# jackhwalters/DCS-Net

Measured on AMD Instinct MI355X. Metric: STFT frames/sec (train fwd+bwd+Adam), higher is better.
Workload: dtype f32

## Files before the change

dcs-net_amd/csrc/attention.hip:

```cpp
#include "conv_common.h"
#include "cbn_geom.h"

namespace {

constexpr int kThreads = 256;
#ifndef DCS_ATT_APP_IT
#define DCS_ATT_APP_IT 2
#endif
#ifndef DCS_ATT_GRID_CAP
#define DCS_ATT_GRID_CAP 8192
#endif
constexpr int kMaxChunks = DCS_ATT_MAX_CHUNKS;

inline bool att_geom(int C, int* G) { return att::geom(C, G); }
inline int ca_chunks(long HW, int G) { return att::ca_chunks(HW, G); }

__device__ __forceinline__ void ca_pool_kernel_body(const act_t* __restrict__ x, double* __restrict__ part,
                                                            long HW, int C, int G, int bx, int by, int gx) {
    __shared__ double red[kThreads * 4];
    const int t = threadIdx.x, g = t % G, r0 = t / G, rpi = kThreads / G;
    const int b = by;
    const ActIn4<act_t> x4 = act_in4(x) + (long)b * HW * G;
    float s0 = 0.f, s1 = 0.f, s2 = 0.f, s3 = 0.f;
    for (long r = (long)bx * rpi + r0; r < HW; r += (long)gx * rpi) {
        const float4 v = x4[r * G + g];
        s0 += v.x; s1 += v.y; s2 += v.z; s3 += v.w;
    }
    red[t * 4 + 0] = s0; red[t * 4 + 1] = s1; red[t * 4 + 2] = s2; red[t * 4 + 3] = s3;
    __syncthreads();
    for (int o = t; o < G * 4; o += kThreads) {
        const int gg = o / 4, i = o % 4;
        double a = 0;
        for (int r = 0; r < rpi; ++r) a += red[(r * G + gg) * 4 + i];
        part[(((long)b * gx + bx) * C + 2 * gg) * 2 + i] = a;
    }
}

__device__ __forceinline__ void ca_fc_kernel_body(const double* __restrict__ part, int nchunks,
                                                          const float2* __restrict__ w1, const float2* __restrict__ w2,
                                                          float2* __restrict__ ca_out, float2* __restrict__ pooled_out,
                                                          float2* __restrict__ hidden_out, long HW, int C, int Ch, int bx, int by, int gx) {
    __shared__ float2 pooled[128];
    __shared__ float2 hid[64];
    __shared__ double red[kThreads * 2];
    const int b = bx, t = threadIdx.x;
    {
        const int nsl = kThreads / C, c = t % C, sl = t / C;
        double sr = 0, si = 0;
        if (sl < nsl)
#pragma unroll 8
            for (int k = sl; k < nchunks; k += nsl) {
                const double* p = part + (((long)b * nchunks + k) * C + c) * 2;
                sr += p[0]; si += p[1];
            }
        red[t * 2] = sr; red[t * 2 + 1] = si;
        __syncthreads();
        if (t < C) {
            for (int q = 1; q < nsl; ++q) { sr += red[(q * C + t) * 2]; si += red[(q * C + t) * 2 + 1]; }
            const float2 m = make_float2((float)(sr / (double)HW), (float)(si / (double)HW));
            pooled[t] = m;
            pooled_out[(long)b * C + t] = m;
        }
    }
    __syncthreads();
    for (int h = t >> 5; h < Ch; h += kThreads / 32) {
        float ar = 0.f, ai = 0.f;
#pragma unroll 4
        for (int c = t & 31; c < C; c += 32) {
            const float2 w = w1[c * Ch + h], p = pooled[c];
            ar = fmaf(w.x, p.x, ar); ar = fmaf(-w.y, p.y, ar);
            ai = fmaf(w.x, p.y, ai); ai = fmaf(w.y, p.x, ai);
        }
#pragma unroll
        for (int o = 16; o > 0; o >>= 1) { ar += __shfl_xor(ar, o, 64); ai += __shfl_xor(ai, o, 64); }
        if ((t & 31) == 0) {
            hidden_out[(long)b * Ch + h] = make_float2(ar, ai);
            hid[h] = make_float2(ar > 0.f ? ar : 0.f, ai > 0.f ? ai : 0.f);
        }
    }
    __syncthreads();
    for (int c = t; c < C; c += kThreads) {
        float ar = 0.f, ai = 0.f;
#pragma unroll 8
        for (int h = 0; h < Ch; ++h) {
            const float2 w = w2[h * C + c], p = hid[h];
            ar = fmaf(w.x, p.x, ar); ar = fmaf(-w.y, p.y, ar);
            ai = fmaf(w.x, p.y, ai); ai = fmaf(w.y, p.x, ai);
        }
        ar += ar; ai += ai;
        ca_out[(long)b * C + c] = make_float2(1.f / (1.f + expf(-ar)), 1.f / (1.f + expf(-ai)));
    }
}

__device__ __forceinline__ float group_sum(float v, int G) { return dcs_group_sum(v, G); }
__device__ __forceinline__ float group_max(float v, int G) { return dcs_group_max(v, G); }

__device__ __forceinline__ void spatial_pool_kernel_body(const act_t* __restrict__ x,
                                                                 const float* __restrict__ ca,
                                                                 float4* __restrict__ pooled, long HW, int C, int G, int bx, int by, int gx) {
    const int t = threadIdx.x, g = t % G, r0 = t / G, rpi = kThreads / G;
    const int b = by;
    const ActIn4<act_t> x4 = act_in4(x) + (long)b * HW * G;
    float4 a = make_float4(1.f, 0.f, 1.f, 0.f);
    if (ca) a = reinterpret_cast<const float4*>(ca)[(long)b * G + g];
    const float invC = 1.f / (float)C;
    const long iters = (HW + (long)gx * rpi - 1) / ((long)gx * rpi);
    for (long k = 0; k < iters; ++k) {
        const long r = (k * gx + bx) * rpi + r0;
        const bool ok = r < HW;
        float4 v = make_float4(0.f, 0.f, 0.f, 0.f);
        if (ok) v = x4[r * G + g];
        const float z0r = a.x * v.x - a.y * v.y, z0i = a.x * v.y + a.y * v.x;
        const float z1r = a.z * v.z - a.w * v.w, z1i = a.z * v.w + a.w * v.z;
        const float sr = group_sum(z0r + z1r, G), si = group_sum(z0i + z1i, G);
        const float mr = group_max(fmaxf(z0r, z1r), G), mi = group_max(fmaxf(z0i, z1i), G);
        if (ok && g == 0) pooled[(long)b * HW + r] = make_float4(sr * invC, si * invC, mr, mi);
    }
}

template <bool DROP>
__device__ __forceinline__ void attention_apply_kernel_body(const act_t* __restrict__ x,
                                                                    const float* __restrict__ ca,
                                                                    const float2* __restrict__ sa, act_t* __restrict__ y,
                                                                    long HW, int C, int G, float drop_p, uint64_t seed, const uint64_t* __restrict__ seed_dev, int bx, int by, int gx) {
    if (seed_dev) seed += seed_dev[0];
    const int t = threadIdx.x, g = t % G, r0 = t / G, rpi = kThreads / G;
    const int b = by;
    const long base = (long)b * HW * G;
    const ActIn4<act_t> x4 = act_in4(x) + base;
    const ActOut4<act_t> y4 = act_out4(y) + base;
    float4 a = make_float4(1.f, 0.f, 1.f, 0.f);
    if (ca) a = reinterpret_cast<const float4*>(ca)[(long)b * G + g];
    const float inv_keep = DROP ? 1.f / (1.f - drop_p) : 1.f;
    for (long r = (long)bx * rpi + r0; r < HW; r += (long)gx * rpi) {
        const float4 v = x4[r * G + g];
        float2 s = make_float2(1.f, 0.f);
        if (sa) s = sa[(long)b * HW + r];
        const float z0r = fmaf(a.x, v.x, -(a.y * v.y)), z0i = fmaf(a.x, v.y, a.y * v.x);
        const float z1r = fmaf(a.z, v.z, -(a.w * v.w)), z1i = fmaf(a.z, v.w, a.w * v.z);
        float4 o;
        o.x = fmaf(s.x, z0r, -(s.y * z0i)); o.y = fmaf(s.x, z0i, s.y * z0r);
        o.z = fmaf(s.x, z1r, -(s.y * z1i)); o.w = fmaf(s.x, z1i, s.y * z1r);
        if (DROP) {
            const uint64_t e = (uint64_t)(base + r * G + g) * 4;
            o.x *= dcs_keep_scale(seed, e, drop_p, inv_keep);
            o.y *= dcs_keep_scale(seed, e + 1, drop_p, inv_keep);
            o.z *= dcs_keep_scale(seed, e + 2, drop_p, inv_keep);
            o.w *= dcs_keep_scale(seed, e + 3, drop_p, inv_keep);
        }
        y4[r * G + g] = o;
    }
}

constexpr int kMaxBatch = 8;
template <class P> struct Tbl { P p[kMaxBatch]; int x0[kMaxBatch + 1]; };
template <class P> __device__ __forceinline__ int tbl_find(const Tbl<P>& t, int bx) {
    int z = 0;
#pragma unroll
    for (int k = 1; k < kMaxBatch; ++k) z += bx >= t.x0[k] ? 1 : 0;
    return z;
}

struct CaPoolP { const act_t* x; double* part; long HW; int C, G, nx; };
struct CaFcP { const double* part; int nchunks; const float2* w1; const float2* w2; float2* ca; float2* pooled; float2* hidden;
               long HW; int C, Ch; };
struct SpPoolP { const act_t* x; const float* ca; float4* pooled; long HW; int C, G, nx; };
struct ApplyP { const act_t* x; const float* ca; const float2* sa; act_t* y; long HW; int C, G, nx; };

__global__ __launch_bounds__(kThreads) void ca_pool_kernel(CaPoolP p) {
    ca_pool_kernel_body(p.x, p.part, p.HW, p.C, p.G, blockIdx.x, blockIdx.y, gridDim.x);
}
__global__ __launch_bounds__(kThreads) void ca_pool_multi_kernel(Tbl<CaPoolP> t) {
    const int z = tbl_find(t, blockIdx.x);
    const CaPoolP& p = t.p[z];
    ca_pool_kernel_body(p.x, p.part, p.HW, p.C, p.G, blockIdx.x - t.x0[z], blockIdx.y, p.nx);
}
__global__ __launch_bounds__(kThreads) void ca_fc_kernel(CaFcP p) {
    ca_fc_kernel_body(p.part, p.nchunks, p.w1, p.w2, p.ca, p.pooled, p.hidden, p.HW, p.C, p.Ch, blockIdx.x, 0, 0);
}
__global__ __launch_bounds__(kThreads) void ca_fc_multi_kernel(Tbl<CaFcP> t) {
    const CaFcP& p = t.p[blockIdx.z];
    ca_fc_kernel_body(p.part, p.nchunks, p.w1, p.w2, p.ca, p.pooled, p.hidden, p.HW, p.C, p.Ch, blockIdx.x, 0, 0);
}
__global__ __launch_bounds__(kThreads) void spatial_pool_kernel(SpPoolP p) {
    spatial_pool_kernel_body(p.x, p.ca, p.pooled, p.HW, p.C, p.G, blockIdx.x, blockIdx.y, gridDim.x);
}
__global__ __launch_bounds__(kThreads) void spatial_pool_multi_kernel(Tbl<SpPoolP> t) {
    const int z = tbl_find(t, blockIdx.x);
    const SpPoolP& p = t.p[z];
    spatial_pool_kernel_body(p.x, p.ca, p.pooled, p.HW, p.C, p.G, blockIdx.x - t.x0[z], blockIdx.y, p.nx);
}
template <bool DROP>
__global__ __launch_bounds__(kThreads) void attention_apply_kernel(ApplyP p, float drop_p, uint64_t seed, const uint64_t* seed_dev) {
    attention_apply_kernel_body<DROP>(p.x, p.ca, p.sa, p.y, p.HW, p.C, p.G, drop_p, seed, seed_dev, blockIdx.x, blockIdx.y, gridDim.x);
}
__global__ __launch_bounds__(kThreads) void attention_apply_multi_kernel(Tbl<ApplyP> t) {
    const int z = tbl_find(t, blockIdx.x);
    const ApplyP& p = t.p[z];
    attention_apply_kernel_body<false>(p.x, p.ca, p.sa, p.y, p.HW, p.C, p.G, 0.f, 0, nullptr, blockIdx.x - t.x0[z], blockIdx.y, p.nx);
}

#ifndef DCS_ACT_BF16
__global__ __launch_bounds__(kThreads) void dropout_kernel(const float* __restrict__ x, float* __restrict__ y, long n,
                                                            float drop_p, uint64_t seed, const uint64_t* __restrict__ seed_dev) {
    if (seed_dev) seed += seed_dev[0];
    const float inv_keep = 1.f / (1.f - drop_p);
    for (long i = (long)blockIdx.x * kThreads + threadIdx.x; i < n; i += (long)gridDim.x * kThreads)
        y[i] = x[i] * (drop_p > 0.f ? dcs_keep_scale(seed, (uint64_t)i, drop_p, inv_keep) : 1.f);
}
#endif

inline int stream_grid(long HW, int G, int B) {
    const int rpi = kThreads / G;
    long it = (HW + rpi - 1) / rpi;
    long nb = it <= DCS_ATT_SMALL_IT ? (it + DCS_ATT_APP_IT - 1) / DCS_ATT_APP_IT : (it + 3) / 4;
    long cap = (it <= DCS_ATT_SMALL_IT ? DCS_ATT_GRID_CAP : 2048) / (B > 0 ? B : 1);
    if (cap < 1) cap = 1;
    return (int)(nb < 1 ? 1 : (nb > cap ? cap : nb));
}

}

#ifndef DCS_ACT_BF16
extern "C" long dcs_ca_workspace_bytes(int B, long HW, int C) {
    int G;
    if (B <= 0 || HW <= 0 || !att_geom(C, &G)) return -1;
    return (long)B * ca_chunks(HW, G) * C * 2 * (long)sizeof(double);
}
#endif

extern "C" int DCS_SYM(dcs_channel_attention_fwd)(const act_t* x, const float* w1, const float* w2, float* ca_out,
                                         float* pooled_out, float* hidden_out, void* workspace, long workspace_bytes,
                                         int B, long HW, int C, int Ch, dcs_stream_t stream) {
    int G;
    if (!x || !w1 || !w2 || !ca_out || !pooled_out || !hidden_out || !workspace) return DCS_ERR_BADARG;
    if (B <= 0 || B > 65535 || HW <= 0 || !att_geom(C, &G) || Ch <= 0 || Ch > 64) return DCS_ERR_BADARG;
    const int nch = ca_chunks(HW, G);
    if (workspace_bytes < (long)B * nch * C * 2 * (long)sizeof(double)) return DCS_ERR_WORKSPACE;
    hipStream_t s = dcs_stream(stream);
    const CaPoolP pp{x, (double*)workspace, HW, C, G, nch};
    DCS_LAUNCH(ca_pool_kernel, dim3(nch, B), dim3(kThreads), 0, s, pp);
    DCS_CHECK_LAUNCH();
    const CaFcP fp{(const double*)workspace, nch, (const float2*)w1, (const float2*)w2, (float2*)ca_out, (float2*)pooled_out,
                   (float2*)hidden_out, HW, C, Ch};
    DCS_LAUNCH(ca_fc_kernel, dim3(B), dim3(kThreads), 0, s, fp);
    DCS_CHECK_LAUNCH();
    return DCS_OK;
}

#ifndef DCS_ACT_BF16
extern "C" int dcs_ca_pool_chunks(long HW, int C) {
    int G;
    if (HW <= 0 || !att_geom(C, &G)) return -1;
    return ca_chunks(HW, G);
}

extern "C" int dcs_channel_attention_fc_fwd(const void* part, const float* w1, const float* w2, float* ca_out,
                                            float* pooled_out, float* hidden_out, int B, long HW, int C, int Ch,
                                            dcs_stream_t stream) {
    int G;
    if (!part || !w1 || !w2 || !ca_out || !pooled_out || !hidden_out) return DCS_ERR_BADARG;
    if (B <= 0 || B > 65535 || HW <= 0 || !att_geom(C, &G) || Ch <= 0 || Ch > 64) return DCS_ERR_BADARG;
    const CaFcP fp{(const double*)part, ca_chunks(HW, G), (const float2*)w1, (const float2*)w2, (float2*)ca_out,
                   (float2*)pooled_out, (float2*)hidden_out, HW, C, Ch};
    DCS_LAUNCH(ca_fc_kernel, dim3(B), dim3(kThreads), 0, dcs_stream(stream), fp);
    DCS_CHECK_LAUNCH();
    return DCS_OK;
}
#endif

extern "C" int DCS_SYM(dcs_spatial_pool_fwd)(const act_t* x, const float* ca, float* pooled, int B, long HW, int C,
                                    dcs_stream_t stream) {
    int G;
    if (!x || !pooled || B <= 0 || B > 65535 || HW <= 0 || !att_geom(C, &G)) return DCS_ERR_BADARG;
    const int nx = stream_grid(HW, G, B);
    const SpPoolP sp{x, ca, (float4*)pooled, HW, C, G, nx};
    DCS_LAUNCH(spatial_pool_kernel, dim3(nx, B), dim3(kThreads), 0, dcs_stream(stream), sp);
    DCS_CHECK_LAUNCH();
    return DCS_OK;
}

extern "C" int DCS_SYM(dcs_attention_apply_fwd)(const act_t* x, const float* ca, const float* sa, act_t* y, int B, long HW,
                                       int C, float drop_p, unsigned long long seed, const unsigned long long* seed_dev, dcs_stream_t stream) {
    int G;
    if (!x || !y || B <= 0 || B > 65535 || HW <= 0 || !att_geom(C, &G)) return DCS_ERR_BADARG;
    if (!(drop_p >= 0.f && drop_p < 1.f)) return DCS_ERR_BADARG;
    const int nx = stream_grid(HW, G, B);
    dim3 grid(nx, B);
    const ApplyP ap{x, ca, (const float2*)sa, y, HW, C, G, nx};
    if (drop_p > 0.f)
        DCS_LAUNCH(attention_apply_kernel<true>, grid, dim3(kThreads), 0, dcs_stream(stream), ap, drop_p,
                           (uint64_t)seed, (const uint64_t*)seed_dev);
    else
        DCS_LAUNCH(attention_apply_kernel<false>, grid, dim3(kThreads), 0, dcs_stream(stream), ap, drop_p,
                           (uint64_t)seed, (const uint64_t*)seed_dev);
    DCS_CHECK_LAUNCH();
    return DCS_OK;
}

static long fwd_batched_workspace_bytes(int n, const dcs_attention_item* items, int B) {
    if (n < 1 || n > kMaxBatch || !items || B <= 0) return -1;
    long total = 0;
    for (int i = 0; i < n; ++i) {
        int G;
        if (!att_geom(items[i].C, &G)) return -1;
        const long b = (long)B * ca_chunks((long)items[i].H * items[i].W, G) * items[i].C * 2 * (long)sizeof(double);
        total += (b + 255) / 256 * 256;
    }
    return total;
}

#ifndef DCS_ACT_BF16
extern "C" long dcs_attention_fwd_batched_workspace_bytes(int n, const dcs_attention_item* items, int B) {
    return fwd_batched_workspace_bytes(n, items, B);
}
#endif

extern "C" int DCS_SYM(dcs_attention_fwd_batched)(int n, const dcs_attention_item* items, void* workspace, long workspace_bytes, int B,
                                         dcs_stream_t stream) {
    if (n < 1 || n > kMaxBatch || !items || !workspace || B <= 0 || B > 65535) return DCS_ERR_BADARG;
    if (workspace_bytes < fwd_batched_workspace_bytes(n, items, B)) return DCS_ERR_WORKSPACE;
    Tbl<CaPoolP> tp; Tbl<CaFcP> tf; Tbl<SpPoolP> ts; Tbl<ApplyP> ta;
    conv::Args ca_[kMaxBatch];
    int nx_pool = 1, nx_stream = 1;
    char* ws = (char*)workspace;
    for (int i = 0; i < n; ++i) {
        const dcs_attention_item& it = items[i];
        int G;
        if (!it.x || !it.w1 || !it.w2 || !it.wsa || !it.sa_bias || !it.ca || !it.pooled || !it.hidden || !it.sp || !it.sa ||
            !it.y || it.H <= 0 || it.W <= 0 || it.Ch <= 0 || it.Ch > 64 || !att_geom(it.C, &G))
            return DCS_ERR_BADARG;
        const long HW = (long)it.H * it.W;
        const int nch = ca_chunks(HW, G), nxs = stream_grid(HW, G, B);
        tp.p[i] = CaPoolP{(const act_t*)it.x, (double*)ws, HW, it.C, G, nch};
        tf.p[i] = CaFcP{(const double*)ws, nch, (const float2*)it.w1, (const float2*)it.w2, (float2*)it.ca, (float2*)it.pooled,
                        (float2*)it.hidden, HW, it.C, it.Ch};
        ts.p[i] = SpPoolP{(const act_t*)it.x, it.ca, (float4*)it.sp, HW, it.C, G, nxs};
        ta.p[i] = ApplyP{(const act_t*)it.x, it.ca, (const float2*)it.sa, (act_t*)it.y, HW, it.C, G, nxs};
        ws += ((long)B * nch * it.C * 2 * (long)sizeof(double) + 255) / 256 * 256;
        nx_pool = nch > nx_pool ? nch : nx_pool;
        nx_stream = nxs > nx_stream ? nxs : nx_stream;
        conv::Args& a = ca_[i];
        a = conv::Args{};
        a.x1 = (const act2_t*)it.sp;     a.x2 = nullptr; a.wp = (const float2*)it.wsa; a.bias = (const float2*)it.sa_bias;
        a.y = (act2_t*)it.sa;
        a.B = B; a.Hin = it.H; a.Win = it.W; a.C1 = 2; a.C2 = 0; a.up_f = 1; a.up_t = 1; a.zero_ins = 0; a.Cout = 1;
        a.kh = 7; a.kw = 7; a.sf = 1; a.st = 1; a.pad_f = 3; a.pad_t = 3; a.act = DCS_ACT_SIGMOID;
        a.Hv = it.H; a.Wv = it.W; a.Hout = it.H; a.Wout = it.W;
    }
    hipStream_t s = dcs_stream(stream);
    {
        int ap = 0, as_ = 0;
        for (int k = 0; k <= kMaxBatch; ++k) {
            tp.x0[k] = k < n ? ap : 0x7fffffff; ts.x0[k] = ta.x0[k] = k < n ? as_ : 0x7fffffff;
            if (k < n) { ap += tp.p[k].nx; as_ += ts.p[k].nx; }
        }
        tp.x0[n] = ap; ts.x0[n] = ta.x0[n] = as_;
        nx_pool = ap; nx_stream = as_;
    }
    DCS_LAUNCH(ca_pool_multi_kernel, dim3(nx_pool, B, 1), dim3(kThreads), 0, s, tp);
    DCS_CHECK_LAUNCH();
    DCS_LAUNCH(ca_fc_multi_kernel, dim3(B, 1, n), dim3(kThreads), 0, s, tf);
    DCS_CHECK_LAUNCH();
    DCS_LAUNCH(spatial_pool_multi_kernel, dim3(nx_stream, B, 1), dim3(kThreads), 0, s, ts);
    DCS_CHECK_LAUNCH();
    const int rc = dcs_conv_direct_multi(ca_, n, s);
    if (rc != DCS_OK) return rc;
    DCS_LAUNCH(attention_apply_multi_kernel, dim3(nx_stream, B, 1), dim3(kThreads), 0, s, ta);
    DCS_CHECK_LAUNCH();
    return DCS_OK;
}

#ifndef DCS_ACT_BF16
extern "C" int dcs_dropout_fwd(const float* x, float* y, long n, float drop_p, unsigned long long seed,
                               const unsigned long long* seed_dev, dcs_stream_t stream) {
    if (!x || !y || n <= 0 || !(drop_p >= 0.f && drop_p < 1.f)) return DCS_ERR_BADARG;
    long nb = (n + kThreads * 4 - 1) / (kThreads * 4);
    const int grid = (int)(nb < 1 ? 1 : (nb > 2048 ? 2048 : nb));
    DCS_LAUNCH(dropout_kernel, dim3(grid), dim3(kThreads), 0, dcs_stream(stream), x, y, n, drop_p,
                       (uint64_t)seed, (const uint64_t*)seed_dev);
    DCS_CHECK_LAUNCH();
    return DCS_OK;
}
#endif
```

dcs-net_amd/dcsnet/_lib.py:

```python
import ctypes
import os

_HERE = os.path.dirname(os.path.abspath(__file__))
LIB_PATH = os.environ.get('DCS_LIB_PATH') or os.path.join(os.path.dirname(_HERE), 'lib', 'libdcsnet_hip.so')

ACT_NONE, ACT_RELU, ACT_LRELU, ACT_SIGMOID = 0, 1, 2, 3

_P = ctypes.c_void_p
_I = ctypes.c_int
_L = ctypes.c_long
_F = ctypes.c_float
_U64 = ctypes.c_ulonglong



class AttentionItem(ctypes.Structure):
    _fields_ = [(n, _P) for n in ('x', 'w1', 'w2', 'wsa', 'sa_bias', 'ca', 'pooled', 'hidden', 'sp', 'sa', 'y', 'g_out',
                                  'wsa_bwd', 'g_pre', 'g_sp', 'g_x', 'g_fc0_r', 'g_fc0_i', 'g_fc2_r', 'g_fc2_i')] + \
               [(n, _I) for n in ('H', 'W', 'C', 'Ch')] + [('g_pooled', _P)]


SIGNATURES = {
    'dcs_abi_version': (_I, []),
    'dcs_error_string': (ctypes.c_char_p, [_I]),
    'dcs_pack_conv_weight': (_I, [_P, _P, _P, _P, _P, _P, _I, _I, _I, _I, _I, _I, _I, _P]),
    'dcs_cconv2d_fwd_workspace_bytes': (_L, [_I] * 14),
    'dcs_cconv2d_fwd': (_I, [_P, _P, _P, _P, _P, _P, _L] + [_I] * 15 + [_P]),
    'dcs_cconv2d_fwd_affine': (_I, [_P, _P, _P, _P, _P, _P, _P, _L] + [_I] * 15 + [_P]),
    'dcs_cconv2d_fwd_stats_rows': (_I, [_I] * 14),
    'dcs_cconv2d_fwd_stats': (_I, [_P] * 6 + [_I, _P, _P, _L] + [_I] * 14 + [_P]),
    'dcs_rconv2d_fwd_workspace_bytes': (_L, [_I] * 14),
    'dcs_rconv2d_fwd': (_I, [_P, _P, _P, _P, _P, _P, _L] + [_I] * 15 + [_P]),
    'dcs_rconv2d_bwd_data_workspace_bytes': (_L, [_I] * 11),
    'dcs_rconv2d_bwd_data': (_I, [_P, _P, _P, _P, _L] + [_I] * 11 + [_P]),
    'dcs_rbn_fwd': (_I, [_P] * 9 + [_L, _L, _I, _F, _F, _I, _I, _P]),
    'dcs_rbn_bwd': (_I, [_P] * 8 + [_L, _L, _I, _I, _I, _P]),
    'dcs_packed_weight_floats': (_L, [_I] * 6),
    'dcs_packed_weight_bwd_floats': (_L, [_I] * 10),
    'dcs_pack_conv_weight_bwd': (_I, [_P, _P] + [_I] * 10 + [_P]),
    'dcs_cconv2d_bwd_data_workspace_bytes': (_L, [_I] * 14),
    'dcs_cconv2d_bwd_data': (_I, [_P] * 5 + [_L] + [_I] * 14 + [_P]),
    'dcs_upsample_cat_bwd': (_I, [_P, _P, _P] + [_I] * 7 + [_P]),
    'dcs_cconv2d_bwd_weight_workspace_bytes': (_L, [_I] * 14),
    'dcs_cconv2d_bwd_weight': (_I, [_P] * 8 + [_L] + [_I] * 15 + [_P]),
    'dcs_cbn_workspace_bytes': (_L, [_L, _I]),
    'dcs_cbn_fwd': (_I, [_P] * 9 + [_L, _L, _I, _F, _F, _I, _I, _F, _U64, _P, _P]),
    'dcs_cbn_fwd_slabs': (_I, [_P] * 9 + [_I, _I, _P, _L, _I, _F, _F, _I, _F, _U64, _P, _P]),
    'dcs_ca_pool_chunks': (_I, [_L, _I]),
    'dcs_cbn_fwd_slabs_pool': (_I, [_P] * 9 + [_I, _I, _P, _P, _L, _I, _L, _I, _F, _F, _I, _P]),
    'dcs_channel_attention_fc_fwd': (_I, [_P] * 6 + [_I, _L, _I, _I, _P]),
    'dcs_cbn_bwd_workspace_bytes': (_L, [_L, _I]),
    'dcs_cbn_bwd': (_I, [_P] * 9 + [_L, _L, _I, _I, _I, _F, _U64, _P, _P]),
    'dcs_cbn_bwd_add': (_I, [_P] * 9 + [_L, _L, _I, _I, _I, _F, _U64, _P, _P, _F, _L, _P, _P]),
    'dcs_ca_workspace_bytes': (_L, [_I, _L, _I]),
    'dcs_channel_attention_fwd': (_I, [_P] * 7 + [_L, _I, _L, _I, _I, _P]),
    'dcs_spatial_pool_fwd': (_I, [_P, _P, _P, _I, _L, _I, _P]),
    'dcs_attention_apply_fwd': (_I, [_P, _P, _P, _P, _I, _L, _I, _F, _U64, _P, _P]),
    'dcs_rattention_workspace_bytes': (_L, [_I, _L, _I]),
    'dcs_rattention_fwd': (_I, [_P] * 8 + [_L] + [_I] * 6 + [_P]),
    'dcs_rattention_train_workspace_bytes': (_L, [_I, _L, _I, _I]),
    'dcs_rattention_pool_fwd': (_I, [_P] * 8 + [_L] + [_I] * 5 + [_P]),
    'dcs_rattention_apply_fwd': (_I, [_P] * 4 + [_I] * 4 + [_P]),
    'dcs_rattention_apply_bwd': (_I, [_P] * 8 + [_L] + [_I] * 4 + [_P]),
    'dcs_rattention_pool_bwd': (_I, [_P] * 11 + [_I] + [_P, _L] + [_I] * 5 + [_P]),
    'dcs_attention_bwd_sa': (_I, [_P] * 5 + [_I, _L, _I, _F, _U64, _P, _P]),
    'dcs_attention_bwd_workspace_bytes': (_L, [_I, _L, _I, _I]),
    'dcs_attention_bwd_x': (_I, [_P] * 16 + [_L, _I, _L, _I, _I, _F, _U64, _P, _P]),
    'dcs_attention_bwd_fc_weights': (_I, [_P, _L, _P, _P, _P, _P, _P, _P, _I, _L, _I, _I, _P]),
    'dcs_attention_fwd_batched_workspace_bytes': (_L, [_I, _P, _I]),
    'dcs_attention_fwd_batched': (_I, [_I, _P, _P, _L, _I, _P]),
    'dcs_attention_bwd_batched_workspace_bytes': (_L, [_I, _P, _I]),
    'dcs_attention_bwd_batched': (_I, [_I, _P, _P, _L, _I, _P]),
    'dcs_lstm_layer_fwd': (_I, [_P] * 6 + [_I, _I, _I, _I, _L, _L, _L, _P]),
    'dcs_lstm_layer_fwd_bias': (_I, [_P, _P, _P, _P, _P, _P, _P, _P, _I, _I, _I, _I, _L, _L, _L, _P]),
    'dcs_lstm_layer_bwd': (_I, [_P] * 6 + [_I] * 4 + [_P]),
    'dcs_dropout_fwd': (_I, [_P, _P, _L, _F, _U64, _P, _P]),
    'dcs_complex_act_fwd': (_I, [_P, _P, _L, _I, _P]),
    'dcs_complex_upsample_fwd': (_I, [_P, _P, _I, _I, _I, _I, _I, _I, _P]),
    'dcs_tapsum_fwd': (_I, [_P, _P, _P, _P] + [_I] * 10 + [_P]),
    'dcs_cconv_up2_single_fwd': (_I, [_P] * 6 + [_I] * 6 + [_P]),
    'dcs_cconv_up2_single_bwd_data': (_I, [_P] * 4 + [_I] * 6 + [_P]),
    'dcs_cconv_up2_single_bwd_weight_workspace_bytes': (_L, []),
    'dcs_cconv_up2_single_bwd_weight': (_I, [_P] * 7 + [_I, _P, _L] + [_I] * 5 + [_P]),
    'dcs_tapsum_bwd_workspace_bytes': (_L, []),
    'dcs_tapsum_bwd': (_I, [_P, _P, _P, _P, _P, _L] + [_I] * 10 + [_P]),
    'dcs_bound_crm_fwd': (_I, [_P, _P, _L, _F, _P]),
    'dcs_bound_mask_apply_fwd': (_I, [_P, _P, _P, _P, _P, _L, _F, _P]),
    'dcs_bound_mask_apply_bwd': (_I, [_P] * 6 + [_L, _F, _P]),
    'dcs_bound2_mask_apply_fwd': (_I, [_P] * 6 + [_L, _F, _F, _U64, _P, _P]),
    'dcs_bound2_mask_apply_bwd': (_I, [_P] * 7 + [_L, _F, _F, _U64, _P, _P]),
    'dcs_bound2_apply_polar_frames_fwd': (_I, [_P] * 4 + [_I] * 4 + [_F, _F, _U64, _P, _P]),
    'dcs_bound2_apply_polar_frames_bwd': (_I, [_P] * 5 + [_I] * 4 + [_F, _I, _F, _U64, _P, _P]),
    'dcs_complex_abs_f32': (_I, [_P, _P, _L, _P]),
    'dcs_rmask_apply_polar_frames_fwd': (_I, [_P] * 4 + [_I] * 4 + [_F, _I, _P]),
    'dcs_rmask_apply_polar_frames_bwd': (_I, [_P] * 5 + [_I] * 4 + [_F, _I, _I, _P]),
    'dcs_irfft512_frames': (_I, [_P, _P, _L, _P]),
    'dcs_rfft512_frames': (_I, [_P, _P, _L, _P]),
    'dcs_rfft512_ola_frames': (_I, [_P, _P, _P, _P, _I, _I, _I, _F, _P]),
    'dcs_irfft512_ola_frames': (_I, [_P, _P, _P, _P, _I, _I, _I, _F, _P]),
    'dcs_polar_frames_fwd': (_I, [_P, _P, _I, _I, _I, _I, _F, _P]),
    'dcs_polar_frames_bwd': (_I, [_P, _P, _P, _I, _I, _I, _I, _F, _I, _P]),
    'dcs_istft_envelope': (_I, [_P, _P, _I, _I, _I, _P]),
    'dcs_istft_ola_fwd': (_I, [_P, _P, _P, _P, _I, _I, _I, _I, _F, _P]),
    'dcs_istft_ola_bwd': (_I, [_P, _P, _P, _P, _I, _I, _I, _I, _F, _P]),
    'dcs_stft_frames_fwd': (_I, [_P, _P, _P, _P, _I, _I, _I, _I, _I, _P]),
    'dcs_stft_bins_fwd': (_I, [_P, _P, _I, _I, _I, _F, _P]),
    'dcs_sisnr_fwd': (_I, [_P, _P, _P, _P, _I, _I, _F, _P]),
    'dcs_sisnr_bwd': (_I, [_P, _P, _P, _P, _F, _P, _I, _I, _P]),
    'dcs_sisnr_losses_fwd': (_I, [_P, _P, _P, _I, _F, _P]),
    'dcs_lstm_whh_grad': (_I, [_P, _P, _P, _I, _I, _I, _P]),
    'dcs_atb_chunks': (_I, [_P, _P, _P, _L, _L, _L, _L, _I, _I, _I, _I, _I, _I, _I, _I, _P]),
    'dcs_chunk_sum_acc': (_I, [_P, _P, _L, _L, _I, _I, _I, _L, _P]),
    'dcs_atb_chunks_strided': (_I, [_P, _P, _P, _L, _L, _L, _L, _I, _I, _I, _I, _I, _I, _I, _I, _I, _P]),
    'dcs_gemm_f32': (_I, [_P, _P, _P] + [_I] * 8 + [_L, _L, _I, _L, _L, _L, _I, _I, _P]),
    'dcs_lstm_combine_fwd': (_I, [_P, _P, _L, _P]),
    'dcs_lstm_combine_bwd': (_I, [_P, _P, _L, _P]),
    'dcs_lstm_param_grads': (_I, [_P, _P, _P, _P, _P, _I, _I, _I, _P]),
    'dcs_lstm_param_grads_ih': (_I, [_P, _P, _P, _P, _P, _I, _I, _I, _P, _P, _I, _L, _I, _P]),
    'dcs_sisnr_losses_guard_fwd': (_I, [_P, _P, _P, _I, _F, _P, _P]),
    'dcs_sisnr_pair_bwd': (_I, [_P, _P, _P, _P, _P, _P, _F, _P, _I, _I, _P]),
    'dcs_crm_fwd': (_I, [_P, _P, _P, _L, _F, _P]),
    'dcs_adam_amsgrad_step': (_I, [_P] * 6 + [_F, _F, _L, _P, _F, _F, _F, _F, _I, _P, _P, _P]),
    'dcs_adam_amsgrad_step_sumsq': (_I, [_P] * 6 + [_I, _F, _F, _L, _P, _F, _F, _F, _F, _I, _P, _P, _P]),
    'dcs_swa_average_f32': (_I, [_P, _P, _L, _L, _P]),
    'dcs_grad_sumsq_parts': (_I, [_P, _L, _P, _I, _P, _P, _P, _P, _I, _P]),
    'dcs_step_guard': (_I, [_P, _P, _P]),
    'dcs_stream_hold': (_I, [_P, _I, _P]),
    'dcs_kernel_timer_begin': (_I, [_I]),
    'dcs_kernel_timer_end': (_I, []),
    'dcs_kernel_timer_read': (_I, [_I, _P]),
    'dcs_step_advance': (_I, [_P, _P, _P, _P]),
    'dcs_step_advance_counters': (_I, [_P, _P, _P, _P, _I, _P]),
    'dcs_pack_tap_rows': (_I, [_P, _P, _P, _P, _I, _I, _I, _I, _P]),
    'dcs_tap_rows_wgrad_scatter': (_I, [_P, _P, _P, _P, _I, _I, _I, _I, _P]),
    'dcs_set_conv_precision': (_I, [_I]),
    'dcs_get_conv_precision': (_I, []),
    'dcs_wgrad_defer_begin': (_I, []),
    'dcs_wgrad_defer_suspend': (_I, [_I]),
    'dcs_wgrad_defer_flush': (_I, [_P]),
    'dcs_pack_plan_begin': (_I, []),
    'dcs_pack_plan_end': (_I, [_P]),
    'dcs_pack_plan_jobs': (_I, [_P, _P, _P]),
    'dcs_pack_plan_run': (_I, [_P, _P]),
    'dcs_pack_plan_destroy': (_I, [_P]),
    'dcs_resample_poly_f32': (_I, [_P, _P, _I, _L, _P, _I, _I, _I, _P]),
    'dcs_stoi_workspace_bytes': (_L, [_I, _L]),
    'dcs_stoi_f32': (_I, [_P, _P, _I, _L, _P, _P, _P, _P, _P, _L, _P]),
    'dcs_resample_sinc_f32': (_I, [_P, _P, _P, _P, _I, _L, _P, _I, _I, _I, _P]),
    'dcs_audio_stft_batch_f32': (_I, [_P, _P, _P, _I, _P, _P, _I, _P, _I, _I, _I, _F, _P, _P, _P, _P]),
    'dcs_audio_stft_segments_f32': (_I, [_P, _P, _I, _P, _P, _I, _P, _I, _I, _I, _I, _F, _P, _P]),
    'dcs_segments_stitch_f32': (_I, [_P, _L, _P, _P, _I, _L, _I, _I, _I, _P, _P, _P]),
}

_lib = None


class DcsHipError(RuntimeError):
    pass


for _n in ('dcs_cconv2d_fwd', 'dcs_cconv2d_fwd_affine', 'dcs_cconv2d_fwd_stats', 'dcs_cconv2d_bwd_data', 'dcs_cconv2d_bwd_weight',
           'dcs_cconv_up2_single_fwd', 'dcs_cconv_up2_single_bwd_data', 'dcs_cconv_up2_single_bwd_weight', 'dcs_tapsum_bwd', 'dcs_cbn_fwd', 'dcs_cbn_fwd_slabs', 'dcs_cbn_fwd_slabs_pool', 'dcs_cbn_bwd', 'dcs_cbn_bwd_add',
           'dcs_channel_attention_fwd', 'dcs_spatial_pool_fwd', 'dcs_attention_apply_fwd', 'dcs_attention_fwd_batched',
           'dcs_attention_bwd_sa', 'dcs_attention_bwd_x', 'dcs_attention_bwd_batched'):
    SIGNATURES[_n + '_h'] = SIGNATURES[_n]


def load():
    global _lib
    if _lib is not None:
        return _lib
    import torch
    if not os.path.exists(LIB_PATH):
        raise DcsHipError(f'{LIB_PATH} not found: build it with `python dcs-net_amd/build.py` '
                          '(there is no CPU or eager fallback)')
    lib = ctypes.CDLL(LIB_PATH)
    for name, (res, args) in SIGNATURES.items():
        try:
            fn = getattr(lib, name)
        except AttributeError as e:
            raise DcsHipError(f'{LIB_PATH} does not export {name}; rebuild it') from e
        fn.restype = res
        fn.argtypes = args
    _lib = lib
    return lib


def check(code, what):
    if code != 0:
        msg = load().dcs_error_string(code).decode()
        raise DcsHipError(f'{what}: {msg} (code {code})')


def ptr(t):
    return None if t is None else t.data_ptr()


def cur_stream():
    import torch
    return torch.cuda.current_stream().cuda_stream
```

dcs-net_amd/dcsnet/functional.py:

```python
import os
import weakref

import torch

from . import _derived
from . import ops
from .ops import ACT_NONE, ACT_RELU, ACT_LRELU, ACT_SIGMOID, to_nhwc, from_nhwc
from ._lib import DcsHipError

_PACKED = _derived.Derived(capacity=512)


def bump_param_generation():
    _derived.bump_generation()
    ops.pack_plan_invalidate()


def note_state_update():
    _derived.bump_generation()


state_generation = _derived.generation


def begin_pack_plan():
    _derived.bump_generation()
    return ops.pack_plan_begin()


def end_pack_plan():
    return ops.pack_plan_end()


def run_pack_plan(plan):
    ops.pack_plan_run(plan)


def packed_weight(w_r, w_i, b_r, b_i, transposed, up=(1, 1), tap_rows=0):
    plan = ops.PLAN
    if plan is not None:
        pkey = (id(w_r), id(w_i), id(b_r), id(b_i), bool(transposed), tuple(up), int(tap_rows))
        if plan.valid and not plan.recording:
            e = plan.fwd.get(pkey)
            if e is not None and e[0][0]() is w_r and e[0][1]() is w_i and e[2] == (
                    w_r._version, w_i._version, None if b_r is None else b_r._version,
                    None if b_i is None else b_i._version):
                return e[1]

    def make():
        d = lambda t: None if t is None else t.detach()
        wr, wi = d(w_r), d(w_i)
        if wr.dim() == 2:
            wr, wi = wr.view(*wr.shape, 1, 1), wi.view(*wi.shape, 1, 1)
        if tap_rows:
            packed = ops.pack_tap_rows(wr, wi, int(tap_rows))
        else:
            packed = ops.pack_conv_weight(wr, wi, d(b_r), d(b_i), transposed, tuple(up))
        if plan is not None and plan.recording:
            wref = lambda t: None if t is None else weakref.ref(t)
            plan.fwd[pkey] = [(wref(w_r), wref(w_i), wref(b_r), wref(b_i)), packed, None]
        return packed
    return _PACKED.get(w_r, (bool(transposed), tuple(up), int(tap_rows)), (w_r, w_i, b_r, b_i), make, ops.conv_precision())


ATTENTION_BATCH_MAX = ops.ATTENTION_BATCH_MAX

FLUSH_AT_NEXT_FORK = False
WGRAD_SIDE = None
sink_hits = 0


def _sink(p):
    if p is None or not p.requires_grad:
        return None
    s = getattr(p, '_dcs_grad_sink', None)
    if s is None or p.grad is None or p.grad.data_ptr() != s.data_ptr():
        return None
    global sink_hits
    sink_hits += 1
    return s


DEFER_FC = os.environ.get('DCS_DEFER_FC', '1') != '0'
PENDING_SIDE = []


def _run_pending_side():
    while PENDING_SIDE:
        job = PENDING_SIDE.pop(0)
        ops.attention_bwd_fc_weights(job)
        if ops.WGRAD_DEFER is not None:
            ops.WGRAD_DEFER.append(job)


class _CConv2dFn(torch.autograd.Function):

    @staticmethod
    def forward(ctx, x1, x2, w_r, w_i, b_r, b_i, transposed, ksize, stride, pad, up, act, holder=None):
        wp, bias = packed_weight(w_r, w_i, b_r, b_i, transposed, up)
        if holder is not None:
            y, holder['stat'] = ops.cconv2d_stats(x1, x2, wp, bias, ksize, stride, pad, up)
        else:
            y = ops.cconv2d(x1, x2, wp, bias, ksize, stride, pad, up, act)
        ctx.geom = (transposed, tuple(ksize), tuple(stride), tuple(pad), tuple(up), act, tuple(w_r.shape),
                    b_r is not None)
        ctx.sinks = (_sink(w_r), _sink(w_i), _sink(b_r), _sink(b_i))
        ctx.save_for_backward(x1, x2, wp, y if act == ACT_SIGMOID else None)
        return y

    @staticmethod
    def backward(ctx, gy):
        x1, x2, wp, y = ctx.saved_tensors
        transposed, ksize, stride, pad, up, act, w_shape, has_bias = ctx.geom
        gy = gy.contiguous()
        if act == ACT_SIGMOID:
            gy = gy * y * (1.0 - y)
        elif act != ACT_NONE:
            raise DcsHipError('cconv2d backward: only ACT_NONE / ACT_SIGMOID epilogues are differentiable here')
        gx1 = gx2 = gw_r = gw_i = gb_r = gb_i = None
        need = ctx.needs_input_grad
        want_w = need[2] or need[3] or need[4] or need[5]
        side = None
        if (want_w and WGRAD_SIDE is not None and ops.WGRAD_DEFER is not None and gy.is_cuda and
                ctx.sinks[0] is not None and ctx.sinks[1] is not None and (not has_bias or (ctx.sinks[2] is not None and ctx.sinks[3] is not None))):
            side = WGRAD_SIDE
            side.wait_stream(torch.cuda.current_stream())
        if need[0] or need[1]:
            C1 = x1.shape[3]
            Cin = C1 + (x2.shape[3] if x2 is not None else 0)
            gx1, gx2 = ops.cconv2d_bwd_data(gy, ops.pack_conv_weight_bwd(wp, ksize, stride, pad, up),
                                            (x1.shape[1], x1.shape[2], Cin), ksize, stride, pad, up, C1)
        if want_w:
            if side is not None:
                with torch.cuda.stream(side):
                    _run_pending_side()
                    g = ops.cconv2d_bwd_weight(x1, x2, gy, w_shape, has_bias, ksize, stride, pad, up, transposed, ctx.sinks,
                                               immediate=True)
                    global FLUSH_AT_NEXT_FORK
                    if FLUSH_AT_NEXT_FORK:
                        FLUSH_AT_NEXT_FORK = False
                        ops.wgrad_defer_flush(partial=True)
            else:
                g = ops.cconv2d_bwd_weight(x1, x2, gy, w_shape, has_bias, ksize, stride, pad, up, transposed, ctx.sinks)
            gw_r, gw_i, gb_r, gb_i = (None if sk is not None else t for t, sk in zip(g, ctx.sinks))
        return gx1, gx2, gw_r, gw_i, gb_r, gb_i, None, None, None, None, None, None, None


def cconv2d(x1, x2, w_r, w_i, b_r, b_i, transposed, ksize, stride, pad, up=(1, 1), act=ACT_NONE):
    return _CConv2dFn.apply(x1, x2, w_r, w_i, b_r, b_i, transposed, tuple(ksize), tuple(stride), tuple(pad),
                            tuple(up), act)


def cconv2d_with_stats(x1, x2, w_r, w_i, b_r, b_i, transposed, ksize, stride, pad, up=(1, 1)):
    holder = {}
    y = _CConv2dFn.apply(x1, x2, w_r, w_i, b_r, b_i, transposed, tuple(ksize), tuple(stride), tuple(pad), tuple(up),
                         ACT_NONE, holder)
    return y, holder.get('stat')


def cconv2d_cbn_eval(x1, x2, w_r, w_i, b_r, b_i, transposed, ksize, stride, pad, up, coef, act):
    wp, bias = packed_weight(w_r, w_i, b_r, b_i, transposed, tuple(up))
    return ops.cconv2d(x1, x2, wp, bias, tuple(ksize), tuple(stride), tuple(pad), tuple(up), act, coef=coef)


class _CbnFn(torch.autograd.Function):

    @staticmethod
    def forward(ctx, x, weight, bias, running_mean, running_covar, eps, momentum, use_batch_stats, act, drop_p, seed, stat=None):
        y, stats, coef = ops.cbn(x, weight, bias, running_mean, running_covar, eps, momentum, use_batch_stats,
                                 act, drop_p, seed, stat=stat)
        ctx.cfg = (bool(use_batch_stats), act, float(drop_p), int(seed), weight is not None)
        ctx.sinks = (_sink(weight), _sink(bias))
        ctx.save_for_backward(x, weight, stats, coef)
        return y

    @staticmethod
    def backward(ctx, g_out):
        x, weight, stats, coef = ctx.saved_tensors
        use_batch, act, drop_p, seed, affine = ctx.cfg
        g_x, g_w, g_b = ops.cbn_bwd(x, g_out.contiguous(), weight, stats, coef, use_batch, act, drop_p, seed, affine,
                                    ctx.sinks, need_gx=ctx.needs_input_grad[0])
        g_w = None if ctx.sinks[0] is not None else g_w
        g_b = None if ctx.sinks[1] is not None else g_b
        return g_x, g_w, g_b, None, None, None, None, None, None, None, None, None


def cbn(x, weight, bias, running_mean, running_covar, eps, momentum, use_batch_stats, act=ACT_NONE,
        drop_p=0.0, seed=0, stat=None):
    return _CbnFn.apply(x, weight, bias, running_mean, running_covar, eps, momentum, use_batch_stats, act,
                        drop_p, seed, stat)


class _CbnTwoFn(torch.autograd.Function):

    @staticmethod
    def forward(ctx, x, weight, bias, running_mean, running_covar, eps, momentum, use_batch_stats, act, drop_p, seed, stat=None):
        y, stats, coef = ops.cbn(x, weight, bias, running_mean, running_covar, eps, momentum, use_batch_stats,
                                 act, drop_p, seed, stat=stat)
        ctx.cfg = (bool(use_batch_stats), act, float(drop_p), int(seed), weight is not None)
        ctx.sinks = (_sink(weight), _sink(bias))
        ctx.save_for_backward(x, weight, stats, coef)
        ctx.set_materialize_grads(False)
        y2 = torch.empty(0, dtype=y.dtype, device=y.device).set_(y.untyped_storage(), y.storage_offset(), y.shape, y.stride())
        return y, y2

    @staticmethod
    def backward(ctx, g_a, g_b):
        x, weight, stats, coef = ctx.saved_tensors
        use_batch, act, drop_p, seed, affine = ctx.cfg
        if g_a is None and g_b is None:
            return (None,) * 12
        if g_a is None:
            g_a, g_b = g_b, None
        g_add = None
        for g_ in (g_a, g_b):
            if g_ is not None and _POOL_ADD:
                hit = _POOL_ADD.pop(g_.data_ptr(), None)
                if hit is not None:
                    if g_add is not None:
                        raise DcsHipError('cbn_two backward: two split pool terms for one stage output')
                    g_add = hit
        g_x, g_w, g_b_ = ops.cbn_bwd(x, g_a.contiguous(), weight, stats, coef, use_batch, act, drop_p, seed, affine,
                                     ctx.sinks, g_add=g_add, g_out2=None if g_b is None else g_b.contiguous())
        g_w = None if ctx.sinks[0] is not None else g_w
        g_b_ = None if ctx.sinks[1] is not None else g_b_
        return g_x, g_w, g_b_, None, None, None, None, None, None, None, None, None


def cbn_two(x, weight, bias, running_mean, running_covar, eps, momentum, use_batch_stats, act=ACT_NONE,
            drop_p=0.0, seed=0, stat=None):
    y, y2 = _CbnTwoFn.apply(x, weight, bias, running_mean, running_covar, eps, momentum, use_batch_stats, act,
                            drop_p, seed, stat)
    y2._dcs_adds_pool_term = True
    return y, y2


def channel_attention(x, fc0_r, fc0_i, fc2_r, fc2_i):
    w1, _ = packed_weight(fc0_r, fc0_i, None, None, False)
    w2, _ = packed_weight(fc2_r, fc2_i, None, None, False)
    ca, _, _ = ops.channel_attention(x, w1, w2)
    return ca


def spatial_attention(x, ca, conv_r, conv_i, ksize):
    pooled = ops.spatial_pool(x, ca)
    wp, bias = packed_weight(conv_r, conv_i, None, None, False)
    k = (ksize, ksize)
    return ops.cconv2d(pooled, None, wp, bias, k, (1, 1), (ksize // 2, ksize // 2), (1, 1), ACT_SIGMOID)


def attention_apply(x, ca, sa, drop_p=0.0, seed=0):
    return ops.attention_apply(x, ca, sa, drop_p, seed)


class _AttentionFn(torch.autograd.Function):

    @staticmethod
    def forward(ctx, x, fc0_r, fc0_i, fc2_r, fc2_i, c1_r, c1_i, ksize, drop_p, seed):
        w1, _ = packed_weight(fc0_r, fc0_i, None, None, False)
        w2, _ = packed_weight(fc2_r, fc2_i, None, None, False)
        wsa, zero_bias = packed_weight(c1_r, c1_i, None, None, False)
        ca, pooled, hidden = ops.channel_attention(x, w1, w2)
        sp = ops.spatial_pool(x, ca)
        sa = ops.cconv2d(sp, None, wsa, zero_bias, (ksize, ksize), (1, 1), (ksize // 2, ksize // 2), (1, 1),
                         ACT_SIGMOID)
        out = ops.attention_apply(x, ca, sa, drop_p, seed)
        ctx.cfg = (ksize, float(drop_p), int(seed))
        ctx.sinks = tuple(_sink(t) for t in (fc0_r, fc0_i, fc2_r, fc2_i, c1_r, c1_i))
        ctx.save_for_backward(x, ca, sa, sp, pooled, hidden, w1, w2, wsa)
        return out

    @staticmethod
    def backward(ctx, g_out):
        x, ca, sa, sp, pooled, hidden, w1, w2, wsa = ctx.saved_tensors
        ksize, drop_p, seed = ctx.cfg
        g = ops.attention_bwd(x, g_out.contiguous(), ca, sa, sp, pooled, hidden, w1, w2, wsa, ksize, drop_p, seed,
                              ctx.sinks)
        gw = tuple(None if sk is not None else t for t, sk in zip(g[1:], ctx.sinks))
        return (g[0], *gw, None, None, None)


def attention_block(x, fc0_r, fc0_i, fc2_r, fc2_i, c1_r, c1_i, ksize, drop_p=0.0, seed=0):
    return _AttentionFn.apply(x, fc0_r, fc0_i, fc2_r, fc2_i, c1_r, c1_i, ksize, drop_p, seed)


class _CbnAttentionFn(torch.autograd.Function):

    @staticmethod
    def forward(ctx, x, weight, bias, running_mean, running_covar, eps, momentum, use_batch_stats, act,
                fc0_r, fc0_i, fc2_r, fc2_i, c1_r, c1_i, ksize, drop_p, seed, stat=None):
        w1, _ = packed_weight(fc0_r, fc0_i, None, None, False)
        w2, _ = packed_weight(fc2_r, fc2_i, None, None, False)
        wsa, zero_bias = packed_weight(c1_r, c1_i, None, None, False)
        if stat is not None and use_batch_stats and weight is not None and ops.FUSE_APPLY_POOL:
            a, stats, coef, ca, pooled, hidden = ops.cbn_channel_attention(x, weight, bias, running_mean, running_covar, eps,
                                                                           momentum, act, stat, w1, w2)
        else:
            a, stats, coef = ops.cbn(x, weight, bias, running_mean, running_covar, eps, momentum, use_batch_stats, act, 0.0, 0,
                                     stat=stat)
            ca, pooled, hidden = ops.channel_attention(a, w1, w2)
        sp = ops.spatial_pool(a, ca)
        sa = ops.cconv2d(sp, None, wsa, zero_bias, (ksize, ksize), (1, 1), (ksize // 2, ksize // 2), (1, 1), ACT_SIGMOID)
        out = ops.attention_apply(a, ca, sa, drop_p, seed)
        ctx.cfg = (bool(use_batch_stats), act, weight is not None, ksize, float(drop_p), int(seed))
        ctx.sinks = tuple(_sink(t) for t in (weight, bias, fc0_r, fc0_i, fc2_r, fc2_i, c1_r, c1_i))
        ctx.save_for_backward(x, weight, stats, coef, a, ca, sa, sp, pooled, hidden, w1, w2, wsa)
        return out

    @staticmethod
    def backward(ctx, g_out):
        x, weight, stats, coef, a, ca, sa, sp, pooled, hidden, w1, w2, wsa = ctx.saved_tensors
        use_batch, act, affine, ksize, drop_p, seed = ctx.cfg
        sk = ctx.sinks
        defer = DEFER_FC and WGRAD_SIDE is not None and ops.WGRAD_DEFER is not None and all(s_ is not None for s_ in sk[2:6])
        g = ops.attention_bwd(a, g_out.contiguous(), ca, sa, sp, pooled, hidden, w1, w2, wsa, ksize, drop_p, seed, sk[2:],
                              split_pool=True, defer_fc=defer)
        if defer:
            PENDING_SIDE.append(g[8])
        g_x, g_w, g_b = ops.cbn_bwd(x, g[0], weight, stats, coef, use_batch, act, 0.0, 0, affine, sk[:2], g_add=g[7])
        full = (g_w, g_b, *g[1:7])
        gp = tuple(None if s_ is not None else t for t, s_ in zip(full, sk))
        return (g_x, gp[0], gp[1], None, None, None, None, None, None, *gp[2:], None, None, None, None)


def cbn_attention(x, weight, bias, running_mean, running_covar, eps, momentum, use_batch_stats, act,
                  fc0_r, fc0_i, fc2_r, fc2_i, c1_r, c1_i, ksize, drop_p=0.0, seed=0, stat=None):
    return _CbnAttentionFn.apply(x, weight, bias, running_mean, running_covar, eps, momentum, use_batch_stats, act,
                                 fc0_r, fc0_i, fc2_r, fc2_i, c1_r, c1_i, ksize, drop_p, seed, stat)


class _AttentionBlocksFn(torch.autograd.Function):

    @staticmethod
    def forward(ctx, n, ksize, split, *args):
        xs, params = args[:n], [args[n + 6 * i:n + 6 * i + 6] for i in range(n)]
        ctx.split = tuple(split)
        w1s, w2s, wsas, biases = [], [], [], []
        for fc0_r, fc0_i, fc2_r, fc2_i, c1_r, c1_i in params:
            w1s.append(packed_weight(fc0_r, fc0_i, None, None, False)[0])
            w2s.append(packed_weight(fc2_r, fc2_i, None, None, False)[0])
            wsa, zero_bias = packed_weight(c1_r, c1_i, None, None, False)
            wsas.append(wsa)
            biases.append(zero_bias)
        outs = ops.attention_blocks_fwd(xs, w1s, w2s, wsas, biases)
        ctx.n, ctx.ksize = n, ksize
        ctx.sinks = [tuple(_sink(t) for t in pr) for pr in params]
        ctx.shapes = [(tuple(pr[0].shape), tuple(pr[2].shape)) for pr in params]
        saved = []
        for x, o, w1, w2, wsa in zip(xs, outs, w1s, w2s, wsas):
            saved += [x, o['ca'], o['sa'], o['sp'], o['pooled'], o['hidden'], w1, w2, wsa]
        ctx.save_for_backward(*saved)
        return tuple(o['y'] for o in outs)

    @staticmethod
    def backward(ctx, *g_outs):
        n, ksize = ctx.n, ctx.ksize
        t = ctx.saved_tensors
        k, pad = (ksize, ksize), (ksize // 2, ksize // 2)
        saved, gs, wbs, fcs, sps = [], [], [], [], []
        for i in range(n):
            x, ca, sa, sp, pooled, hidden, w1, w2, wsa = t[9 * i:9 * i + 9]
            saved.append(dict(x=x, ca=ca, sa=sa, pooled=pooled, hidden=hidden, w1=w1, w2=w2))
            sps.append(sp)
            g = g_outs[i]
            gs.append(torch.zeros_like(x) if g is None else g.contiguous())
            wbs.append(ops.pack_conv_weight_bwd(wsa, k, (1, 1), pad))
            sk, (s0, s2) = ctx.sinks[i], ctx.shapes[i]
            new = lambda shape: torch.empty(shape, dtype=torch.float32, device=x.device)
            fcs.append(tuple(sk[j] if sk[j] is not None else new(s0 if j < 2 else s2) for j in range(4)))
        split = tuple(sp_ and ctx.needs_input_grad[3 + i] for i, sp_ in enumerate(ctx.split))
        res = ops.attention_blocks_bwd(saved, gs, wbs, fcs, split)
        if any(split):
            _POOL_ADD.clear()
            for (g_x, _, g_pooled), sp_ in zip(res, split):
                if sp_:
                    _POOL_ADD[g_x.data_ptr()] = g_pooled
            torch.autograd.Variable._execution_engine.queue_callback(_pool_add_consumed)
        grads_x, grads_p = [], []
        for i in range(n):
            g_x, g_pre, _ = res[i]
            sk = ctx.sinks[i]
            g_c1r, g_c1i, _, _ = ops.cconv2d_bwd_weight(sps[i], None, g_pre, (1, 2, ksize, ksize), False, k, (1, 1), pad,
                                                        outs=(sk[4], sk[5], None, None))
            full = (*fcs[i], g_c1r, g_c1i)
            grads_x.append(g_x)
            grads_p += [None if s_ is not None else g_ for g_, s_ in zip(full, sk)]
        global FLUSH_AT_NEXT_FORK
        if WGRAD_SIDE is not None and ops.WGRAD_DEFER is not None:
            ops.WGRAD_DEFER.append((sps, [r[1] for r in res]))
            FLUSH_AT_NEXT_FORK = True
        return (None, None, None, *grads_x, *grads_p)


SPLIT_SKIP_POOL = os.environ.get('DCS_SPLIT_SKIP_POOL', '1') != '0'
_POOL_ADD = {}


def _pool_add_consumed():
    if _POOL_ADD:
        _POOL_ADD.clear()
        raise DcsHipError('attention_blocks backward: a split average-pool term was not consumed by a cbn_two backward')


def attention_blocks(xs, params, ksize):
    flat = [p for pr in params for p in pr]
    split = tuple(bool(SPLIT_SKIP_POOL and getattr(x, '_dcs_adds_pool_term', False) and torch.is_grad_enabled() and x.requires_grad)
                  for x in xs)
    return _AttentionBlocksFn.apply(len(xs), ksize, split, *xs, *flat)



def _as_real(z):
    if z.dtype != torch.complex64:
        raise DcsHipError(f'expected complex64, got {z.dtype}')
    return torch.view_as_real(z.contiguous() if not _dense(z) else z)


def _dense(z):
    return z.is_contiguous() or (z.dim() == 4 and z.is_contiguous(memory_format=torch.channels_last))


def _elementwise(z, act):
    if z.dim() == 4 and z.is_contiguous(memory_format=torch.channels_last) and not z.is_contiguous():
        x = to_nhwc(z)
        return from_nhwc(ops.complex_act(x, act))
    x = torch.view_as_real(z.contiguous())
    return torch.view_as_complex(ops.complex_act(x, act))


def complex_relu(z):
    return _elementwise(z, ACT_RELU)


def complex_lrelu(z):
    return _elementwise(z, ACT_LRELU)


def complex_sigmoid(z):
    return _elementwise(z, ACT_SIGMOID)


def complex_upsample(z, scale_factor):
    sf = (scale_factor, scale_factor) if isinstance(scale_factor, (int, float)) else tuple(scale_factor)
    up = (int(sf[0]), int(sf[1]))
    if up != tuple(sf) or min(up) < 1:
        raise DcsHipError(f'complex_upsample: integer scale factors only, got {scale_factor}')
    return from_nhwc(ops.complex_upsample(to_nhwc(z), up))


def complex_linear(z, w_r, w_i, b_r, b_i):
    in_f = z.shape[-1]
    lead = z.shape[:-1]
    x = torch.view_as_real(z.reshape(-1, in_f).contiguous())
    N = x.shape[0]
    W = 16 if N % 16 == 0 else 1
    x = x.view(1, N // W, W, in_f, 2)
    y = cconv2d(x, None, w_r, w_i, b_r, b_i, False, (1, 1), (1, 1), (0, 0))
    return torch.view_as_complex(y.view(N, -1, 2)).view(*lead, -1)


class _LstmRecFn(torch.autograd.Function):

    @staticmethod
    def forward(ctx, gx, w_hh):
        n_sets, seqs, S, _, G4 = gx.shape
        need = gx.requires_grad or w_hh.requires_grad
        out, gates, c = ops.lstm_layer(gx, w_hh, n_sets, seqs, S, (seqs * S * 2 * G4, S * 2 * G4, 2 * G4), need)
        ctx.dims = (n_sets, seqs, S)
        if need:
            ctx.save_for_backward(out, gates, c, w_hh)
        return out

    @staticmethod
    def backward(ctx, g_out):
        out, gates, c, w_hh = ctx.saved_tensors
        n_sets, seqs, S = ctx.dims
        H = w_hh.shape[-1]
        g_pre = ops.lstm_layer_bwd(g_out.contiguous(), gates, c, w_hh, n_sets, seqs, S)
        g_pre5 = g_pre.view(n_sets, seqs, S, 2, 4 * H)
        g_whh = None
        if ctx.needs_input_grad[1]:
            o = out.view(n_sets, seqs, S, 2, H)
            h_prev = torch.zeros_like(o)
            h_prev[:, :, 1:, 0] = o[:, :, :-1, 0]
            h_prev[:, :, :-1, 1] = o[:, :, 1:, 1]
            g_whh = torch.einsum('sntdj,sntdk->sdjk', g_pre5, h_prev)
        return g_pre5, g_whh


def _project(inp, w_ih, shared, per_set=False, train=True):
    G8, K = w_ih.shape[1], w_ih.shape[2]
    M = inp.shape[-2]
    if not (ops.gemm_ok(M, G8, K, 2, train) and inp.is_contiguous() and w_ih.is_contiguous()):
        if shared and not per_set:
            return torch.mm(inp, w_ih.reshape(2 * G8, -1).t())
        return torch.matmul(inp, w_ih.transpose(1, 2))
    if shared and not per_set:
        gx = torch.empty((M, 2 * G8), dtype=torch.float32, device=inp.device)
        return ops.gemm_f32(inp, w_ih, gx, M, 2 * G8, K, K, K, 2 * G8, True)
    gx = torch.empty((2, M, G8), dtype=torch.float32, device=inp.device)
    return ops.gemm_f32(inp, w_ih, gx, M, G8, K, K, K, G8, True, nbatch=2, a_batch=0 if shared else M * K, b_batch=G8 * K,
                        c_batch=M * G8)


def _project_bwd(g_gx, w_ih, shared):
    G8, K = w_ih.shape[1], w_ih.shape[2]
    M = g_gx.shape[1]
    if not (ops.gemm_ok(M, K, G8, 2, True) and g_gx.is_contiguous() and w_ih.is_contiguous()):
        if shared:
            g_inp = torch.mm(g_gx[0], w_ih[0])
            return g_inp.addmm_(g_gx[1], w_ih[1])
        return torch.bmm(g_gx, w_ih)
    if shared:
        g_inp = torch.empty((M, K), dtype=torch.float32, device=g_gx.device)
        return ops.gemm_f32(g_gx, w_ih, g_inp, M, K, G8, G8, K, K, False, nseg=2, a_seg=M * G8, b_seg=G8 * K)
    g_inp = torch.empty((2, M, K), dtype=torch.float32, device=g_gx.device)
    return ops.gemm_f32(g_gx, w_ih, g_inp, M, K, G8, G8, K, K, False, nbatch=2, a_batch=M * G8, b_batch=G8 * K, c_batch=M * K)


class _ProjectFn(torch.autograd.Function):

    @staticmethod
    def forward(ctx, inp, w_ih):
        ctx.save_for_backward(inp, w_ih)
        return _project(inp, w_ih, shared=inp.dim() == 2, per_set=True)

    @staticmethod
    def backward(ctx, g):
        inp, w_ih = ctx.saved_tensors
        g = g.contiguous()
        g_inp = _project_bwd(g, w_ih, shared=inp.dim() == 2) if ctx.needs_input_grad[0] else None
        g_w = torch.matmul(g.transpose(1, 2), inp) if ctx.needs_input_grad[1] else None
        return g_inp, g_w


class _LstmLayerFn(torch.autograd.Function):

    @staticmethod
    def forward(ctx, inp, anchor, st, B2, S):
        w_ih, w_hh = st['weight_ih'][0], st['weight_hh'][0]
        need = inp.requires_grad or anchor.requires_grad
        ctx.planes = 0
        if inp.is_complex():
            zr = torch.view_as_real(inp)
            G8, K = w_ih.shape[1], w_ih.shape[2]
            ctx.planes = R0 = zr.shape[0] * zr.shape[1]
            gx = torch.empty((2 * R0, 2 * G8), dtype=torch.float32, device=inp.device)
            ops.gemm_f32(zr, w_ih, gx, 2 * R0, 2 * G8, K, K, K, 2 * G8, True, a_planes=R0)
            inp = zr
            G4 = G8 // 2
            strides = (G8, S * 2 * G8, 2 * G8)
        elif inp.dim() == 2:
            G8 = w_ih.shape[1]
            gx = _project(inp, w_ih, shared=True)
            G4 = G8 // 2
            strides = (G8, S * 2 * G8, 2 * G8)
        else:
            gx = _project(inp, w_ih, shared=False)
            G4 = gx.shape[-1] // 2
            strides = (B2 * S * 2 * G4, S * 2 * G4, 2 * G4)
        out, gates, c, hprev = ops.lstm_layer(gx, w_hh, 2, B2, S, strides, need, True,
                                              bias=(st['bias_ih'][0], st['bias_hh'][0]))
        ctx.st, ctx.dims = st, (B2, S)
        if need:
            ctx.save_for_backward(inp, hprev, gates, c)
        return out

    @staticmethod
    def backward(ctx, g_out):
        global sink_hits
        inp, hprev, gates, c = ctx.saved_tensors
        st, (B2, S) = ctx.st, ctx.dims
        w_ih, w_hh = st['weight_ih'][0], st['weight_hh'][0]
        H = w_hh.shape[-1]
        NT = B2 * S
        g_pre, b_part = ops.lstm_layer_bwd(g_out.contiguous(), gates, c, w_hh, 2, B2, S, True)
        g_gx = g_pre.view(2, NT, 8 * H)
        _LstmLayerFn._param_grads(st, inp, hprev, g_pre, b_part, g_gx, B2, S, H, NT, planes=ctx.planes)
        if ctx.planes:
            g_z = None
            if ctx.needs_input_grad[0]:
                G8, K = w_ih.shape[1], w_ih.shape[2]
                gz = torch.empty(inp.shape, dtype=torch.float32, device=inp.device)
                ops.gemm_f32(g_gx, w_ih, gz, NT, K, G8, G8, K, K, False, nseg=2, a_seg=NT * G8, b_seg=G8 * K, c_planes=ctx.planes)
                g_z = torch.view_as_complex(gz)
            return g_z, None, None, None, None
        g_inp = _project_bwd(g_gx, w_ih, shared=inp.dim() == 2) if ctx.needs_input_grad[0] else None
        return g_inp, None, None, None, None

    @staticmethod
    def _param_grads(st, inp, hprev, g_pre, b_part, g_gx, B2, S, H, NT, planes=0):
        global sink_hits
        CK = 16 if NT % 32 == 0 else 1
        if H % 64 == 0 and NT % (8 * CK) == 0:
            part = ops.lstm_whh_grad(g_pre, hprev, NT, CK, H)
        else:
            R = NT // CK
            part = torch.empty((2, 2 * CK, 4 * H, H), dtype=g_pre.dtype, device=g_pre.device)
            for d in range(2):
                a = g_pre.as_strided((2 * CK, R, 4 * H), (R * 8 * H, 8 * H, 1), g_pre.storage_offset() + d * 4 * H)
                h = hprev.as_strided((2 * CK, R, H), (R * 2 * H, 2 * H, 1), hprev.storage_offset() + d * H)
                torch.bmm(a.transpose(1, 2), h, out=part[d])
        b_part = b_part.contiguous()
        g_wih = st['weight_ih'][1]
        sink_hits += 16
        ih = None
# ... 563 lines not shown
```

dcs-net_amd/dcsnet/ops.py:

```python
import os as _os
import torch

from . import _lib
from ._lib import ACT_NONE, ACT_RELU, ACT_LRELU, ACT_SIGMOID, check, ptr, cur_stream


def _chk(t, name, dims=None, act=False):
    if t is None:
        return
    if not t.is_cuda:
        raise _lib.DcsHipError(f'{name}: expected a CUDA (HIP) tensor; the HIP path has no CPU fallback')
    if t.dtype != torch.float32 and not (act and t.dtype == torch.bfloat16):
        raise _lib.DcsHipError(f'{name}: expected float32{" or bfloat16" if act else ""}, got {t.dtype}')
    if not t.is_contiguous():
        raise _lib.DcsHipError(f'{name}: expected a contiguous tensor')
    if dims is not None and t.dim() != dims:
        raise _lib.DcsHipError(f'{name}: expected {dims} dims, got shape {tuple(t.shape)}')


def _sym(name, *acts):
    dts = {t.dtype for t in acts if t is not None}
    if len(dts) > 1:
        raise _lib.DcsHipError(f'{name}: activation tensors of different dtypes {sorted(str(d) for d in dts)}')
    bf = dts == {torch.bfloat16}
    if bf and conv_precision() != 'bf16' and 'conv' in name:
        raise _lib.DcsHipError(f'{name}: bf16 activations need set_conv_precision("bf16") (bf16 weight panels)')
    return getattr(_lib.load(), name + ('_h' if bf else ''))


CONV_TIMER = None

SEED_STATE = None

_workspaces = {}
_retired = []


def set_conv_precision(mode):
    code = {'f32': 0, 'fp32': 0, 'bf16': 1, 'bf16x6': 2}[mode]
    check(_lib.load().dcs_set_conv_precision(code), 'dcs_set_conv_precision')
    global BF16_OPERANDS_ON_PURPOSE, _conv_precision
    _conv_precision = _CONV_PRECISIONS[code]
    if code != 1:
        BF16_OPERANDS_ON_PURPOSE = False
    elif not _IN_SET_ACTIVATION_DTYPE:
        BF16_OPERANDS_ON_PURPOSE = True
    pack_plan_drop()


BF16_OPERANDS_ON_PURPOSE = _os.environ.get('DCS_CONV_PRECISION', '').strip() == '1'
_IN_SET_ACTIVATION_DTYPE = False


_CONV_PRECISIONS = ('f32', 'bf16', 'bf16x6')
_conv_precision = None


def conv_precision():
    global _conv_precision
    if _conv_precision is None:
        _conv_precision = _CONV_PRECISIONS[_lib.load().dcs_get_conv_precision()]
    return _conv_precision


class PackPlan:

    def __init__(self):
        self.handle, self.recording, self.valid = None, True, False
        self.fwd, self.bwd, self.keep = {}, {}, []

    def stats(self):
        import ctypes
        nj, nl = ctypes.c_int(0), ctypes.c_int(0)
        check(_lib.load().dcs_pack_plan_jobs(self.handle, ctypes.byref(nj), ctypes.byref(nl)), 'dcs_pack_plan_jobs')
        return nj.value, nl.value

    def __del__(self):
        try:
            if self.handle:
                _lib.load().dcs_pack_plan_destroy(self.handle)
        except Exception:
            pass


PLAN = None


def pack_plan_begin():
    global PLAN
    check(_lib.load().dcs_pack_plan_begin(), 'dcs_pack_plan_begin')
    PLAN = PackPlan()
    return PLAN


def pack_plan_end():
    import ctypes
    h = ctypes.c_void_p()
    plan = PLAN
    check(_lib.load().dcs_pack_plan_end(ctypes.byref(h)), 'dcs_pack_plan_end')
    plan.handle, plan.recording = h.value, False
    _plan_snapshot(plan)
    plan.valid = True
    return plan


def _plan_snapshot(plan):
    for e in plan.fwd.values():
        e[2] = tuple(None if r is None or r() is None else r()._version for r in e[0])


def pack_plan_run(plan):
    global PLAN
    PLAN = plan
    check(_lib.load().dcs_pack_plan_run(plan.handle, cur_stream()), 'dcs_pack_plan_run')
    _plan_snapshot(plan)
    plan.valid = True


def pack_plan_invalidate():
    if PLAN is not None:
        PLAN.valid = False


def pack_plan_drop():
    global PLAN
    PLAN = None



def _workspace(nbytes, device):
    key = (device.index, cur_stream())
    buf = _workspaces.get(key)
    if buf is None or buf.numel() < nbytes:
        if buf is not None:
            _retired.append(buf)
        buf = torch.empty(max(int(nbytes), 1 << 20), dtype=torch.uint8, device=device)
        _workspaces[key] = buf
    return buf


def pack_conv_weight(w_r, w_i, b_r=None, b_i=None, transposed=False, up=(1, 1)):
    for n, t in (('w_r', w_r), ('w_i', w_i), ('b_r', b_r), ('b_i', b_i)):
        _chk(t, n)
    if transposed:
        Cin, Cout, kh, kw = w_r.shape
    else:
        Cout, Cin, kh, kw = w_r.shape
    lib = _lib.load()
    buf = torch.empty(lib.dcs_packed_weight_floats(Cout, Cin, kh, kw, up[0], up[1]), dtype=torch.float32,
                      device=w_r.device)
    wp = buf[:kh * kw * Cin * Cout * 2].view(kh * kw, Cin, Cout, 2)
    bias = torch.empty((Cout, 2), dtype=torch.float32, device=w_r.device)
    check(lib.dcs_pack_conv_weight(ptr(w_r), ptr(w_i), ptr(b_r), ptr(b_i), ptr(wp), ptr(bias),
                                   Cout, Cin, kh, kw, int(bool(transposed)), up[0], up[1], cur_stream()),
          'dcs_pack_conv_weight')
    return wp, bias


def pack_tap_rows(w_r, w_i, ct):
    _chk(w_r, 'w_r', 4)
    _chk(w_i, 'w_i', 4)
    Cin, one, kh, kw = w_r.shape
    if one != 1 or ct < kh * kw:
        raise _lib.DcsHipError(f'pack_tap_rows: expected [Cin,1,kh,kw] and ct >= kh*kw, got {tuple(w_r.shape)}, ct={ct}')
    lib = _lib.load()
    buf = torch.empty(lib.dcs_packed_weight_floats(ct, Cin, 1, 1, 1, 1), dtype=torch.float32, device=w_r.device)
    wp = buf[:Cin * ct * 2].view(1, Cin, ct, 2)
    bias = torch.empty((ct, 2), dtype=torch.float32, device=w_r.device)
    check(lib.dcs_pack_tap_rows(ptr(w_r), ptr(w_i), ptr(wp), ptr(bias), Cin, kh, kw, ct, cur_stream()), 'dcs_pack_tap_rows')
    return wp, bias


def tap_rows_scatter(gt_r, gt_i, w_shape, outs=None):
    Cin, _, kh, kw = w_shape
    acc = outs is not None and outs[0] is not None and outs[1] is not None
    g_r = outs[0] if acc else torch.empty(w_shape, dtype=torch.float32, device=gt_r.device)
    g_i = outs[1] if acc else torch.empty(w_shape, dtype=torch.float32, device=gt_r.device)
    check(_lib.load().dcs_tap_rows_wgrad_scatter(ptr(gt_r), ptr(gt_i), ptr(g_r), ptr(g_i), Cin, kh, kw, int(acc),
                                                 cur_stream()), 'dcs_tap_rows_wgrad_scatter')
    return g_r, g_i


def cconv2d(x1, x2, wp, bias, ksize, stride=(1, 1), pad=(0, 0), up=(1, 1), act=ACT_NONE, coef=None):
    _chk(x1, 'x1', 5, act=True)
    _chk(x2, 'x2', 5, act=True)
    _chk(wp, 'wp', 4)
    _chk(bias, 'bias', 2)
    B, Hin, Win, C1, _ = x1.shape
    C2 = 0
    if x2 is not None:
        if x2.shape[:3] != x1.shape[:3]:
            raise _lib.DcsHipError(f'cconv2d: x1 {tuple(x1.shape)} and x2 {tuple(x2.shape)} differ in B/H/W')
        C2 = x2.shape[3]
    kh, kw = ksize
    if wp.shape[0] != kh * kw or wp.shape[1] != C1 + C2:
        raise _lib.DcsHipError(f'cconv2d: packed weight {tuple(wp.shape)} does not match k={ksize}, Cin={C1 + C2}')
    Cout = wp.shape[2]
    Hout = (Hin * up[0] + 2 * pad[0] - kh) // stride[0] + 1
    Wout = (Win * up[1] + 2 * pad[1] - kw) // stride[1] + 1
    y = torch.empty((B, Hout, Wout, Cout, 2), dtype=x1.dtype, device=x1.device)
    lib = _lib.load()
    nbytes = lib.dcs_cconv2d_fwd_workspace_bytes(B, Hin, Win, C1, C2, up[0], up[1], Cout, kh, kw, stride[0], stride[1],
                                                 pad[0], pad[1])
    ws = _workspace(nbytes, x1.device) if nbytes > 0 else None
    nbytes = max(nbytes, 0)
    ev = (CONV_TIMER.begin(8.0 * B * Hout * Wout * Cout * (C1 + C2) * kh * kw, 'enc_fwd' if max(stride) > 1 else None,
                           executed=_fold_fraction(C1, C1 + C2, Cout, ksize, stride, pad, up),
                           emulated=_emulated(C1 + C2, Cout, kh * kw if tuple(up) == (1, 1) else 0) and (C1 % 2 == 0 or C1 + C2 == 1),
                           nbytes=_conv_bytes(x1, B * Hin * Win * (C1 + C2), B * Hout * Wout * Cout, kh * kw * (C1 + C2) * Cout))
          if CONV_TIMER is not None else None)
    if coef is not None:
        _chk(coef, 'coef', 2)
        if tuple(coef.shape) != (Cout, 6):
            raise _lib.DcsHipError(f'cconv2d: coef {tuple(coef.shape)} does not match Cout={Cout}')
    check(_sym('dcs_cconv2d_fwd_affine', x1, x2)(ptr(x1), ptr(x2), ptr(wp), ptr(bias), ptr(coef), ptr(y), ptr(ws), nbytes, B, Hin, Win,
                                     C1, C2, up[0], up[1], Cout, kh, kw, stride[0], stride[1], pad[0], pad[1], act,
                                     cur_stream()), 'dcs_cconv2d_fwd_affine')
    if ev is not None:
        CONV_TIMER.end(ev)
    return y


def cconv2d_stats(x1, x2, wp, bias, ksize, stride=(1, 1), pad=(0, 0), up=(1, 1)):
    import ctypes
    _chk(x1, 'x1', 5, act=True)
    _chk(x2, 'x2', 5, act=True)
    _chk(wp, 'wp', 4)
    _chk(bias, 'bias', 2)
    B, Hin, Win, C1, _ = x1.shape
    C2 = 0 if x2 is None else x2.shape[3]
    kh, kw = ksize
    Cout = wp.shape[2]
    lib = _lib.load()
    geo = (B, Hin, Win, C1, C2, up[0], up[1], Cout, kh, kw, stride[0], stride[1], pad[0], pad[1])
    rows = lib.dcs_cconv2d_fwd_stats_rows(*geo) if STATS_EPILOGUE else 0
    if rows < 1:
        return cconv2d(x1, x2, wp, bias, ksize, stride, pad, up, ACT_NONE), None
    if x2 is not None and x2.shape[:3] != x1.shape[:3]:
        raise _lib.DcsHipError(f'cconv2d: x1 {tuple(x1.shape)} and x2 {tuple(x2.shape)} differ in B/H/W')
    if wp.shape[0] != kh * kw or wp.shape[1] != C1 + C2:
        raise _lib.DcsHipError(f'cconv2d: packed weight {tuple(wp.shape)} does not match k={ksize}, Cin={C1 + C2}')
    Hout = (Hin * up[0] + 2 * pad[0] - kh) // stride[0] + 1
    Wout = (Win * up[1] + 2 * pad[1] - kw) // stride[1] + 1
    y = torch.empty((B, Hout, Wout, Cout, 2), dtype=x1.dtype, device=x1.device)
    part = torch.empty((Cout, 5, rows), dtype=torch.float32, device=x1.device)
    nbytes = max(lib.dcs_cconv2d_fwd_workspace_bytes(*geo), 0)
    ws = _workspace(nbytes, x1.device) if nbytes > 0 else None
    ev = (CONV_TIMER.begin(8.0 * B * Hout * Wout * Cout * (C1 + C2) * kh * kw, 'enc_fwd' if max(stride) > 1 else None,
                           executed=_fold_fraction(C1, C1 + C2, Cout, ksize, stride, pad, up),
                           emulated=_emulated(C1 + C2, Cout, kh * kw if tuple(up) == (1, 1) else 0) and (C1 % 2 == 0 or C1 + C2 == 1),
                           nbytes=_conv_bytes(x1, B * Hin * Win * (C1 + C2), B * Hout * Wout * Cout, kh * kw * (C1 + C2) * Cout))
          if CONV_TIMER is not None else None)
    used = ctypes.c_int(0)
    check(_sym('dcs_cconv2d_fwd_stats', x1, x2)(ptr(x1), ptr(x2), ptr(wp), ptr(bias), ptr(y), ptr(part), rows, ctypes.byref(used), ptr(ws),
                                    nbytes, *geo, cur_stream()), 'dcs_cconv2d_fwd_stats')
    if ev is not None:
        CONV_TIMER.end(ev)
    return y, (part, used.value, bias)


import os as _os
FUSE_APPLY_POOL = _os.environ.get('DCS_FUSE_APPLY_POOL', '1') != '0'
STATS_EPILOGUE = _os.environ.get('DCS_STATS_EPILOGUE', '1') != '0'


def _conv_bytes(act, n_in, n_out, n_w):
    e = 4.0 if act.dtype == torch.bfloat16 else 8.0
    w = 4.0 if conv_precision() == 'bf16' else 8.0
    return e * (n_in + n_out) + w * n_w


def _emulated(k_channels, n_channels, taps=0):
    if conv_precision() == 'bf16x6' and k_channels == 1 and n_channels == 8 and taps == 49:
        return True
    return (conv_precision() == 'bf16x6' and n_channels % 8 == 0 and
            (k_channels % 16 == 0 or (k_channels == 8 and taps in (49, 16) and n_channels != 8)))


def _wgrad_emulated(C1, Cin, Cout, ksize):
    import os
    if conv_precision() != 'bf16x6' or os.environ.get('DCS_WGRAD_X6', '1') == '0':
        return False
    if Cin % 8 or Cout % 8 or C1 % 2 or ksize[0] != ksize[1]:
        return False
    return ksize[0] in (1, 3, 5) or (ksize[0] == 7 and 16 <= Cout < 32)


def _fold_fraction(C1, Cin, Cout, ksize, stride, pad, up):
    if (tuple(ksize) == (3, 3) and tuple(stride) == (1, 1) and tuple(pad) == (1, 1) and tuple(up) in ((2, 1), (1, 2), (2, 2))
            and Cin % 8 == 0 and Cout % 8 == 0 and C1 % 2 == 0):
        return (2 if up[0] == 2 else 3) * (2 if up[1] == 2 else 3) / 9.0
    return 1.0


def pack_conv_weight_bwd(wp, ksize, stride=(1, 1), pad=(0, 0), up=(1, 1)):
    _chk(wp, 'wp', 4)
    taps, Cin, Cout, _ = wp.shape
    kh, kw = ksize
    plan = PLAN
    key = (wp.data_ptr(), tuple(ksize), tuple(stride), tuple(pad), tuple(up))
    if plan is not None and plan.valid and not plan.recording:
        hit = plan.bwd.get(key)
        if hit is not None:
            return hit
    lib = _lib.load()
    geo = (Cout, Cin, kh, kw, stride[0], stride[1], pad[0], pad[1], up[0], up[1])
    buf = torch.empty(lib.dcs_packed_weight_bwd_floats(*geo), dtype=torch.float32, device=wp.device)
    wpb = buf[:taps * Cin * Cout * 2].view(taps, Cout, Cin, 2)
    check(lib.dcs_pack_conv_weight_bwd(ptr(wp), ptr(wpb), *geo, cur_stream()), 'dcs_pack_conv_weight_bwd')
    if plan is not None and plan.recording:
        plan.bwd[key] = wpb
        plan.keep.append((wp, buf))
    return wpb


def cconv2d_bwd_data(gy, wp_bwd, in_shape, ksize, stride, pad, up=(1, 1), C1=None):
    _chk(gy, 'gy', 5, act=True)
    _chk(wp_bwd, 'wp_bwd', 4)
    B, Hout, Wout, Cout, _ = gy.shape
    Hin, Win, Cin = in_shape
    C1 = Cin if C1 is None else C1
    C2 = Cin - C1
    gx1 = torch.empty((B, Hin, Win, C1, 2), dtype=gy.dtype, device=gy.device)
    gx2 = torch.empty((B, Hin, Win, C2, 2), dtype=gy.dtype, device=gy.device) if C2 else None
    lib = _lib.load()
    geo = (B, Hin, Win, C1, C2, up[0], up[1], Cout, ksize[0], ksize[1], stride[0], stride[1], pad[0], pad[1])
    nbytes = lib.dcs_cconv2d_bwd_data_workspace_bytes(*geo)
    if nbytes < 0:
        raise _lib.DcsHipError(f'cconv2d_bwd_data: unsupported geometry {geo}')
    ws = _workspace(nbytes, gy.device) if nbytes else None
    ev = (CONV_TIMER.begin(8.0 * B * Hout * Wout * Cout * Cin * ksize[0] * ksize[1],
                           executed=_fold_fraction(C1, Cin, Cout, ksize, stride, pad, up), emulated=_emulated(Cout, Cin),
                           nbytes=_conv_bytes(gy, B * Hout * Wout * Cout, B * Hin * Win * Cin, ksize[0] * ksize[1] * Cin * Cout))
          if CONV_TIMER is not None else None)
    check(_sym('dcs_cconv2d_bwd_data', gy)(ptr(gy), ptr(wp_bwd), ptr(gx1), ptr(gx2), ptr(ws), ws.numel() if ws is not None else 0,
                                   *geo, cur_stream()), 'dcs_cconv2d_bwd_data')
    if ev is not None:
        CONV_TIMER.end(ev)
    return gx1, gx2


def cconv2d_bwd_weight(x1, x2, gy, w_shape, has_bias, ksize, stride, pad, up=(1, 1), transposed=False, outs=None, immediate=False):
    _chk(x1, 'x1', 5, act=True)
    _chk(x2, 'x2', 5, act=True)
    _chk(gy, 'gy', 5, act=True)
    B, Hin, Win, C1, _ = x1.shape
    C2 = 0 if x2 is None else x2.shape[3]
    Cout = gy.shape[3]
    dev = gy.device
    o = outs or (None, None, None, None)
    gw_r = o[0] if o[0] is not None else torch.empty(w_shape, dtype=torch.float32, device=dev)
    gw_i = o[1] if o[1] is not None else torch.empty(w_shape, dtype=torch.float32, device=dev)
    gb_r = (o[2] if o[2] is not None else torch.empty(Cout, dtype=torch.float32, device=dev)) if has_bias else None
    gb_i = (o[3] if o[3] is not None else torch.empty(Cout, dtype=torch.float32, device=dev)) if has_bias else None
    for n, t in (('gw_r', gw_r), ('gw_i', gw_i), ('gb_r', gb_r), ('gb_i', gb_i)):
        _chk(t, n)
    lib = _lib.load()
    geo = (B, Hin, Win, C1, C2, up[0], up[1], Cout, ksize[0], ksize[1], stride[0], stride[1], pad[0], pad[1])
    nbytes = lib.dcs_cconv2d_bwd_weight_workspace_bytes(*geo)
    if nbytes < 0:
        raise _lib.DcsHipError(f'cconv2d_bwd_weight: unsupported geometry {geo}')
    scope = WGRAD_DEFER
    all_out = outs is not None and o[0] is not None and o[1] is not None and (not has_bias or (o[2] is not None and o[3] is not None))
    if scope is not None and all_out:
        ws = torch.empty(max(nbytes, 16), dtype=torch.uint8, device=dev)
        scope.append((ws, x1, x2, gy))
    else:
        ws = _workspace(nbytes, dev)
    suspend = scope is not None and (not all_out or immediate)
    if suspend:
        lib.dcs_wgrad_defer_suspend(1)
    ev = None
    if CONV_TIMER is not None:
        ev = CONV_TIMER.begin(8.0 * B * gy.shape[1] * gy.shape[2] * Cout * (C1 + C2) * ksize[0] * ksize[1],
                              executed=_fold_fraction(C1, C1 + C2, Cout, ksize, stride, pad, up),
                              emulated=_wgrad_emulated(C1, C1 + C2, Cout, ksize),
                              nbytes=(_conv_bytes(x1, B * Hin * Win * (C1 + C2) + B * gy.shape[1] * gy.shape[2] * Cout, 0, 0) +
                                      8.0 * ksize[0] * ksize[1] * (C1 + C2) * Cout))
    try:
        check(_sym('dcs_cconv2d_bwd_weight', x1, x2, gy)(ptr(x1), ptr(x2), ptr(gy), ptr(gw_r), ptr(gw_i), ptr(gb_r), ptr(gb_i), ptr(ws),
                                         ws.numel(), *geo, int(bool(transposed)), cur_stream()), 'dcs_cconv2d_bwd_weight')
    finally:
        if suspend:
            lib.dcs_wgrad_defer_suspend(0)
    if ev is not None:
        CONV_TIMER.end(ev)
    return gw_r, gw_i, gb_r, gb_i


WGRAD_DEFER = None


def wgrad_defer_begin():
    global WGRAD_DEFER
    check(_lib.load().dcs_wgrad_defer_begin(), 'dcs_wgrad_defer_begin')
    WGRAD_DEFER = []


def wgrad_defer_flush(partial=False):
    global WGRAD_DEFER
    ev = CONV_TIMER.begin(0.0) if CONV_TIMER is not None else None
    try:
        check(_lib.load().dcs_wgrad_defer_flush(cur_stream()), 'dcs_wgrad_defer_flush')
    finally:
        if not partial:
            WGRAD_DEFER = None
    if partial:
        check(_lib.load().dcs_wgrad_defer_begin(), 'dcs_wgrad_defer_begin')
    if ev is not None:
        CONV_TIMER.end(ev)



def cbn(x, weight, bias, running_mean, running_covar, eps=1e-5, momentum=0.1, use_batch_stats=True,
        act=ACT_NONE, drop_p=0.0, seed=0, out=None, coef_cached=None, stat=None):
    _chk(x, 'x', 5, act=True)
    for n, t in (('weight', weight), ('bias', bias), ('running_mean', running_mean), ('running_covar', running_covar)):
        _chk(t, n)
    B, H, W, C, _ = x.shape
    P = B * H * W
    y = torch.empty_like(x) if out is None else out
    lib = _lib.load()
    if stat is not None and use_batch_stats:
        part, rows, pivot = stat
        _chk(part, 'stat part', 3)
        _chk(pivot, 'stat pivot', 2)
        if part.shape[2] < rows or tuple(part.shape[:2]) != (C, 5) or tuple(pivot.shape) != (C, 2):
            raise _lib.DcsHipError(f'cbn: statistics slabs {tuple(part.shape)} / pivot {tuple(pivot.shape)} do not match C={C}')
        stats = torch.empty((C, 8), dtype=torch.float32, device=x.device)
        coef = torch.empty((C, 6), dtype=torch.float32, device=x.device)
        check(_sym('dcs_cbn_fwd_slabs', x, y)(ptr(x), ptr(y), ptr(weight), ptr(bias), ptr(running_mean), ptr(running_covar), ptr(stats),
                                    ptr(coef), ptr(part), int(rows), int(part.shape[2]), ptr(pivot), P, C, eps,
                                    -1.0 if momentum is None else momentum, act, float(drop_p), int(seed), ptr(SEED_STATE),
                                    cur_stream()), 'dcs_cbn_fwd_slabs')
        return y, stats, coef
    nbytes = lib.dcs_cbn_workspace_bytes(P, C)
    if nbytes < 0:
        raise _lib.DcsHipError(f'cbn: unsupported channel count C={C}')
    ws = _workspace(nbytes, x.device)
    mode = int(bool(use_batch_stats))
    if coef_cached is not None:
        if mode != 0:
            raise _lib.DcsHipError('cbn: cached coefficients are an eval-mode feature')
        stats, coef = coef_cached
        mode = 2
    else:
        stats = torch.empty((C, 8), dtype=torch.float32, device=x.device)
        coef = torch.empty((C, 6), dtype=torch.float32, device=x.device)
    check(_sym('dcs_cbn_fwd', x, y)(ptr(x), ptr(y), ptr(weight), ptr(bias), ptr(running_mean), ptr(running_covar),
                          ptr(stats), ptr(coef), ptr(ws), ws.numel(), P, C, eps,
                          -1.0 if momentum is None else momentum, mode, act,
                          float(drop_p), int(seed), ptr(SEED_STATE), cur_stream()), 'dcs_cbn_fwd')
    return y, stats, coef


def cbn_channel_attention(x, weight, bias, running_mean, running_covar, eps, momentum, act, stat, w1, w2):
    _chk(x, 'x', 5, act=True)
    for n, t in (('weight', weight), ('bias', bias), ('running_mean', running_mean), ('running_covar', running_covar),
                 ('w1', w1), ('w2', w2)):
        _chk(t, n)
    part, rows, pivot = stat
    B, H, W, C, _ = x.shape
    HW = H * W
    Ch = w1.shape[-2]
    lib = _lib.load()
    nch = lib.dcs_ca_pool_chunks(HW, C)
    if nch < 1 or part.shape[2] < rows or tuple(part.shape[:2]) != (C, 5) or tuple(pivot.shape) != (C, 2):
        raise _lib.DcsHipError(f'cbn_channel_attention: unsupported C={C} or mismatching statistics slabs {tuple(part.shape)}')
    dev = x.device
    a = torch.empty_like(x)
    new = lambda *sh: torch.empty(sh, dtype=torch.float32, device=dev)
    stats, coef, ca, pooled, hidden = new(C, 8), new(C, 6), new(B, C, 2), new(B, C, 2), new(B, Ch, 2)
    nbytes = B * nch * C * 2 * 8
    ws = _workspace(nbytes, dev)
    check(_sym('dcs_cbn_fwd_slabs_pool', x, a)(ptr(x), ptr(a), ptr(weight), ptr(bias), ptr(running_mean), ptr(running_covar),
                                              ptr(stats), ptr(coef), ptr(part), int(rows), int(part.shape[2]), ptr(pivot),
                                              ptr(ws), ws.numel(), B, HW, C, eps, -1.0 if momentum is None else momentum, act,
                                              cur_stream()), 'dcs_cbn_fwd_slabs_pool')
    check(lib.dcs_channel_attention_fc_fwd(ptr(ws), ptr(w1), ptr(w2), ptr(ca), ptr(pooled), ptr(hidden), B, HW, C, Ch,
                                           cur_stream()), 'dcs_channel_attention_fc_fwd')
    return a, stats, coef, ca, pooled, hidden


def cbn_bwd(x, g_out, weight, stats, coef, use_batch_stats, act, drop_p=0.0, seed=0, affine=True, outs=None,
            g_add=None, g_out2=None, need_gx=True):
    _chk(x, 'x', 5, act=True)
    _chk(g_out, 'g_out', 5, act=True)
    _chk(g_out2, 'g_out2', 5, act=True)
    if g_out2 is not None and g_out2.shape != g_out.shape:
        raise _lib.DcsHipError(f'cbn_bwd: g_out {tuple(g_out.shape)} vs g_out2 {tuple(g_out2.shape)}')
    B, H, W, C, _ = x.shape
    P = B * H * W
    g_x = torch.empty_like(x) if need_gx else None
    o = outs or (None, None)
    g_w = (o[0] if o[0] is not None else torch.empty((C, 3), dtype=torch.float32, device=x.device)) if affine else None
    g_b = (o[1] if o[1] is not None else torch.empty((C, 2), dtype=torch.float32, device=x.device)) if affine else None
    lib = _lib.load()
    nbytes = lib.dcs_cbn_bwd_workspace_bytes(P, C)
    if nbytes < 0:
        raise _lib.DcsHipError(f'cbn_bwd: unsupported channel count C={C}')
    ws = _workspace(nbytes, x.device)
    if g_add is not None:
        _chk(g_add, 'g_add', 3)
    check(_sym('dcs_cbn_bwd_add', x, g_out, g_out2)(ptr(x), ptr(g_out), ptr(g_x), ptr(weight), ptr(stats), ptr(coef), ptr(g_w), ptr(g_b),
                              ptr(ws), ws.numel(), P, C, int(bool(use_batch_stats)), act, float(drop_p), int(seed),
                              ptr(SEED_STATE), ptr(g_add), 1.0 / (H * W), H * W, ptr(g_out2), cur_stream()), 'dcs_cbn_bwd_add')
    return g_x, g_w, g_b


def channel_attention(x, w1, w2):
    _chk(x, 'x', 5, act=True)
    _chk(w1, 'w1')
    _chk(w2, 'w2')
    B, H, W, C, _ = x.shape
    Ch = w1.shape[-2]
    ca = torch.empty((B, C, 2), dtype=torch.float32, device=x.device)
    pooled = torch.empty((B, C, 2), dtype=torch.float32, device=x.device)
    hidden = torch.empty((B, Ch, 2), dtype=torch.float32, device=x.device)
    lib = _lib.load()
    nbytes = lib.dcs_ca_workspace_bytes(B, H * W, C)
    if nbytes < 0:
        raise _lib.DcsHipError(f'channel_attention: unsupported channel count C={C}')
    ws = _workspace(nbytes, x.device)
    check(_sym('dcs_channel_attention_fwd', x)(ptr(x), ptr(w1), ptr(w2), ptr(ca), ptr(pooled), ptr(hidden), ptr(ws),
                                        ws.numel(), B, H * W, C, Ch, cur_stream()), 'dcs_channel_attention_fwd')
    return ca, pooled, hidden


def spatial_pool(x, ca=None):
    _chk(x, 'x', 5, act=True)
    _chk(ca, 'ca', 3)
    B, H, W, C, _ = x.shape
    pooled = torch.empty((B, H, W, 2, 2), dtype=torch.float32, device=x.device)
    check(_sym('dcs_spatial_pool_fwd', x)(ptr(x), ptr(ca), ptr(pooled), B, H * W, C, cur_stream()),
          'dcs_spatial_pool_fwd')
    return pooled


def attention_apply(x, ca=None, sa=None, drop_p=0.0, seed=0, out=None):
    _chk(x, 'x', 5, act=True)
    _chk(ca, 'ca', 3)
    _chk(sa, 'sa')
    B, H, W, C, _ = x.shape
    y = torch.empty_like(x) if out is None else out
    check(_sym('dcs_attention_apply_fwd', x, y)(ptr(x), ptr(ca), ptr(sa), ptr(y), B, H * W, C, float(drop_p),
                                              int(seed), ptr(SEED_STATE), cur_stream()), 'dcs_attention_apply_fwd')
    return y


def attention_bwd(x, g_out, ca, sa, sp, pooled, hidden, w1, w2, wsa, ksize, drop_p=0.0, seed=0, outs=None,
                  split_pool=False, defer_fc=False):
    _chk(x, 'x', 5, act=True)
    _chk(g_out, 'g_out', 5, act=True)
    B, H, W, C, _ = x.shape
    HW = H * W
    Ch = hidden.shape[1]
    dev = x.device
    lib = _lib.load()
    g_pre = torch.empty((B, H, W, 1, 2), dtype=torch.float32, device=dev)
    check(_sym('dcs_attention_bwd_sa', x, g_out)(ptr(x), ptr(g_out), ptr(ca), ptr(sa), ptr(g_pre), B, HW, C, float(drop_p),
                                   int(seed), ptr(SEED_STATE), cur_stream()), 'dcs_attention_bwd_sa')
    k, pad = (ksize, ksize), (ksize // 2, ksize // 2)
    g_sp, _ = cconv2d_bwd_data(g_pre, pack_conv_weight_bwd(wsa, k, (1, 1), pad), (H, W, 2), k, (1, 1), pad)
    o = outs or (None,) * 6
    g_c1r, g_c1i, _, _ = cconv2d_bwd_weight(sp, None, g_pre, (1, 2, ksize, ksize), False, k, (1, 1), pad,
                                            outs=(o[4], o[5], None, None))
    g_x = torch.empty_like(x)
    new = lambda shape: torch.empty(shape, dtype=torch.float32, device=dev)
    g0r = o[0] if o[0] is not None else new((Ch, C, 1, 1))
    g0i = o[1] if o[1] is not None else new((Ch, C, 1, 1))
    g2r = o[2] if o[2] is not None else new((C, Ch, 1, 1))
    g2i = o[3] if o[3] is not None else new((C, Ch, 1, 1))
    nbytes = lib.dcs_attention_bwd_workspace_bytes(B, HW, C, Ch)
    if nbytes < 0:
        raise _lib.DcsHipError(f'attention_bwd: unsupported channel count C={C}')
    defer_fc = bool(defer_fc and split_pool)
    ws = torch.empty(nbytes, dtype=torch.uint8, device=dev) if defer_fc else _workspace(nbytes, dev)
    g_pooled = new((B, C, 2)) if split_pool else None
    fcp = (None,) * 4 if defer_fc else (g0r, g0i, g2r, g2i)
    check(_sym('dcs_attention_bwd_x', x, g_out)(ptr(x), ptr(g_out), ptr(ca), ptr(sa), ptr(g_sp), ptr(pooled), ptr(hidden), ptr(w1),
                                  ptr(w2), ptr(g_x), ptr(fcp[0]), ptr(fcp[1]), ptr(fcp[2]), ptr(fcp[3]), ptr(g_pooled), ptr(ws),
                                  ws.numel(), B, HW, C, Ch, float(drop_p), int(seed), ptr(SEED_STATE), cur_stream()),
          'dcs_attention_bwd_x')
    if defer_fc:
        return g_x, g0r, g0i, g2r, g2i, g_c1r, g_c1i, g_pooled, (ws, pooled, hidden, g0r, g0i, g2r, g2i, B, HW, C, Ch)
    if split_pool:
        return g_x, g0r, g0i, g2r, g2i, g_c1r, g_c1i, g_pooled
    return g_x, g0r, g0i, g2r, g2i, g_c1r, g_c1i


def attention_bwd_fc_weights(job):
    ws, pooled, hidden, g0r, g0i, g2r, g2i, B, HW, C, Ch = job
    check(_lib.load().dcs_attention_bwd_fc_weights(ptr(ws), ws.numel(), ptr(pooled), ptr(hidden), ptr(g0r), ptr(g0i), ptr(g2r),
                                                   ptr(g2i), B, HW, C, Ch, cur_stream()), 'dcs_attention_bwd_fc_weights')


ATTENTION_BATCH_MAX = 8


def _attention_items(blocks):
    items = (_lib.AttentionItem * len(blocks))()
    for it, blk in zip(items, blocks):
        for k, v in blk.items():
            setattr(it, k, v if isinstance(v, int) else ptr(v))
    return items


def attention_blocks_fwd(xs, w1s, w2s, wsas, biases):
    lib = _lib.load()
    B, dev = xs[0].shape[0], xs[0].device
    new = lambda *shape: torch.empty(shape, dtype=torch.float32, device=dev)
    blocks, outs = [], []
    for x, w1, w2, wsa, bias in zip(xs, w1s, w2s, wsas, biases):
        _chk(x, 'x', 5, act=True)
        _, H, W, C, _ = x.shape
        Ch = w1.shape[-2]
        o = dict(y=torch.empty_like(x), ca=new(B, C, 2), pooled=new(B, C, 2), hidden=new(B, Ch, 2), sp=new(B, H, W, 2, 2),
                 sa=new(B, H, W, 1, 2))
        blocks.append(dict(x=x, w1=w1, w2=w2, wsa=wsa, sa_bias=bias, H=H, W=W, C=C, Ch=Ch, **o))
        outs.append(o)
    items = _attention_items(blocks)
    n = len(blocks)
    nbytes = lib.dcs_attention_fwd_batched_workspace_bytes(n, items, B)
    if nbytes < 0:
        raise _lib.DcsHipError('attention_blocks_fwd: unsupported block geometry')
    ws = _workspace(nbytes, dev)
    check(_sym('dcs_attention_fwd_batched', *xs)(n, items, ptr(ws), ws.numel(), B, cur_stream()), 'dcs_attention_fwd_batched')
    return outs


def attention_blocks_bwd(saved, g_outs, wsa_bwds, fc_outs, split_pool=None):
    lib = _lib.load()
    B, dev = g_outs[0].shape[0], g_outs[0].device
    blocks, res = [], []
    split_pool = split_pool or (False,) * len(saved)
    for (sv, g, wb, fo), split in zip(zip(saved, g_outs, wsa_bwds, fc_outs), split_pool):
        _chk(g, 'g_out', 5, act=True)
        x = sv['x']
        _, H, W, C, _ = x.shape
        g_pre = torch.empty((B, H, W, 1, 2), dtype=torch.float32, device=dev)
        g_sp = torch.empty((B, H, W, 2, 2), dtype=torch.float32, device=dev)
        g_x = torch.empty_like(x)
        g_pooled = torch.empty((B, C, 2), dtype=torch.float32, device=dev) if split else None
        blocks.append(dict(x=x, w1=sv['w1'], w2=sv['w2'], ca=sv['ca'], pooled=sv['pooled'], hidden=sv['hidden'], sa=sv['sa'],
                           g_out=g, wsa_bwd=wb, g_pre=g_pre, g_sp=g_sp, g_x=g_x, g_fc0_r=fo[0], g_fc0_i=fo[1], g_fc2_r=fo[2],
                           g_fc2_i=fo[3], H=H, W=W, C=C, Ch=sv['hidden'].shape[1], **({'g_pooled': g_pooled} if split else {})))
        res.append((g_x, g_pre, g_pooled))
    items = _attention_items(blocks)
    n = len(blocks)
    nbytes = lib.dcs_attention_bwd_batched_workspace_bytes(n, items, B)
    if nbytes < 0:
        raise _lib.DcsHipError('attention_blocks_bwd: unsupported block geometry')
    ws = _workspace(nbytes, dev)
    check(_sym('dcs_attention_bwd_batched', *g_outs, *[sv['x'] for sv in saved])(n, items, ptr(ws), ws.numel(), B, cur_stream()), 'dcs_attention_bwd_batched')
    return res


def lstm_layer(gx, w_hh, n_sets, seqs_per_set, S, strides, save=False, save_hprev=False, bias=None):
    _chk(gx, 'gx')
    _chk(w_hh, 'w_hh', 4)
    H = w_hh.shape[-1]
    NS = n_sets * seqs_per_set
    out = torch.empty((NS, S, 2 * H), dtype=torch.float32, device=gx.device)
    gates = torch.empty((NS, S, 2, 4 * H), dtype=torch.float32, device=gx.device) if save else None
    c = torch.empty((NS, S, 2, H), dtype=torch.float32, device=gx.device) if save else None
    hprev = torch.empty((NS, S, 2, H), dtype=torch.float32, device=gx.device) if save and save_hprev else None
    ba, bb = (None, None) if bias is None else bias
    _chk(ba, 'bias_a')
    _chk(bb, 'bias_b')
    check(_lib.load().dcs_lstm_layer_fwd_bias(ptr(gx), ptr(w_hh), ptr(ba), ptr(bb), ptr(out), ptr(gates), ptr(c), ptr(hprev),
                                              n_sets, seqs_per_set, S, H, strides[0], strides[1], strides[2], cur_stream()),
          'dcs_lstm_layer_fwd_bias')
    return (out, gates, c, hprev) if save_hprev else (out, gates, c)


def lstm_layer_bwd(g_out, gates, c, w_hh, n_sets, seqs_per_set, S, bias_part=False):
    _chk(g_out, 'g_out', 3)
    _chk(gates, 'gates', 4)
    _chk(c, 'c', 4)
    _chk(w_hh, 'w_hh', 4)
    g_pre = torch.empty_like(gates)
    part = torch.empty((gates.shape[0], 2, gates.shape[-1]), dtype=torch.float32, device=gates.device) if bias_part else None
    check(_lib.load().dcs_lstm_layer_bwd(ptr(g_out), ptr(gates), ptr(c), ptr(w_hh), ptr(g_pre), ptr(part), n_sets,
                                         seqs_per_set, S, w_hh.shape[-1], cur_stream()), 'dcs_lstm_layer_bwd')
    return (g_pre, part) if bias_part else g_pre


def dropout(x, drop_p, seed, out=None):
    _chk(x, 'x')
    y = torch.empty_like(x) if out is None else out
    check(_lib.load().dcs_dropout_fwd(ptr(x), ptr(y), x.numel(), float(drop_p), int(seed), ptr(SEED_STATE), cur_stream()),
          'dcs_dropout_fwd')
    return y


def complex_act(x, act, out=None):
    _chk(x, 'x')
    y = torch.empty_like(x) if out is None else out
    check(_lib.load().dcs_complex_act_fwd(ptr(x), ptr(y), x.numel(), act, cur_stream()), 'dcs_complex_act_fwd')
    return y


def complex_upsample(x, up):
    _chk(x, 'x', 5)
    B, H, W, C, _ = x.shape
    y = torch.empty((B, H * up[0], W * up[1], C, 2), dtype=torch.float32, device=x.device)
    check(_lib.load().dcs_complex_upsample_fwd(ptr(x), ptr(y), B, H, W, C, up[0], up[1], cur_stream()),
          'dcs_complex_upsample_fwd')
    return y


def tapsum(z, ksize, up, pad, backward=False, grad=None, bias=None, bias_grad=None, out_dtype=torch.float32):
    lib = _lib.load()
    if not backward:
        _chk(z, 'z', 5)
        B, Hs, Ws, CT, _ = z.shape
        y = torch.empty((B, Hs * up[0], Ws * up[1], 1, 2), dtype=torch.float32, device=z.device)
        b_r, b_i = bias if bias is not None else (None, None)
        check(lib.dcs_tapsum_fwd(ptr(z), ptr(y), ptr(b_r), ptr(b_i), B, Hs, Ws, CT, ksize[0], ksize[1], up[0], up[1],
                                 pad[0], pad[1], cur_stream()), 'dcs_tapsum_fwd')
        return y
    _chk(grad, 'grad', 5)
    B, Hs, Ws, CT, _ = z
    gz = torch.empty((B, Hs, Ws, CT, 2), dtype=out_dtype, device=grad.device)
    gb_r, gb_i = bias_grad if bias_grad is not None else (None, None)
    ws = _workspace(lib.dcs_tapsum_bwd_workspace_bytes(), grad.device) if gb_r is not None else None
    check(_sym('dcs_tapsum_bwd', gz)(ptr(grad), ptr(gz), ptr(gb_r), ptr(gb_i), ptr(ws), 0 if ws is None else ws.numel(), B, Hs, Ws, CT,
                             ksize[0], ksize[1], up[0], up[1], pad[0], pad[1], cur_stream()), 'dcs_tapsum_bwd')
    return gz


def cconv_up2_single(x1, x2, wt, b_r, b_i):
    _chk(x1, 'x1', 5, act=True)
    _chk(x2, 'x2', 5, act=True)
    _chk(wt, 'wt', 4)
    B, Hs, Ws, C1, _ = x1.shape
    C2 = 0 if x2 is None else x2.shape[3]
    y = torch.empty((B, 2 * Hs, 2 * Ws, 1, 2), dtype=torch.float32, device=x1.device)
    check(_sym('dcs_cconv_up2_single_fwd', x1, x2)(ptr(x1), ptr(x2), ptr(wt), ptr(b_r), ptr(b_i), ptr(y), B, Hs, Ws, C1, C2,
                                               wt.shape[2], cur_stream()), 'dcs_cconv_up2_single_fwd')
    return y


def cconv_up2_single_bwd_data(gy, wt, C1, C2, out_dtype=torch.float32):
    _chk(gy, 'gy', 5)
    _chk(wt, 'wt', 4)
    B, Ho, Wo = gy.shape[:3]
    Hs, Ws = Ho // 2, Wo // 2
    gx1 = torch.empty((B, Hs, Ws, C1, 2), dtype=out_dtype, device=gy.device)
    gx2 = torch.empty((B, Hs, Ws, C2, 2), dtype=out_dtype, device=gy.device) if C2 else None
    ev = (CONV_TIMER.begin(8.0 * B * Hs * Ws * 16 * (C1 + C2), emulated=True,
                           nbytes=gy.numel() * 4.0 + B * Hs * Ws * (C1 + C2) * 2.0 * gx1.element_size())
          if CONV_TIMER is not None else None)
    check(_sym('dcs_cconv_up2_single_bwd_data', gx1, gx2)(ptr(gy), ptr(wt), ptr(gx1), ptr(gx2), B, Hs, Ws, C1, C2, wt.shape[2],
                                                          cur_stream()), 'dcs_cconv_up2_single_bwd_data')
    if ev is not None:
        CONV_TIMER.end(ev)
    return gx1, gx2


def cconv_up2_single_bwd_weight(gy, x1, x2, w_shape, outs=None, bias_outs=None):
    _chk(gy, 'gy', 5)
    _chk(x1, 'x1', 5, act=True)
    _chk(x2, 'x2', 5, act=True)
    B, Hs, Ws, C1, _ = x1.shape
    C2 = 0 if x2 is None else x2.shape[3]
    acc = outs is not None and outs[0] is not None and outs[1] is not None
    g_r = outs[0] if acc else torch.empty(w_shape, dtype=torch.float32, device=gy.device)
    g_i = outs[1] if acc else torch.empty(w_shape, dtype=torch.float32, device=gy.device)
    gb_r, gb_i = bias_outs if bias_outs is not None else (None, None)
    lib = _lib.load()
    ws = _workspace(lib.dcs_cconv_up2_single_bwd_weight_workspace_bytes(), gy.device)
    ev = (CONV_TIMER.begin(8.0 * B * Hs * Ws * 16 * (C1 + C2), emulated=True,
                           nbytes=gy.numel() * 4.0 + B * Hs * Ws * (C1 + C2) * 2.0 * x1.element_size())
          if CONV_TIMER is not None else None)
    check(_sym('dcs_cconv_up2_single_bwd_weight', x1, x2)(ptr(gy), ptr(x1), ptr(x2), ptr(g_r), ptr(g_i), ptr(gb_r), ptr(gb_i), int(acc),
                                                            ptr(ws), ws.numel(), B, Hs, Ws, C1, C2, cur_stream()),
          'dcs_cconv_up2_single_bwd_weight')
    if ev is not None:
        CONV_TIMER.end(ev)
    return g_r, g_i


def bound_crm(M, eps=10e-7, out=None):
    _chk(M, 'M')
    y = torch.empty_like(M) if out is None else out
    check(_lib.load().dcs_bound_crm_fwd(ptr(M), ptr(y), M.numel() // 2, eps, cur_stream()), 'dcs_bound_crm_fwd')
    return y


def bound_mask_apply(Y, M_in, eps=10e-7):
    _chk(Y, 'Y')
    _chk(M_in, 'M_in')
    if Y.shape != M_in.shape:
        raise _lib.DcsHipError(f'bound_mask_apply: Y {tuple(Y.shape)} vs M {tuple(M_in.shape)}')
    M, N, S = torch.empty_like(Y), torch.empty_like(Y), torch.empty_like(Y)
    check(_lib.load().dcs_bound_mask_apply_fwd(ptr(Y), ptr(M_in), ptr(M), ptr(N), ptr(S), Y.numel() // 2, eps,
                                               cur_stream()), 'dcs_bound_mask_apply_fwd')
    return M, N, S


def bound_mask_apply_pair(Y, M_in, eps=10e-7):
    _chk(Y, 'Y')
    _chk(M_in, 'M_in')
    if Y.shape != M_in.shape:
        raise _lib.DcsHipError(f'bound_mask_apply: Y {tuple(Y.shape)} vs M {tuple(M_in.shape)}')
    M = torch.empty_like(Y)
    NS = torch.empty((2,) + tuple(Y.shape), dtype=Y.dtype, device=Y.device)
    check(_lib.load().dcs_bound_mask_apply_fwd(ptr(Y), ptr(M_in), ptr(M), ptr(NS[0]), ptr(NS[1]), Y.numel() // 2, eps,
                                               cur_stream()), 'dcs_bound_mask_apply_fwd')
    return M, NS


def bound2_mask_apply(Y, D_raw, eps=10e-7, pair=False, keep_m1=False, drop_p=0.0, seed=0):
    _chk(Y, 'Y')
    _chk(D_raw, 'D_raw')
    if Y.shape != D_raw.shape:
        raise _lib.DcsHipError(f'bound2_mask_apply: Y {tuple(Y.shape)} vs D {tuple(D_raw.shape)}')
    M = torch.empty_like(Y)
    M1 = torch.empty_like(Y) if keep_m1 else None
    if pair:
        NS = torch.empty((2,) + tuple(Y.shape), dtype=Y.dtype, device=Y.device)
        N, S = NS[0], NS[1]
    else:
        N, S = torch.empty_like(Y), torch.empty_like(Y)
    check(_lib.load().dcs_bound2_mask_apply_fwd(ptr(Y), ptr(D_raw), ptr(M1), ptr(M), ptr(N), ptr(S), Y.numel() // 2, eps,
                                                float(drop_p), int(seed), ptr(SEED_STATE), cur_stream()),
          'dcs_bound2_mask_apply_fwd')
    return (M1, M, NS) if pair else (M1, M, N, S)


def bound2_mask_apply_bwd(Y, D_raw, g_M1, g_M, g_N, g_S, eps=10e-7, drop_p=0.0, seed=0):
    _chk(D_raw, 'D_raw')
    for n, t in (('Y', Y), ('g_M1', g_M1), ('g_M', g_M), ('g_N', g_N), ('g_S', g_S)):
        _chk(t, n)
    g = torch.empty_like(D_raw)
    check(_lib.load().dcs_bound2_mask_apply_bwd(ptr(Y), ptr(D_raw), ptr(g_M1), ptr(g_M), ptr(g_N), ptr(g_S), ptr(g),
                                                D_raw.numel() // 2, eps, float(drop_p), int(seed), ptr(SEED_STATE),
                                                cur_stream()), 'dcs_bound2_mask_apply_bwd')
    return g


def bound_mask_apply_bwd(Y, M_in, g_M, g_N, g_S, eps=10e-7):
    _chk(M_in, 'M_in')
    for n, t in (('Y', Y), ('g_M', g_M), ('g_N', g_N), ('g_S', g_S)):
        _chk(t, n)
    g = torch.empty_like(M_in)
    check(_lib.load().dcs_bound_mask_apply_bwd(ptr(Y), ptr(M_in), ptr(g_M), ptr(g_N), ptr(g_S), ptr(g),
                                               M_in.numel() // 2, eps, cur_stream()), 'dcs_bound_mask_apply_bwd')
    return g


def bound2_apply_polar_frames(Y, D_raw, Fp, eps=10e-7, drop_p=0.0, seed=0, want_mask=False, grad=None, g_M=None, hermitian=False):
    _chk(Y, 'Y', 4)
    _chk(D_raw, 'D_raw', 4)
    if Y.shape != D_raw.shape:
        raise _lib.DcsHipError(f'bound2_apply_polar_frames: Y {tuple(Y.shape)} vs D {tuple(D_raw.shape)}')
    B, F, T, _ = Y.shape
    lib = _lib.load()
    if grad is None:
        out = torch.empty((2 * B, T, Fp, 2), dtype=torch.float32, device=Y.device)
        M = torch.empty_like(Y) if want_mask else None
        check(lib.dcs_bound2_apply_polar_frames_fwd(ptr(Y), ptr(D_raw), ptr(M), ptr(out), B, F, Fp, T, eps, float(drop_p), int(seed),
                                                    ptr(SEED_STATE), cur_stream()), 'dcs_bound2_apply_polar_frames_fwd')
        return M, out
    _chk(grad, 'grad', 4)
    _chk(g_M, 'g_M', 4)
    if tuple(grad.shape) != (2 * B, T, Fp, 2):
        raise _lib.DcsHipError(f'bound2_apply_polar_frames: grad {tuple(grad.shape)} for B={B}, T={T}, Fp={Fp}')
    g = torch.empty_like(D_raw)
    check(lib.dcs_bound2_apply_polar_frames_bwd(ptr(Y), ptr(D_raw), ptr(grad), ptr(g_M), ptr(g), B, F, Fp, T, eps, int(bool(hermitian)),
                                                float(drop_p), int(seed), ptr(SEED_STATE), cur_stream()),
          'dcs_bound2_apply_polar_frames_bwd')
    return g


def complex_abs(Y):
    if Y.is_complex():
        if not Y.is_cuda:
            raise _lib.DcsHipError('complex_abs: expected a CUDA (HIP) tensor; the HIP path has no CPU fallback')
        if Y.dtype != torch.complex64:
            raise _lib.DcsHipError(f'complex_abs: expected complex64, got {Y.dtype}')
        Y = torch.view_as_real(Y.contiguous())
    _chk(Y, 'Y')
    if Y.dim() < 1 or Y.shape[-1] != 2 or Y.numel() == 0:
        raise _lib.DcsHipError(f'complex_abs: expected (re, im) pairs, got shape {tuple(Y.shape)}')
    out = torch.empty(Y.shape[:-1], dtype=torch.float32, device=Y.device)
    check(_lib.load().dcs_complex_abs_f32(ptr(Y), ptr(out), out.numel(), cur_stream()), 'dcs_complex_abs_f32')
    return out


def rmask_apply_polar_frames(Y, D, Fp, eps=10e-7, pair=True, want_mask=False, grad=None, g_M=None, hermitian=False):
    _chk(Y, 'Y', 4)
    _chk(D, 'D', 3)
    if tuple(Y.shape) != tuple(D.shape) + (2,):
        raise _lib.DcsHipError(f'rmask_apply_polar_frames: Y {tuple(Y.shape)} vs D {tuple(D.shape)}')
    B, F, T, _ = Y.shape
    rows = 2 * B if pair else B
    lib = _lib.load()
    if grad is None:
        out = torch.empty((rows, T, Fp, 2), dtype=torch.float32, device=Y.device)
        M = torch.empty_like(D) if want_mask else None
        check(lib.dcs_rmask_apply_polar_frames_fwd(ptr(Y), ptr(D), ptr(M), ptr(out), B, F, Fp, T, eps, int(bool(pair)), cur_stream()),
              'dcs_rmask_apply_polar_frames_fwd')
        return M, out
    _chk(grad, 'grad', 4)
    _chk(g_M, 'g_M', 3)
    if tuple(grad.shape) != (rows, T, Fp, 2) or (g_M is not None and g_M.shape != D.shape):
        raise _lib.DcsHipError(f'rmask_apply_polar_frames: grad {tuple(grad.shape)} for B={B}, T={T}, Fp={Fp}, pair={bool(pair)}')
    g = torch.empty_like(D)
    check(lib.dcs_rmask_apply_polar_frames_bwd(ptr(Y), ptr(D), ptr(grad), ptr(g_M), ptr(g), B, F, Fp, T, eps, int(bool(hermitian)),
                                               int(bool(pair)), cur_stream()), 'dcs_rmask_apply_polar_frames_bwd')
    return g


def polar_frames(z, Fp, eps=10e-7, grad=None, hermitian=False):
    _chk(z, 'z', 4)
    B, F, T, _ = z.shape
    lib = _lib.load()
    if grad is None:
        out = torch.empty((B, T, Fp, 2), dtype=torch.float32, device=z.device)
        check(lib.dcs_polar_frames_fwd(ptr(z), ptr(out), B, F, Fp, T, eps, cur_stream()), 'dcs_polar_frames_fwd')
        return out
    _chk(grad, 'grad', 4)
    gz = torch.empty_like(z)
    check(lib.dcs_polar_frames_bwd(ptr(z), ptr(grad), ptr(gz), B, F, Fp, T, eps, int(bool(hermitian)), cur_stream()),
          'dcs_polar_frames_bwd')
    return gz


# ... 499 lines not shown
```

include/dcsnet_hip.h:

```cpp
#ifndef DCSNET_HIP_H
#define DCSNET_HIP_H

#ifdef __cplusplus
extern "C" {
#endif

typedef void* dcs_stream_t;

#define DCS_OK              0
#define DCS_ERR_BADARG     (-1)
#define DCS_ERR_LAUNCH     (-2)
#define DCS_ERR_WORKSPACE  (-3)

#define DCS_ACT_NONE   0
#define DCS_ACT_RELU   1
#define DCS_ACT_LRELU  2
#define DCS_ACT_SIGMOID 3

int         dcs_abi_version(void);
const char* dcs_error_string(int code);

long dcs_packed_weight_floats(int Cout, int Cin, int kh, int kw, int up_f, int up_t);
int dcs_pack_conv_weight(const float* w_r, const float* w_i, const float* b_r, const float* b_i,
                         float* wp, float* bias_out,
                         int Cout, int Cin, int kh, int kw, int transposed, int up_f, int up_t,
                         dcs_stream_t stream);

long dcs_cconv2d_fwd_workspace_bytes(int B, int Hin, int Win, int C1, int C2, int up_f, int up_t,
                                     int Cout, int kh, int kw, int sf, int st, int pad_f, int pad_t);
int dcs_cconv2d_fwd(const float* x1, const float* x2, const float* wp, const float* bias, float* y,
                    void* workspace, long workspace_bytes,
                    int B, int Hin, int Win, int C1, int C2, int up_f, int up_t,
                    int Cout, int kh, int kw, int sf, int st, int pad_f, int pad_t, int act,
                    dcs_stream_t stream);

int dcs_cconv2d_fwd_stats_rows(int B, int Hin, int Win, int C1, int C2, int up_f, int up_t,
                               int Cout, int kh, int kw, int sf, int st, int pad_f, int pad_t);
int dcs_cconv2d_fwd_stats(const float* x1, const float* x2, const float* wp, const float* bias, float* y,
                          float* stat, int stat_rows, int* rows_used, void* workspace, long workspace_bytes,
                          int B, int Hin, int Win, int C1, int C2, int up_f, int up_t,
                          int Cout, int kh, int kw, int sf, int st, int pad_f, int pad_t, dcs_stream_t stream);

int dcs_cconv2d_fwd_affine(const float* x1, const float* x2, const float* wp, const float* bias, const float* coef, float* y,
                           void* workspace, long workspace_bytes,
                           int B, int Hin, int Win, int C1, int C2, int up_f, int up_t,
                           int Cout, int kh, int kw, int sf, int st, int pad_f, int pad_t, int act,
                           dcs_stream_t stream);

long dcs_rconv2d_fwd_workspace_bytes(int B, int Hin, int Win, int C1r, int C2r, int up_f, int up_t, int Coutr,
                                     int kh, int kw, int sf, int st, int pad_f, int pad_t);
int dcs_rconv2d_fwd(const float* x1, const float* x2, const float* bm, const float* bias, float* y,
                    void* workspace, long workspace_bytes,
                    int B, int Hin, int Win, int C1r, int C2r, int up_f, int up_t,
                    int Coutr, int kh, int kw, int sf, int st, int pad_f, int pad_t, int act,
                    dcs_stream_t stream);
long dcs_rconv2d_bwd_data_workspace_bytes(int B, int Hv, int Wv, int Cinr, int Coutr, int kh, int kw, int sf, int st,
                                          int pad_f, int pad_t);
int dcs_rconv2d_bwd_data(const float* gy, const float* bm_bwd, float* gxv, void* workspace, long workspace_bytes,
                         int B, int Hv, int Wv, int Cinr, int Coutr, int kh, int kw, int sf, int st, int pad_f, int pad_t,
                         dcs_stream_t stream);

int dcs_rbn_fwd(const float* x, float* y, const float* weight, const float* bias, float* running_mean, float* running_var,
                float* stats_out, float* coef_out, void* workspace, long workspace_bytes, long P, int Cr, float eps,
                float momentum, int use_batch_stats, int act, dcs_stream_t stream);
int dcs_rbn_bwd(const float* x, const float* g_out, float* g_x, const float* stats, const float* coef, float* g_weight,
                float* g_bias, void* workspace, long workspace_bytes, long P, int Cr, int use_batch_stats, int act,
                dcs_stream_t stream);

long dcs_packed_weight_bwd_floats(int Cout, int Cin, int kh, int kw, int sf, int st, int pad_f, int pad_t,
                                  int up_f, int up_t);
int  dcs_pack_conv_weight_bwd(const float* wp, float* wp_bwd, int Cout, int Cin, int kh, int kw,
                              int sf, int st, int pad_f, int pad_t, int up_f, int up_t, dcs_stream_t stream);
long dcs_cconv2d_bwd_data_workspace_bytes(int B, int Hin, int Win, int C1, int C2, int up_f, int up_t,
                                          int Cout, int kh, int kw, int sf, int st, int pad_f, int pad_t);
int  dcs_cconv2d_bwd_data(const float* gy, const float* wp_bwd, float* gx1, float* gx2,
                          void* workspace, long workspace_bytes,
                          int B, int Hin, int Win, int C1, int C2, int up_f, int up_t,
                          int Cout, int kh, int kw, int sf, int st, int pad_f, int pad_t, dcs_stream_t stream);
int  dcs_upsample_cat_bwd(const float* gxv, float* gx1, float* gx2, int B, int Hin, int Win, int C1, int C2,
                          int up_f, int up_t, dcs_stream_t stream);
long dcs_cconv2d_bwd_weight_workspace_bytes(int B, int Hin, int Win, int C1, int C2, int up_f, int up_t,
                                            int Cout, int kh, int kw, int sf, int st, int pad_f, int pad_t);
int  dcs_cconv2d_bwd_weight(const float* x1, const float* x2, const float* gy,
                            float* gw_r, float* gw_i, float* gb_r, float* gb_i,
                            void* workspace, long workspace_bytes,
                            int B, int Hin, int Win, int C1, int C2, int up_f, int up_t,
                            int Cout, int kh, int kw, int sf, int st, int pad_f, int pad_t, int transposed,
                            dcs_stream_t stream);

long dcs_cbn_workspace_bytes(long P, int C);
int  dcs_cbn_fwd(const float* x, float* y, const float* weight, const float* bias,
                 float* running_mean, float* running_covar,
                 float* stats_out, float* coef_out, void* workspace, long workspace_bytes,
                 long P, int C, float eps, float momentum, int use_batch_stats, int act,
                 float drop_p, unsigned long long seed, const unsigned long long* seed_dev, dcs_stream_t stream);

int  dcs_cbn_fwd_slabs(const float* x, float* y, const float* weight, const float* bias,
                       float* running_mean, float* running_covar, float* stats_out, float* coef_out,
                       const float* part, int rows, int stride, const float* pivot,
                       long P, int C, float eps, float momentum, int act,
                       float drop_p, unsigned long long seed, const unsigned long long* seed_dev, dcs_stream_t stream);

int dcs_ca_pool_chunks(long HW, int C);
int dcs_cbn_fwd_slabs_pool(const float* x, float* y, const float* weight, const float* bias,
                           float* running_mean, float* running_covar, float* stats_out, float* coef_out,
                           const float* part, int rows, int stride, const float* pivot, void* pool_part, long pool_bytes,
                           int B, long HW, int C, float eps, float momentum, int act, dcs_stream_t stream);
int dcs_channel_attention_fc_fwd(const void* pool_part, const float* w1, const float* w2, float* ca_out, float* pooled_out,
                                 float* hidden_out, int B, long HW, int C, int Ch, dcs_stream_t stream);

long dcs_cbn_bwd_workspace_bytes(long P, int C);
int  dcs_cbn_bwd(const float* x, const float* g_out, float* g_x, const float* weight,
                 const float* stats, const float* coef, float* g_weight, float* g_bias,
                 void* workspace, long workspace_bytes, long P, int C, int use_batch_stats, int act,
                 float drop_p, unsigned long long seed, const unsigned long long* seed_dev, dcs_stream_t stream);
int  dcs_cbn_bwd_add(const float* x, const float* g_out, float* g_x, const float* weight, const float* stats,
                     const float* coef, float* g_weight, float* g_bias, void* workspace, long workspace_bytes,
                     long P, int C, int use_batch_stats, int act, float drop_p, unsigned long long seed,
                     const unsigned long long* seed_dev, const float* g_add, float add_scale, long HW,
                     const float* g_out2, dcs_stream_t stream);

long dcs_ca_workspace_bytes(int B, long HW, int C);
int  dcs_channel_attention_fwd(const float* x, const float* w1, const float* w2,
                               float* ca_out, float* pooled_out, float* hidden_out,
                               void* workspace, long workspace_bytes,
                               int B, long HW, int C, int Ch, dcs_stream_t stream);

int dcs_spatial_pool_fwd(const float* x, const float* ca, float* pooled,
                         int B, long HW, int C, dcs_stream_t stream);

int dcs_attention_apply_fwd(const float* x, const float* ca, const float* sa, float* y,
                            int B, long HW, int C, float drop_p, unsigned long long seed,
                            const unsigned long long* seed_dev, dcs_stream_t stream);

typedef struct {
    const float* x; const float* w1; const float* w2; const float* wsa; const float* sa_bias;
    float* ca; float* pooled; float* hidden; float* sp; float* sa; float* y;
    const float* g_out; const float* wsa_bwd; float* g_pre; float* g_sp; float* g_x;
    float* g_fc0_r; float* g_fc0_i; float* g_fc2_r; float* g_fc2_i;
    int H, W, C, Ch;
    float* g_pooled;
} dcs_attention_item;
long dcs_attention_fwd_batched_workspace_bytes(int n, const dcs_attention_item* items, int B);
int dcs_attention_fwd_batched(int n, const dcs_attention_item* items, void* workspace, long workspace_bytes, int B,
                              dcs_stream_t stream);
long dcs_attention_bwd_batched_workspace_bytes(int n, const dcs_attention_item* items, int B);
int dcs_attention_bwd_batched(int n, const dcs_attention_item* items, void* workspace, long workspace_bytes, int B,
                              dcs_stream_t stream);

long dcs_rattention_workspace_bytes(int B, long HW, int C);
int  dcs_rattention_fwd(const float* x, const float* w1, const float* w2, const float* wsa, const float* sa_bias,
                        float* ca_out, float* y, void* workspace, long workspace_bytes,
                        int B, int H, int W, int C, int Ch, int ksize, dcs_stream_t stream);

long dcs_rattention_train_workspace_bytes(int B, long HW, int C, int Ch);
int  dcs_rattention_pool_fwd(const float* x, const float* w1, const float* w2, float* ca_out, float* mx_out, float* hid_out,
                             float* pooled, void* workspace, long workspace_bytes, int B, int H, int W, int C, int Ch,
                             dcs_stream_t stream);
int  dcs_rattention_apply_fwd(const float* x, const float* ca, const float* sa, float* y, int B, int H, int W, int C,
                              dcs_stream_t stream);
int  dcs_rattention_apply_bwd(const float* gy, const float* x, const float* ca, const float* sa, float* gx, float* g_sa,
                              float* g_ca, void* workspace, long workspace_bytes, int B, int H, int W, int C,
                              dcs_stream_t stream);
int  dcs_rattention_pool_bwd(const float* g_pooled, const float* g_ca, const float* x, const float* ca, const float* mx,
                             const float* hid, const float* w1, const float* w2, float* gx, float* gw1, float* gw2,
                             int accumulate, void* workspace, long workspace_bytes, int B, int H, int W, int C, int Ch,
                             dcs_stream_t stream);

int  dcs_attention_bwd_sa(const float* x, const float* g_out, const float* ca, const float* sa, float* g_pre,
                          int B, long HW, int C, float drop_p, unsigned long long seed, const unsigned long long* seed_dev, dcs_stream_t stream);
long dcs_attention_bwd_workspace_bytes(int B, long HW, int C, int Ch);
int  dcs_attention_bwd_x(const float* x, const float* g_out, const float* ca, const float* sa, const float* g_sp,
                         const float* pooled, const float* hidden, const float* w1, const float* w2,
                         float* g_x, float* g_fc0_r, float* g_fc0_i, float* g_fc2_r, float* g_fc2_i, float* g_pooled,
                         void* workspace, long workspace_bytes, int B, long HW, int C, int Ch,
                         float drop_p, unsigned long long seed, const unsigned long long* seed_dev, dcs_stream_t stream);
int dcs_attention_bwd_fc_weights(const void* workspace, long workspace_bytes, const float* pooled, const float* hidden,
                                 float* g_fc0_r, float* g_fc0_i, float* g_fc2_r, float* g_fc2_i, int B, long HW, int C, int Ch,
                                 dcs_stream_t stream);

int dcs_lstm_layer_fwd(const float* gx, const float* w_hh, float* out, float* gates_save, float* c_save,
                       float* hprev_save, int n_sets, int seqs_per_set, int S, int H, long stride_set, long stride_n, long stride_t,
                       dcs_stream_t stream);

int dcs_lstm_layer_fwd_bias(const float* gx, const float* w_hh, const float* bias_a, const float* bias_b, float* out,
                            float* gates_save, float* c_save, float* hprev_save, int n_sets, int seqs_per_set, int S,
                            int Hdim, long stride_set, long stride_n, long stride_t, dcs_stream_t stream);
int dcs_lstm_layer_bwd(const float* g_out, const float* gates, const float* c_save, const float* w_hh,
                       float* g_pre, float* g_bias_part, int n_sets, int seqs_per_set, int S, int H, dcs_stream_t stream);

int dcs_lstm_whh_grad(const float* g_pre, const float* h_prev, float* part, int NT, int CK, int H, dcs_stream_t stream);
int dcs_atb_chunks(const float* A, const float* B, float* part, long a_lo, long a_hi, long b_lo, long b_hi, int nlo, int nhi,
                   int lda, int ldb, int M, int N, int R, int CK, dcs_stream_t stream);
int dcs_chunk_sum_acc(const float* part, float* out, long o_lo, long o_hi, int nlo, int nhi, int CK, long MN,
                      dcs_stream_t stream);
int dcs_atb_chunks_strided(const float* A, const float* B, float* part, long a_lo, long a_hi, long b_lo, long b_hi, int nlo,
                           int nhi, int lda, int ldb, int b_es, int M, int N, int R, int CK, dcs_stream_t stream);
int dcs_gemm_f32(const float* A, const float* B, float* C, int M, int N, int K, int lda, int ldb, int ldc, int b_transposed,
                 int nseg, long a_seg, long b_seg, int nbatch, long a_batch, long b_batch, long c_batch, int a_planes,
                 int c_planes, dcs_stream_t stream);
int dcs_lstm_combine_fwd(const float* o, float* out, long n, dcs_stream_t stream);
int dcs_lstm_combine_bwd(const float* g, float* g_o, long n, dcs_stream_t stream);
int dcs_lstm_param_grads(const float* part, const float* b_part, float* g_whh, float* g_bih, float* g_bhh, int CK,
                         int seqs_per_set, int H, dcs_stream_t stream);
int dcs_lstm_param_grads_ih(const float* part, const float* b_part, float* g_whh, float* g_bih, float* g_bhh, int CK,
                            int seqs_per_set, int H, const float* part_ih, float* g_wih, int CK_ih, long MN_ih, int nsets,
                            dcs_stream_t stream);

int dcs_dropout_fwd(const float* x, float* y, long n, float drop_p, unsigned long long seed,
                    const unsigned long long* seed_dev, dcs_stream_t stream);

int dcs_complex_act_fwd(const float* x, float* y, long n_floats, int act, dcs_stream_t stream);
int dcs_complex_upsample_fwd(const float* x, float* y, int B, int H, int W, int C, int up_f, int up_t,
                             dcs_stream_t stream);

int dcs_tapsum_fwd(const float* z, float* y, const float* b_r, const float* b_i, int B, int Hs, int Ws, int CT,
                   int kh, int kw, int up_f, int up_t, int pad_f, int pad_t, dcs_stream_t stream);
long dcs_tapsum_bwd_workspace_bytes(void);
int dcs_tapsum_bwd(const float* gy, float* gz, float* gb_r, float* gb_i, void* workspace, long workspace_bytes,
                   int B, int Hs, int Ws, int CT, int kh, int kw, int up_f, int up_t, int pad_f, int pad_t,
                   dcs_stream_t stream);

int dcs_cconv_up2_single_fwd(const float* x1, const float* x2, const float* wt, const float* b_r, const float* b_i,
                             float* y, int B, int Hs, int Ws, int C1, int C2, int ct, dcs_stream_t stream);

int dcs_cconv_up2_single_bwd_data(const float* gy, const float* wt, float* gx1, float* gx2, int B, int Hs, int Ws, int C1, int C2,
                                  int ct, dcs_stream_t stream);
long dcs_cconv_up2_single_bwd_weight_workspace_bytes(void);
int dcs_cconv_up2_single_bwd_weight(const float* gy, const float* x1, const float* x2, float* gw_r, float* gw_i, float* gb_r,
                                    float* gb_i, int accumulate, void* workspace, long workspace_bytes, int B, int Hs, int Ws,
                                    int C1, int C2, dcs_stream_t stream);

int dcs_bound_crm_fwd(const float* M_raw, float* M_out, long n, float eps, dcs_stream_t stream);

int dcs_bound_mask_apply_fwd(const float* Y, const float* M_in, float* M_out, float* N_hat, float* S_hat,
                             long n, float eps, dcs_stream_t stream);

int dcs_bound_mask_apply_bwd(const float* Y, const float* M_in, const float* g_M, const float* g_N,
                             const float* g_S, float* g_Min, long n, float eps, dcs_stream_t stream);

int dcs_bound2_mask_apply_fwd(const float* Y, const float* D_raw, float* M1_out, float* M_out, float* N_hat, float* S_hat,
                              long n, float eps, float drop_p, unsigned long long seed, const unsigned long long* seed_dev,
                              dcs_stream_t stream);
int dcs_bound2_mask_apply_bwd(const float* Y, const float* D_raw, const float* g_M1, const float* g_M, const float* g_N,
                              const float* g_S, float* g_D, long n, float eps, float drop_p, unsigned long long seed,
                              const unsigned long long* seed_dev, dcs_stream_t stream);

int dcs_bound2_apply_polar_frames_fwd(const float* Y, const float* D_raw, float* M_out, float* out, int B, int F, int Fp, int T,
                                      float eps, float drop_p, unsigned long long seed, const unsigned long long* seed_dev,
                                      dcs_stream_t stream);
int dcs_bound2_apply_polar_frames_bwd(const float* Y, const float* D_raw, const float* g_out, const float* g_M, float* g_D,
                                      int B, int F, int Fp, int T, float eps, int hermitian, float drop_p,
                                      unsigned long long seed, const unsigned long long* seed_dev, dcs_stream_t stream);

int dcs_complex_abs_f32(const float* Y, float* out, long n, dcs_stream_t stream);
int dcs_rmask_apply_polar_frames_fwd(const float* Y, const float* D, float* M_out, float* out, int B, int F, int Fp, int T,
                                     float eps, int pair, dcs_stream_t stream);
int dcs_rmask_apply_polar_frames_bwd(const float* Y, const float* D, const float* g_out, const float* g_M, float* g_D,
                                     int B, int F, int Fp, int T, float eps, int hermitian, int pair, dcs_stream_t stream);

int dcs_irfft512_frames(const float* X, float* y, long frames, dcs_stream_t stream);
int dcs_rfft512_frames(const float* g, float* G, long frames, dcs_stream_t stream);
int dcs_rfft512_ola_frames(const float* g_y, const float* window, const float* inv_env, float* G, int B, int T, int hop,
                           float scale, dcs_stream_t stream);
int dcs_irfft512_ola_frames(const float* X, const float* window, const float* inv_env, float* y, int B, int T, int hop,
                            float scale, dcs_stream_t stream);
int dcs_polar_frames_fwd(const float* z, float* out, int B, int F, int Fp, int T, float eps, dcs_stream_t stream);
int dcs_polar_frames_bwd(const float* z, const float* g_out, float* g_z, int B, int F, int Fp, int T, float eps,
                         int hermitian, dcs_stream_t stream);
int dcs_istft_envelope(const float* window, float* inv_env, int T, int n_fft, int hop, dcs_stream_t stream);
int dcs_istft_ola_fwd(const float* frames, const float* window, const float* inv_env, float* y, int B, int T,
                      int n_fft, int hop, float scale, dcs_stream_t stream);
int dcs_istft_ola_bwd(const float* g_y, const float* window, const float* inv_env, float* g_frames, int B, int T,
                      int n_fft, int hop, float scale, dcs_stream_t stream);

int dcs_sisnr_fwd(const float* clean, const float* est, float* snr, float* coef, int B, int L, float eps,
                  dcs_stream_t stream);
int dcs_sisnr_bwd(const float* clean, const float* est, const float* coef, const float* g, float scale, float* g_est,
                  int B, int L, dcs_stream_t stream);

int dcs_sisnr_losses_fwd(const float* snr_speech, const float* snr_noise, float* out3, int B, float alpha,
                         dcs_stream_t stream);
int dcs_sisnr_losses_guard_fwd(const float* snr_speech, const float* snr_noise, float* out3, int B, float alpha,
                               float* skip, dcs_stream_t stream);
int dcs_sisnr_pair_bwd(const float* target, const float* est, const float* coef, const float* g_noise,
                       const float* g_speech, const float* g_total, float alpha, float* g_est, int B, int L,
                       dcs_stream_t stream);

int dcs_stft_frames_fwd(const float* clean, const float* noisy, const float* window, float* frames, int B, int L, int T,
                        int n_fft, int hop, dcs_stream_t stream);
int dcs_stft_bins_fwd(const float* spec, float* out, int SB, int T, int F, float scale, dcs_stream_t stream);

int dcs_crm_fwd(const float* S, const float* Y, float* M, long n, float eps, dcs_stream_t stream);

int dcs_adam_amsgrad_step(float* p, const float* g, float* m, float* v, float* vmax,
                          const float* grad_norm, float max_norm, float grad_scale, long n,
                          const float* lr, float beta1, float beta2, float eps, float weight_decay, int step,
                          const int* step_dev, const float* skip, dcs_stream_t stream);
int dcs_grad_sumsq_parts(const float* g, long n, double* parts, int n_parts, const float* skip, int* step_dev, long long* seed_dev,
                         long long* counters, int n_counters, dcs_stream_t stream);
int dcs_adam_amsgrad_step_sumsq(float* p, const float* g, float* m, float* v, float* vmax, const double* sumsq_parts, int n_parts,
                                float max_norm, float grad_scale, long n, const float* lr, float beta1, float beta2, float eps,
                                float weight_decay, int step, const int* step_dev, const float* skip, dcs_stream_t stream);

int dcs_swa_average_f32(float* avg, const float* p, long n, long n_averaged, dcs_stream_t stream);

int dcs_step_guard(const float* loss, float* skip, dcs_stream_t stream);
int dcs_stream_hold(const int* host_flag, int timeout_ms, dcs_stream_t stream);
int dcs_kernel_timer_begin(int slot);
int dcs_kernel_timer_end(void);
int dcs_kernel_timer_read(int slot, float* ms);
int dcs_step_advance(const float* skip, int* step_dev, long long* seed_dev, dcs_stream_t stream);
int dcs_step_advance_counters(const float* skip, int* step_dev, long long* seed_dev, long long* counters, int n_counters,
                              dcs_stream_t stream);

int dcs_pack_tap_rows(const float* w_r, const float* w_i, float* wp, float* bias_out, int Cin, int kh, int kw, int ct,
                      dcs_stream_t stream);
int dcs_tap_rows_wgrad_scatter(const float* gt_r, const float* gt_i, float* gw_r, float* gw_i, int Cin, int kh, int kw,
                               int accumulate, dcs_stream_t stream);

int dcs_set_conv_precision(int mode);
int dcs_get_conv_precision(void);

int dcs_wgrad_defer_begin(void);
int dcs_wgrad_defer_suspend(int suspended);
int dcs_wgrad_defer_flush(dcs_stream_t stream);

int dcs_pack_plan_begin(void);
int dcs_pack_plan_end(void** plan_out);
int dcs_pack_plan_jobs(const void* plan, int* n_jobs, int* n_launches);
int dcs_pack_plan_run(const void* plan, dcs_stream_t stream);
int dcs_pack_plan_destroy(void* plan);

int dcs_resample_poly_f32(const float* x, float* y, int rows, long L, const float* h, int taps, int up, int down,
                          dcs_stream_t stream);
long dcs_stoi_workspace_bytes(int B, long L10);
int dcs_stoi_f32(const float* clean10, const float* est10, int B, long L10, const int* band_lo, const int* band_hi,
                 float* out_d, int* out_kept, void* workspace, long workspace_bytes, dcs_stream_t stream);

int dcs_resample_sinc_f32(const float* x, const long* x_off, float* y, const long* y_off, int rows, long total_out,
                          const float* taps, int orig, int new_, int width, dcs_stream_t stream);
int dcs_audio_stft_batch_f32(const float* clean, const float* noisy, const long* offsets, int n_items, const int* item_index,
                             const int* item_start, int B, const float* window, int n_fft, int T, int hop, float scale,
                             float* out_noise, float* out_noisy, float* out_clean, dcs_stream_t stream);

int dcs_audio_stft_segments_f32(const float* noisy, const long* offsets, int n_items, const int* seg_item,
                                const int* seg_first_frame, int S, const float* window, int n_fft, int T, int overlap, int hop,
                                float scale, float* out, dcs_stream_t stream);
int dcs_segments_stitch_f32(const float* seg, long seg_rows, const int* seg_first, const long* offsets, int n_items,
                            long total_out, int T, int overlap, int hop, float* y, short* pcm, dcs_stream_t stream);

typedef unsigned short dcs_bf16_t;
int dcs_cconv2d_fwd_h(const dcs_bf16_t* x1, const dcs_bf16_t* x2, const float* wp, const float* bias, dcs_bf16_t* y,
                      void* workspace, long workspace_bytes,
                      int B, int Hin, int Win, int C1, int C2, int up_f, int up_t,
                      int Cout, int kh, int kw, int sf, int st, int pad_f, int pad_t, int act, dcs_stream_t stream);
int dcs_cconv2d_fwd_affine_h(const dcs_bf16_t* x1, const dcs_bf16_t* x2, const float* wp, const float* bias, const float* coef,
                             dcs_bf16_t* y, void* workspace, long workspace_bytes,
                             int B, int Hin, int Win, int C1, int C2, int up_f, int up_t,
                             int Cout, int kh, int kw, int sf, int st, int pad_f, int pad_t, int act, dcs_stream_t stream);
int dcs_cconv2d_fwd_stats_h(const dcs_bf16_t* x1, const dcs_bf16_t* x2, const float* wp, const float* bias, dcs_bf16_t* y,
                            float* stat, int stat_rows, int* rows_used, void* workspace, long workspace_bytes,
                            int B, int Hin, int Win, int C1, int C2, int up_f, int up_t,
                            int Cout, int kh, int kw, int sf, int st, int pad_f, int pad_t, dcs_stream_t stream);
int dcs_cconv2d_bwd_data_h(const dcs_bf16_t* gy, const float* wp_bwd, dcs_bf16_t* gx1, dcs_bf16_t* gx2,
                           void* workspace, long workspace_bytes,
                           int B, int Hin, int Win, int C1, int C2, int up_f, int up_t,
                           int Cout, int kh, int kw, int sf, int st, int pad_f, int pad_t, dcs_stream_t stream);
int dcs_cconv2d_bwd_weight_h(const dcs_bf16_t* x1, const dcs_bf16_t* x2, const dcs_bf16_t* gy,
                             float* gw_r, float* gw_i, float* gb_r, float* gb_i, void* workspace, long workspace_bytes,
                             int B, int Hin, int Win, int C1, int C2, int up_f, int up_t,
                             int Cout, int kh, int kw, int sf, int st, int pad_f, int pad_t, int transposed,
                             dcs_stream_t stream);
int dcs_cconv_up2_single_fwd_h(const dcs_bf16_t* x1, const dcs_bf16_t* x2, const float* wt, const float* b_r, const float* b_i,
                               float* y, int B, int Hs, int Ws, int C1, int C2, int ct, dcs_stream_t stream);
int dcs_cconv_up2_single_bwd_data_h(const float* gy, const float* wt, dcs_bf16_t* gx1, dcs_bf16_t* gx2, int B, int Hs, int Ws, int C1,
                                    int C2, int ct, dcs_stream_t stream);
int dcs_cconv_up2_single_bwd_weight_h(const float* gy, const dcs_bf16_t* x1, const dcs_bf16_t* x2, float* gw_r, float* gw_i,
                                      float* gb_r, float* gb_i, int accumulate, void* workspace, long workspace_bytes, int B, int Hs,
                                      int Ws, int C1, int C2, dcs_stream_t stream);
int dcs_tapsum_bwd_h(const float* gy, dcs_bf16_t* gz, float* gb_r, float* gb_i, void* workspace, long workspace_bytes,
                     int B, int Hs, int Ws, int CT, int kh, int kw, int up_f, int up_t, int pad_f, int pad_t,
                     dcs_stream_t stream);
int dcs_cbn_fwd_h(const dcs_bf16_t* x, dcs_bf16_t* y, const float* weight, const float* bias,
                  float* running_mean, float* running_covar, float* stats_out, float* coef_out,
                  void* workspace, long workspace_bytes, long P, int C, float eps, float momentum, int use_batch_stats,
                  int act, float drop_p, unsigned long long seed, const unsigned long long* seed_dev, dcs_stream_t stream);
int dcs_cbn_fwd_slabs_h(const dcs_bf16_t* x, dcs_bf16_t* y, const float* weight, const float* bias,
                        float* running_mean, float* running_covar, float* stats_out, float* coef_out,
                        const float* part, int rows, int stride, const float* pivot,
                        long P, int C, float eps, float momentum, int act,
                        float drop_p, unsigned long long seed, const unsigned long long* seed_dev, dcs_stream_t stream);
int dcs_cbn_fwd_slabs_pool_h(const dcs_bf16_t* x, dcs_bf16_t* y, const float* weight, const float* bias,
                             float* running_mean, float* running_covar, float* stats_out, float* coef_out,
                             const float* part, int rows, int stride, const float* pivot, void* pool_part, long pool_bytes,
                             int B, long HW, int C, float eps, float momentum, int act, dcs_stream_t stream);
int dcs_cbn_bwd_h(const dcs_bf16_t* x, const dcs_bf16_t* g_out, dcs_bf16_t* g_x, const float* weight,
                  const float* stats, const float* coef, float* g_weight, float* g_bias,
                  void* workspace, long workspace_bytes, long P, int C, int use_batch_stats, int act,
                  float drop_p, unsigned long long seed, const unsigned long long* seed_dev, dcs_stream_t stream);
int dcs_cbn_bwd_add_h(const dcs_bf16_t* x, const dcs_bf16_t* g_out, dcs_bf16_t* g_x, const float* weight, const float* stats,
                      const float* coef, float* g_weight, float* g_bias, void* workspace, long workspace_bytes,
                      long P, int C, int use_batch_stats, int act, float drop_p, unsigned long long seed,
                      const unsigned long long* seed_dev, const float* g_add, float add_scale, long HW,
                      const dcs_bf16_t* g_out2, dcs_stream_t stream);
int dcs_channel_attention_fwd_h(const dcs_bf16_t* x, const float* w1, const float* w2,
                                float* ca_out, float* pooled_out, float* hidden_out,
                                void* workspace, long workspace_bytes, int B, long HW, int C, int Ch, dcs_stream_t stream);
int dcs_spatial_pool_fwd_h(const dcs_bf16_t* x, const float* ca, float* pooled, int B, long HW, int C, dcs_stream_t stream);
int dcs_attention_apply_fwd_h(const dcs_bf16_t* x, const float* ca, const float* sa, dcs_bf16_t* y,
                              int B, long HW, int C, float drop_p, unsigned long long seed,
                              const unsigned long long* seed_dev, dcs_stream_t stream);
int dcs_attention_fwd_batched_h(int n, const dcs_attention_item* items, void* workspace, long workspace_bytes, int B,
                                dcs_stream_t stream);
int dcs_attention_bwd_sa_h(const dcs_bf16_t* x, const dcs_bf16_t* g_out, const float* ca, const float* sa, float* g_pre,
                           int B, long HW, int C, float drop_p, unsigned long long seed, const unsigned long long* seed_dev,
                           dcs_stream_t stream);
int dcs_attention_bwd_x_h(const dcs_bf16_t* x, const dcs_bf16_t* g_out, const float* ca, const float* sa, const float* g_sp,
                          const float* pooled, const float* hidden, const float* w1, const float* w2,
                          dcs_bf16_t* g_x, float* g_fc0_r, float* g_fc0_i, float* g_fc2_r, float* g_fc2_i, float* g_pooled,
                          void* workspace, long workspace_bytes, int B, long HW, int C, int Ch,
                          float drop_p, unsigned long long seed, const unsigned long long* seed_dev, dcs_stream_t stream);
int dcs_attention_bwd_batched_h(int n, const dcs_attention_item* items, void* workspace, long workspace_bytes, int B,
                                dcs_stream_t stream);

#ifdef __cplusplus
}
#endif
#endif
```

Baseline: 2.572 million.

## Fuse channel-attention FC into spatial pool and 7x7 spatial conv into apply

```diff
diff --git a/dcs-net_amd/csrc/attention.hip b/dcs-net_amd/csrc/attention.hip
--- a/dcs-net_amd/csrc/attention.hip
+++ b/dcs-net_amd/csrc/attention.hip
@@ -36,85 +36,244 @@
     }
 }
 
+struct CaFcLds { float2 pooled[128]; float2 hid[64]; double red[kThreads * 2]; };
+
+__device__ __forceinline__ void ca_fc_slab_sum(CaFcLds& l, const double* __restrict__ part, int nchunks,
+                                               float2* __restrict__ pooled_out, long HW, int C, int b, bool write) {
+    const int t = threadIdx.x;
+    const int nsl = kThreads / C, c = t % C, sl = t / C;
+    double sr = 0, si = 0;
+    if (sl < nsl)
+#pragma unroll 8
+        for (int k = sl; k < nchunks; k += nsl) {
+            const double* p = part + (((long)b * nchunks + k) * C + c) * 2;
+            sr += p[0]; si += p[1];
+        }
+    l.red[t * 2] = sr; l.red[t * 2 + 1] = si;
+    __syncthreads();
+    if (t < C) {
+        for (int q = 1; q < nsl; ++q) { sr += l.red[(q * C + t) * 2]; si += l.red[(q * C + t) * 2 + 1]; }
+        const float2 m = make_float2((float)(sr / (double)HW), (float)(si / (double)HW));
+        l.pooled[t] = m;
+        if (write) pooled_out[(long)b * C + t] = m;
+    }
+}
+
+__device__ __forceinline__ void ca_fc_mlp(CaFcLds& l, const float2* __restrict__ w1, const float2* __restrict__ w2,
+                                          float2* __restrict__ ca_out, float2* __restrict__ hidden_out, int C, int Ch, int b,
+                                          bool write, float2* ca_s) {
+    const int t = threadIdx.x;
+    for (int h = t >> 5; h < Ch; h += kThreads / 32) {
+        float ar = 0.f, ai = 0.f;
+#pragma unroll 4
+        for (int c = t & 31; c < C; c += 32) {
+            const float2 w = w1[c * Ch + h], p = l.pooled[c];
+            ar = fmaf(w.x, p.x, ar); ar = fmaf(-w.y, p.y, ar);
+            ai = fmaf(w.x, p.y, ai); ai = fmaf(w.y, p.x, ai);
+        }
+#pragma unroll
+        for (int o = 16; o > 0; o >>= 1) { ar += __shfl_xor(ar, o, 64); ai += __shfl_xor(ai, o, 64); }
+        if ((t & 31) == 0) {
+            if (write) hidden_out[(long)b * Ch + h] = make_float2(ar, ai);
+            l.hid[h] = make_float2(ar > 0.f ? ar : 0.f, ai > 0.f ? ai : 0.f);
+        }
+    }
+    __syncthreads();
+    for (int c = t; c < C; c += kThreads) {
+        float ar = 0.f, ai = 0.f;
+#pragma unroll 8
+        for (int h = 0; h < Ch; ++h) {
+            const float2 w = w2[h * C + c], p = l.hid[h];
+            ar = fmaf(w.x, p.x, ar); ar = fmaf(-w.y, p.y, ar);
+            ai = fmaf(w.x, p.y, ai); ai = fmaf(w.y, p.x, ai);
+        }
+        ar += ar; ai += ai;
+        const float2 v = make_float2(1.f / (1.f + expf(-ar)), 1.f / (1.f + expf(-ai)));
+        if (write) ca_out[(long)b * C + c] = v;
+        if (ca_s) ca_s[c] = v;
+    }
+}
+
 __device__ __forceinline__ void ca_fc_kernel_body(const double* __restrict__ part, int nchunks,
                                                           const float2* __restrict__ w1, const float2* __restrict__ w2,
                                                           float2* __restrict__ ca_out, float2* __restrict__ pooled_out,
                                                           float2* __restrict__ hidden_out, long HW, int C, int Ch, int bx, int by, int gx) {
-    __shared__ float2 pooled[128];
-    __shared__ float2 hid[64];
-    __shared__ double red[kThreads * 2];
-    const int b = bx, t = threadIdx.x;
-    {
-        const int nsl = kThreads / C, c = t % C, sl = t / C;
-        double sr = 0, si = 0;
-        if (sl < nsl)
-#pragma unroll 8
-            for (int k = sl; k < nchunks; k += nsl) {
-                const double* p = part + (((long)b * nchunks + k) * C + c) * 2;
-                sr += p[0]; si += p[1];
-            }
-        red[t * 2] = sr; red[t * 2 + 1] = si;
-        __syncthreads();
-        if (t < C) {
-            for (int q = 1; q < nsl; ++q) { sr += red[(q * C + t) * 2]; si += red[(q * C + t) * 2 + 1]; }
-            const float2 m = make_float2((float)(sr / (double)HW), (float)(si / (double)HW));
-            pooled[t] = m;
-            pooled_out[(long)b * C + t] = m;
-        }
-    }
-    __syncthreads();
-    for (int h = t >> 5; h < Ch; h += kThreads / 32) {
-        float ar = 0.f, ai = 0.f;
-#pragma unroll 4
-        for (int c = t & 31; c < C; c += 32) {
-            const float2 w = w1[c * Ch + h], p = pooled[c];
-            ar = fmaf(w.x, p.x, ar); ar = fmaf(-w.y, p.y, ar);
-            ai = fmaf(w.x, p.y, ai); ai = fmaf(w.y, p.x, ai);
-        }
-#pragma unroll
-        for (int o = 16; o > 0; o >>= 1) { ar += __shfl_xor(ar, o, 64); ai += __shfl_xor(ai, o, 64); }
-        if ((t & 31) == 0) {
-            hidden_out[(long)b * Ch + h] = make_float2(ar, ai);
-            hid[h] = make_float2(ar > 0.f ? ar : 0.f, ai > 0.f ? ai : 0.f);
-        }
-    }
-    __syncthreads();
-    for (int c = t; c < C; c += kThreads) {
-        float ar = 0.f, ai = 0.f;
-#pragma unroll 8
-        for (int h = 0; h < Ch; ++h) {
-            const float2 w = w2[h * C + c], p = hid[h];
-            ar = fmaf(w.x, p.x, ar); ar = fmaf(-w.y, p.y, ar);
-            ai = fmaf(w.x, p.y, ai); ai = fmaf(w.y, p.x, ai);
-        }
-        ar += ar; ai += ai;
-        ca_out[(long)b * C + c] = make_float2(1.f / (1.f + expf(-ar)), 1.f / (1.f + expf(-ai)));
-    }
+    __shared__ CaFcLds l;
+    ca_fc_slab_sum(l, part, nchunks, pooled_out, HW, C, bx, true);
+    __syncthreads();
+    ca_fc_mlp(l, w1, w2, ca_out, hidden_out, C, Ch, bx, true, nullptr);
 }
 
 __device__ __forceinline__ float group_sum(float v, int G) { return dcs_group_sum(v, G); }
 __device__ __forceinline__ float group_max(float v, int G) { return dcs_group_max(v, G); }
 
-__device__ __forceinline__ void spatial_pool_kernel_body(const act_t* __restrict__ x,
-                                                                 const float* __restrict__ ca,
-                                                                 float4* __restrict__ pooled, long HW, int C, int G, int bx, int by, int gx) {
+template <bool PRE>
+__device__ __forceinline__ void spatial_pool_stream(const ActIn4<act_t> x4, const float4 a, float4 v0, float4* __restrict__ pooled,
+                                                    long HW, int C, int G, int b, int bx, int gx) {
     const int t = threadIdx.x, g = t % G, r0 = t / G, rpi = kThreads / G;
-    const int b = by;
-    const ActIn4<act_t> x4 = act_in4(x) + (long)b * HW * G;
-    float4 a = make_float4(1.f, 0.f, 1.f, 0.f);
-    if (ca) a = reinterpret_cast<const float4*>(ca)[(long)b * G + g];
     const float invC = 1.f / (float)C;
     const long iters = (HW + (long)gx * rpi - 1) / ((long)gx * rpi);
     for (long k = 0; k < iters; ++k) {
         const long r = (k * gx + bx) * rpi + r0;
         const bool ok = r < HW;
         float4 v = make_float4(0.f, 0.f, 0.f, 0.f);
-        if (ok) v = x4[r * G + g];
+        if (PRE && k == 0) v = v0;
+        else if (ok) v = x4[r * G + g];
         const float z0r = a.x * v.x - a.y * v.y, z0i = a.x * v.y + a.y * v.x;
         const float z1r = a.z * v.z - a.w * v.w, z1i = a.z * v.w + a.w * v.z;
         const float sr = group_sum(z0r + z1r, G), si = group_sum(z0i + z1i, G);
         const float mr = group_max(fmaxf(z0r, z1r), G), mi = group_max(fmaxf(z0i, z1i), G);
         if (ok && g == 0) pooled[(long)b * HW + r] = make_float4(sr * invC, si * invC, mr, mi);
+    }
+}
+
+__device__ __forceinline__ void spatial_pool_kernel_body(const act_t* __restrict__ x,
+                                                                 const float* __restrict__ ca,
+                                                                 float4* __restrict__ pooled, long HW, int C, int G, int bx, int by, int gx) {
+    const int g = threadIdx.x % G;
+    const int b = by;
+    const ActIn4<act_t> x4 = act_in4(x) + (long)b * HW * G;
+    float4 a = make_float4(1.f, 0.f, 1.f, 0.f);
+    if (ca) a = reinterpret_cast<const float4*>(ca)[(long)b * G + g];
+    spatial_pool_stream<false>(x4, a, a, pooled, HW, C, G, b, bx, gx);
+}
+
+constexpr int kFcStage = 1024;
+__device__ __forceinline__ void spatial_pool_fc_kernel_body(const act_t* __restrict__ x, const double* __restrict__ part, int nchunks,
+                                                            const float2* __restrict__ w1, const float2* __restrict__ w2,
+                                                            float2* __restrict__ ca_out, float2* __restrict__ pooled_out,
+                                                            float2* __restrict__ hidden_out, float4* __restrict__ sp,
+                                                            long HW, int C, int Ch, int G, int bx, int by, int gx) {
+    __shared__ CaFcLds l;
+    __shared__ __attribute__((aligned(16))) float2 ca_s[128];
+    __shared__ float2 w_s[2 * kFcStage];
+    const int t = threadIdx.x, g = t % G, r0 = t / G, rpi = kThreads / G;
+    const int b = by, nw = C * Ch;
+    const bool stage = nw <= kFcStage, write = bx == 0;
+    float2 wr[2 * kFcStage / kThreads];
+    if (stage) {
+#pragma unroll
+        for (int j = 0; j < kFcStage / kThreads; ++j) {
+            const int i = t + kThreads * j < nw ? t + kThreads * j : nw - 1;
+            wr[2 * j] = w1[i]; wr[2 * j + 1] = w2[i];
+        }
+    }
+    const ActIn4<act_t> x4 = act_in4(x) + (long)b * HW * G;
+    const long rf = (long)bx * rpi + r0;
+    float4 v0 = make_float4(0.f, 0.f, 0.f, 0.f);
+    if (rf < HW) v0 = x4[rf * G + g];
+    ca_fc_slab_sum(l, part, nchunks, pooled_out, HW, C, b, write);
+    if (stage) {
+#pragma unroll
+        for (int j = 0; j < kFcStage / kThreads; ++j)
+            if (t + kThreads * j < nw) { w_s[t + kThreads * j] = wr[2 * j]; w_s[kFcStage + t + kThreads * j] = wr[2 * j + 1]; }
+    }
+    __syncthreads();
+    ca_fc_mlp(l, stage ? w_s : w1, stage ? w_s + kFcStage : w2, ca_out, hidden_out, C, Ch, b, write, ca_s);
+    __syncthreads();
+    const float4 a = reinterpret_cast<const float4*>(ca_s)[g];
+    spatial_pool_stream<true>(x4, a, v0, sp, HW, C, G, b, bx, gx);
+}
+
+constexpr int kSaK = 7, kSaPad = 3, kSaTaps = kSaK * kSaK * 2, kSaHalo = 704, kSaMaxTh = 32, kSaMaxTw = 32;
+constexpr int kSaNit = (kSaHalo + kThreads - 1) / kThreads;
+static_assert((kSaMaxTh + kSaK - 1) * (256 / kSaMaxTh + kSaK - 1) <= kSaHalo && (256 / kSaMaxTw + kSaK - 1) * (kSaMaxTw + kSaK - 1) <= kSaHalo &&
+              (16 + kSaK - 1) * (16 + kSaK - 1) <= kSaHalo, "haloed window of every tile shape fits");
+typedef float v2f __attribute__((ext_vector_type(2)));
+
+struct SaApplyP { const act_t* x; const float* ca; const float4* sp; const float2* w; const float2* bias; float2* sa; act_t* y;
+                  int H, W, C, G, th, twl, tiles_w, nx; };
+
+template <bool DROP>
+__device__ __forceinline__ void sa_apply_kernel_body(const SaApplyP& p, float drop_p, uint64_t seed, const uint64_t* __restrict__ seed_dev,
+                                                     int tl, int b) {
+    if (seed_dev) seed += seed_dev[0];
+    __shared__ __attribute__((aligned(16))) float2 tile[2][kSaHalo];
+    __shared__ __attribute__((aligned(16))) float4 wl[kSaTaps];
+    __shared__ float2 sa_t[kThreads];
+    const int t = threadIdx.x, G = p.G, g = t % G, r0 = t / G, rpi = kThreads / G;
+    const int th = p.th, tw = 1 << p.twl, npx = th << p.twl;
+    const int oy0 = (tl / p.tiles_w) * th, ox0 = (tl % p.tiles_w) * tw;
+    const int hw_ = tw + kSaK - 1, hn = (th + kSaK - 1) * hw_;
+    const long HW = (long)p.H * p.W, base = (long)b * HW * G;
+    const float2 wv = p.w[t < kSaTaps ? t : 0];
+    const float4* spb = p.sp + (long)b * HW;
+    float4 tv[kSaNit];
+#pragma unroll
+    for (int k = 0; k < kSaNit; ++k) {
+        const int i = t + kThreads * k < hn ? t + kThreads * k : hn - 1;
+        const int y = oy0 - kSaPad + i / hw_, x = ox0 - kSaPad + i % hw_;
+        const int yc = y < 0 ? 0 : (y >= p.H ? p.H - 1 : y), xc = x < 0 ? 0 : (x >= p.W ? p.W - 1 : x);
+        tv[k] = spb[(long)yc * p.W + xc];
+    }
+    const ActIn4<act_t> x4 = act_in4(p.x) + base;
+    const ActOut4<act_t> y4 = act_out4(p.y) + base;
+    const float4 a = reinterpret_cast<const float4*>(p.ca)[(long)b * G + g];
+    float4 v0 = make_float4(0.f, 0.f, 0.f, 0.f);
+    {
+        const int oy = oy0 + (r0 >> p.twl), ox = ox0 + (r0 & (tw - 1));
+        if (r0 < npx && oy < p.H && ox < p.W) v0 = x4[((long)oy * p.W + ox) * G + g];
+    }
+#pragma unroll
+    for (int k = 0; k < kSaNit; ++k) {
+        const int i = t + kThreads * k;
+        if (i < hn) {
+            const int y = oy0 - kSaPad + i / hw_, x = ox0 - kSaPad + i % hw_;
+            const bool in = y >= 0 && y < p.H && x >= 0 && x < p.W;
+            tile[0][i] = in ? make_float2(tv[k].x, tv[k].y) : make_float2(0.f, 0.f);
+            tile[1][i] = in ? make_float2(tv[k].z, tv[k].w) : make_float2(0.f, 0.f);
+        }
+    }
+    if (t < kSaTaps) wl[t] = make_float4(wv.x, wv.y, wv.y, wv.x);
+    __syncthreads();
+    if (t < npx) {
+        const int ty = t >> p.twl, tx = t & (tw - 1);
+        v2f accp = v2f{0.f, 0.f}, accq = v2f{0.f, 0.f};
+#pragma unroll
+        for (int ci = 0; ci < 2; ++ci) {
+#pragma unroll 1
+            for (int dy = 0; dy < kSaK; ++dy) {
+                const float2* row = &tile[ci][(ty + dy) * hw_ + tx];
+                v2f xv[kSaK];
+#pragma unroll
+                for (int dx = 0; dx < kSaK; ++dx) { const float2 v = row[dx]; xv[dx] = v2f{v.x, v.y}; }
+#pragma unroll
+                for (int dx = 0; dx < kSaK; ++dx) {
+                    const float4 w = wl[(dy * kSaK + dx) * 2 + ci];
+                    const v2f wx = v2f{w.x, w.x}, wy = v2f{w.z, w.z};
+                    accp = __builtin_elementwise_fma(wx, xv[dx], accp);
+                    accq = __builtin_elementwise_fma(wy, xv[dx], accq);
+                }
+            }
+        }
+        const v2f acc = v2f{accp.x - accq.y, accp.y + accq.x};
+        const float2 bv = p.bias ? p.bias[0] : make_float2(0.f, 0.f);
+        const float2 s = make_float2(dcs_act(acc.x + bv.x, DCS_ACT_SIGMOID), dcs_act(acc.y + bv.y, DCS_ACT_SIGMOID));
+        sa_t[t] = s;
+        const int oy = oy0 + ty, ox = ox0 + tx;
+        if (oy < p.H && ox < p.W) p.sa[(long)b * HW + (long)oy * p.W + ox] = s;
+    }
+    __syncthreads();
+    const float inv_keep = DROP ? 1.f / (1.f - drop_p) : 1.f;
+    for (int pi = r0; pi < npx; pi += rpi) {
+        const int oy = oy0 + (pi >> p.twl), ox = ox0 + (pi & (tw - 1));
+        if (oy >= p.H || ox >= p.W) continue;
+        const long r = (long)oy * p.W + ox;
+        const float4 v = pi == r0 ? v0 : x4[r * G + g];
+        const float2 s = sa_t[pi];
+        const float z0r = fmaf(a.x, v.x, -(a.y * v.y)), z0i = fmaf(a.x, v.y, a.y * v.x);
+        const float z1r = fmaf(a.z, v.z, -(a.w * v.w)), z1i = fmaf(a.z, v.w, a.w * v.z);
+        float4 o;
+        o.x = fmaf(s.x, z0r, -(s.y * z0i)); o.y = fmaf(s.x, z0i, s.y * z0r);
+        o.z = fmaf(s.x, z1r, -(s.y * z1i)); o.w = fmaf(s.x, z1i, s.y * z1r);
+        if (DROP) {
+            const uint64_t e = (uint64_t)(base + r * G + g) * 4;
+            o.x *= dcs_keep_scale(seed, e, drop_p, inv_keep);
+            o.y *= dcs_keep_scale(seed, e + 1, drop_p, inv_keep);
+            o.z *= dcs_keep_scale(seed, e + 2, drop_p, inv_keep);
+            o.w *= dcs_keep_scale(seed, e + 3, drop_p, inv_keep);
+        }
+        y4[r * G + g] = o;
     }
 }
 
@@ -200,6 +359,46 @@
     attention_apply_kernel_body<false>(p.x, p.ca, p.sa, p.y, p.HW, p.C, p.G, 0.f, 0, nullptr, blockIdx.x - t.x0[z], blockIdx.y, p.nx);
 }
 
+struct SpPoolFcP { const act_t* x; CaFcP f; float4* sp; int G, nx; };
+__global__ __launch_bounds__(kThreads) void spatial_pool_fc_kernel(SpPoolFcP p) {
+    spatial_pool_fc_kernel_body(p.x, p.f.part, p.f.nchunks, p.f.w1, p.f.w2, p.f.ca, p.f.pooled, p.f.hidden, p.sp, p.f.HW, p.f.C, p.f.Ch,
+                                p.G, blockIdx.x, blockIdx.y, gridDim.x);
+}
+__global__ __launch_bounds__(kThreads) void spatial_pool_fc_multi_kernel(Tbl<SpPoolFcP> t) {
+    const int z = tbl_find(t, blockIdx.x);
+    const SpPoolFcP& p = t.p[z];
+    spatial_pool_fc_kernel_body(p.x, p.f.part, p.f.nchunks, p.f.w1, p.f.w2, p.f.ca, p.f.pooled, p.f.hidden, p.sp, p.f.HW, p.f.C, p.f.Ch,
+                                p.G, blockIdx.x - t.x0[z], blockIdx.y, p.nx);
+}
+template <bool DROP>
+__global__ __launch_bounds__(kThreads) void attention_sa_apply_kernel(SaApplyP p, float drop_p, uint64_t seed, const uint64_t* seed_dev) {
+    sa_apply_kernel_body<DROP>(p, drop_p, seed, seed_dev, blockIdx.x, blockIdx.y);
+}
+__global__ __launch_bounds__(kThreads) void attention_sa_apply_multi_kernel(Tbl<SaApplyP> t) {
+    const int z = tbl_find(t, blockIdx.x);
+    sa_apply_kernel_body<false>(t.p[z], 0.f, 0, nullptr, blockIdx.x - t.x0[z], blockIdx.y);
+}
+
+inline int pow2_ceil(int v) { int p = 1; while (p < v) p <<= 1; return p; }
+inline void sa_tile(int B, int H, int W, int G, SaApplyP* p) {
+    const long HW = (long)H * W;
+    int T = 2 * (kThreads / G);
+    if (T > kThreads) T = kThreads;
+    while (T < kThreads && (long)B * ((HW + T - 1) / T) > 4096) T *= 2;
+    int tw = 1;
+    while (tw * tw < 2 * T) tw <<= 1;
+    if (tw > kSaMaxTw) tw = kSaMaxTw;
+    if (tw > pow2_ceil(W)) tw = pow2_ceil(W);
+    int th = T / tw;
+    if (th > pow2_ceil(H)) th = pow2_ceil(H);
+    if (th > kSaMaxTh) th = kSaMaxTh;
+    int twl = 0;
+    while ((1 << twl) < tw) ++twl;
+    p->H = H; p->W = W; p->G = G; p->th = th; p->twl = twl;
+    p->tiles_w = (W + tw - 1) / tw;
+    p->nx = p->tiles_w * ((H + th - 1) / th);
+}
+
 #ifndef DCS_ACT_BF16
 __global__ __launch_bounds__(kThreads) void dropout_kernel(const float* __restrict__ x, float* __restrict__ y, long n,
                                                             float drop_p, uint64_t seed, const uint64_t* __restrict__ seed_dev) {
@@ -298,6 +497,49 @@
     return DCS_OK;
 }
 
+extern "C" int DCS_SYM(dcs_spatial_pool_fc_fwd)(const act_t* x, void* part, long part_bytes, int pool_first, const float* w1,
+                                                const float* w2, float* ca_out, float* pooled_out, float* hidden_out, float* sp,
+                                                int B, long HW, int C, int Ch, dcs_stream_t stream) {
+    int G;
+    if (!x || !part || !w1 || !w2 || !ca_out || !pooled_out || !hidden_out || !sp) return DCS_ERR_BADARG;
+    if (B <= 0 || B > 65535 || HW <= 0 || !att_geom(C, &G) || Ch <= 0 || Ch > 64) return DCS_ERR_BADARG;
+    const int nch = ca_chunks(HW, G);
+    if (part_bytes < (long)B * nch * C * 2 * (long)sizeof(double)) return DCS_ERR_WORKSPACE;
+    hipStream_t s = dcs_stream(stream);
+    if (pool_first) {
+        const CaPoolP pp{x, (double*)part, HW, C, G, nch};
+        DCS_LAUNCH(ca_pool_kernel, dim3(nch, B), dim3(kThreads), 0, s, pp);
+        DCS_CHECK_LAUNCH();
+    }
+    const int nx = stream_grid(HW, G, B);
+    const SpPoolFcP p{x, CaFcP{(const double*)part, nch, (const float2*)w1, (const float2*)w2, (float2*)ca_out, (float2*)pooled_out,
+                               (float2*)hidden_out, HW, C, Ch}, (float4*)sp, G, nx};
+    DCS_LAUNCH(spatial_pool_fc_kernel, dim3(nx, B), dim3(kThreads), 0, s, p);
+    DCS_CHECK_LAUNCH();
+    return DCS_OK;
+}
+
+extern "C" int DCS_SYM(dcs_attention_sa_apply_fwd)(const act_t* x, const float* ca, const float* sp, const float* wsa,
+                                                   const float* sa_bias, float* sa, act_t* y, int B, int H, int W, int C,
+                                                   float drop_p, unsigned long long seed, const unsigned long long* seed_dev,
+                                                   dcs_stream_t stream) {
+    int G;
+    if (!x || !ca || !sp || !wsa || !sa || !y || B <= 0 || B > 65535 || H <= 0 || W <= 0 || !att_geom(C, &G)) return DCS_ERR_BADARG;
+    if (!(drop_p >= 0.f && drop_p < 1.f)) return DCS_ERR_BADARG;
+    SaApplyP p{x, ca, (const float4*)sp, (const float2*)wsa, (const float2*)sa_bias, (float2*)sa, y};
+    p.C = C;
+    sa_tile(B, H, W, G, &p);
+    dim3 grid(p.nx, B);
+    if (drop_p > 0.f)
+        DCS_LAUNCH(attention_sa_apply_kernel<true>, grid, dim3(kThreads), 0, dcs_stream(stream), p, drop_p, (uint64_t)seed,
+                   (const uint64_t*)seed_dev);
+    else
+        DCS_LAUNCH(attention_sa_apply_kernel<false>, grid, dim3(kThreads), 0, dcs_stream(stream), p, drop_p, (uint64_t)seed,
+                   (const uint64_t*)seed_dev);
+    DCS_CHECK_LAUNCH();
+    return DCS_OK;
+}
+
 static long fwd_batched_workspace_bytes(int n, const dcs_attention_item* items, int B) {
     if (n < 1 || n > kMaxBatch || !items || B <= 0) return -1;
     long total = 0;
@@ -316,13 +558,13 @@
 }
 #endif
 
-extern "C" int DCS_SYM(dcs_attention_fwd_batched)(int n, const dcs_attention_item* items, void* workspace, long workspace_bytes, int B,
-                                         dcs_stream_t stream) {
+static int fwd_batched(int n, const dcs_attention_item* items, void* workspace, long workspace_bytes, int B, int merges,
+                       dcs_stream_t stream) {
     if (n < 1 || n > kMaxBatch || !items || !workspace || B <= 0 || B > 65535) return DCS_ERR_BADARG;
     if (workspace_bytes < fwd_batched_workspace_bytes(n, items, B)) return DCS_ERR_WORKSPACE;
-    Tbl<CaPoolP> tp; Tbl<CaFcP> tf; Tbl<SpPoolP> ts; Tbl<ApplyP> ta;
+    Tbl<CaPoolP> tp; Tbl<CaFcP> tf; Tbl<SpPoolP> ts; Tbl<ApplyP> ta; Tbl<SpPoolFcP> tsf; Tbl<SaApplyP> tsa;
     conv::Args ca_[kMaxBatch];
-    int nx_pool = 1, nx_stream = 1;
+    int nx_pool = 1, nx_stream = 1, nx_tiles = 1;
     char* ws = (char*)workspace;
     for (int i = 0; i < n; ++i) {
         const dcs_attention_item& it = items[i];
@@ -337,6 +579,11 @@
                         (float2*)it.hidden, HW, it.C, it.Ch};
         ts.p[i] = SpPoolP{(const act_t*)it.x, it.ca, (float4*)it.sp, HW, it.C, G, nxs};
         ta.p[i] = ApplyP{(const act_t*)it.x, it.ca, (const float2*)it.sa, (act_t*)it.y, HW, it.C, G, nxs};
+        tsf.p[i] = SpPoolFcP{(const act_t*)it.x, tf.p[i], (float4*)it.sp, G, nxs};
+        tsa.p[i] = SaApplyP{(const act_t*)it.x, it.ca, (const float4*)it.sp, (const float2*)it.wsa, (const float2*)it.sa_bias,
+                            (float2*)it.sa, (act_t*)it.y};
+        tsa.p[i].C = it.C;
+        sa_tile(B, it.H, it.W, G, &tsa.p[i]);
         ws += ((long)B * nch * it.C * 2 * (long)sizeof(double) + 255) / 256 * 256;
         nx_pool = nch > nx_pool ? nch : nx_pool;
         nx_stream = nxs > nx_stream ? nxs : nx_stream;
@@ -350,25 +597,47 @@
     }
     hipStream_t s = dcs_stream(stream);
     {
-        int ap = 0, as_ = 0;
+        int ap = 0, as_ = 0, at = 0;
         for (int k = 0; k <= kMaxBatch; ++k) {
-            tp.x0[k] = k < n ? ap : 0x7fffffff; ts.x0[k] = ta.x0[k] = k < n ? as_ : 0x7fffffff;
-            if (k < n) { ap += tp.p[k].nx; as_ += ts.p[k].nx; }
-        }
-        tp.x0[n] = ap; ts.x0[n] = ta.x0[n] = as_;
-        nx_pool = ap; nx_stream = as_;
+            tp.x0[k] = k < n ? ap : 0x7fffffff; ts.x0[k] = ta.x0[k] = tsf.x0[k] = k < n ? as_ : 0x7fffffff;
+            tsa.x0[k] = k < n ? at : 0x7fffffff;
+            if (k < n) { ap += tp.p[k].nx; as_ += ts.p[k].nx; at += tsa.p[k].nx; }
+        }
+        tp.x0[n] = ap; ts.x0[n] = ta.x0[n] = tsf.x0[n] = as_; tsa.x0[n] = at;
+        nx_pool = ap; nx_stream = as_; nx_tiles = at;
     }
     DCS_LAUNCH(ca_pool_multi_kernel, dim3(nx_pool, B, 1), dim3(kThreads), 0, s, tp);
     DCS_CHECK_LAUNCH();
-    DCS_LAUNCH(ca_fc_multi_kernel, dim3(B, 1, n), dim3(kThreads), 0, s, tf);
-    DCS_CHECK_LAUNCH();
-    DCS_LAUNCH(spatial_pool_multi_kernel, dim3(nx_stream, B, 1), dim3(kThreads), 0, s, ts);
-    DCS_CHECK_LAUNCH();
+    if (merges & 1) {
+        DCS_LAUNCH(spatial_pool_fc_multi_kernel, dim3(nx_stream, B, 1), dim3(kThreads), 0, s, tsf);
+        DCS_CHECK_LAUNCH();
+    } else {
+        DCS_LAUNCH(ca_fc_multi_kernel, dim3(B, 1, n), dim3(kThreads), 0, s, tf);
+        DCS_CHECK_LAUNCH();
+        DCS_LAUNCH(spatial_pool_multi_kernel, dim3(nx_stream, B, 1), dim3(kThreads), 0, s, ts);
+        DCS_CHECK_LAUNCH();
+    }
+    if (merges & 2) {
+        DCS_LAUNCH(attention_sa_apply_multi_kernel, dim3(nx_tiles, B, 1), dim3(kThreads), 0, s, tsa);
+        DCS_CHECK_LAUNCH();
+        return DCS_OK;
+    }
     const int rc = dcs_conv_direct_multi(ca_, n, s);
     if (rc != DCS_OK) return rc;
     DCS_LAUNCH(attention_apply_multi_kernel, dim3(nx_stream, B, 1), dim3(kThreads), 0, s, ta);
     DCS_CHECK_LAUNCH();
     return DCS_OK;
+}
+
+extern "C" int DCS_SYM(dcs_attention_fwd_batched)(int n, const dcs_attention_item* items, void* workspace, long workspace_bytes, int B,
+                                         dcs_stream_t stream) {
+    return fwd_batched(n, items, workspace, workspace_bytes, B, 0, stream);
+}
+
+extern "C" int DCS_SYM(dcs_attention_fwd_batched_merged)(int n, const dcs_attention_item* items, void* workspace, long workspace_bytes,
+                                                        int B, int merges, dcs_stream_t stream) {
+    if (merges < 0 || merges > 3) return DCS_ERR_BADARG;
+    return fwd_batched(n, items, workspace, workspace_bytes, B, merges, stream);
 }
 
 #ifndef DCS_ACT_BF16
diff --git a/dcs-net_amd/dcsnet/_lib.py b/dcs-net_amd/dcsnet/_lib.py
--- a/dcs-net_amd/dcsnet/_lib.py
+++ b/dcs-net_amd/dcsnet/_lib.py
@@ -69,6 +69,9 @@
     'dcs_attention_bwd_fc_weights': (_I, [_P, _L, _P, _P, _P, _P, _P, _P, _I, _L, _I, _I, _P]),
     'dcs_attention_fwd_batched_workspace_bytes': (_L, [_I, _P, _I]),
     'dcs_attention_fwd_batched': (_I, [_I, _P, _P, _L, _I, _P]),
+    'dcs_attention_fwd_batched_merged': (_I, [_I, _P, _P, _L, _I, _I, _P]),
+    'dcs_spatial_pool_fc_fwd': (_I, [_P, _P, _L, _I] + [_P] * 6 + [_I, _L, _I, _I, _P]),
+    'dcs_attention_sa_apply_fwd': (_I, [_P] * 7 + [_I, _I, _I, _I, _F, _U64, _P, _P]),
     'dcs_attention_bwd_batched_workspace_bytes': (_L, [_I, _P, _I]),
     'dcs_attention_bwd_batched': (_I, [_I, _P, _P, _L, _I, _P]),
     'dcs_lstm_layer_fwd': (_I, [_P] * 6 + [_I, _I, _I, _I, _L, _L, _L, _P]),
@@ -162,7 +165,8 @@
 for _n in ('dcs_cconv2d_fwd', 'dcs_cconv2d_fwd_affine', 'dcs_cconv2d_fwd_stats', 'dcs_cconv2d_bwd_data', 'dcs_cconv2d_bwd_weight',
            'dcs_cconv_up2_single_fwd', 'dcs_cconv_up2_single_bwd_data', 'dcs_cconv_up2_single_bwd_weight', 'dcs_tapsum_bwd', 'dcs_cbn_fwd', 'dcs_cbn_fwd_slabs', 'dcs_cbn_fwd_slabs_pool', 'dcs_cbn_bwd', 'dcs_cbn_bwd_add',
            'dcs_channel_attention_fwd', 'dcs_spatial_pool_fwd', 'dcs_attention_apply_fwd', 'dcs_attention_fwd_batched',
-           'dcs_attention_bwd_sa', 'dcs_attention_bwd_x', 'dcs_attention_bwd_batched'):
+           'dcs_attention_bwd_sa', 'dcs_attention_bwd_x', 'dcs_attention_bwd_batched',
+           'dcs_attention_fwd_batched_merged', 'dcs_spatial_pool_fc_fwd', 'dcs_attention_sa_apply_fwd'):
     SIGNATURES[_n + '_h'] = SIGNATURES[_n]
 
 
diff --git a/dcs-net_amd/dcsnet/functional.py b/dcs-net_amd/dcsnet/functional.py
--- a/dcs-net_amd/dcsnet/functional.py
+++ b/dcs-net_amd/dcsnet/functional.py
@@ -253,6 +253,13 @@
     return ops.attention_apply(x, ca, sa, drop_p, seed)
 
 
+def _sa_apply(x, ca, sp, wsa, zero_bias, ksize, drop_p, seed):
+    if ops.FUSE_SA_APPLY and ksize == 7:
+        return ops.attention_sa_apply(x, ca, sp, wsa, zero_bias, drop_p, seed)
+    sa = ops.cconv2d(sp, None, wsa, zero_bias, (ksize, ksize), (1, 1), (ksize // 2, ksize // 2), (1, 1), ACT_SIGMOID)
+    return sa, ops.attention_apply(x, ca, sa, drop_p, seed)
+
+
 class _AttentionFn(torch.autograd.Function):
 
     @staticmethod
@@ -260,11 +267,12 @@
         w1, _ = packed_weight(fc0_r, fc0_i, None, None, False)
         w2, _ = packed_weight(fc2_r, fc2_i, None, None, False)
         wsa, zero_bias = packed_weight(c1_r, c1_i, None, None, False)
-        ca, pooled, hidden = ops.channel_attention(x, w1, w2)
-        sp = ops.spatial_pool(x, ca)
-        sa = ops.cconv2d(sp, None, wsa, zero_bias, (ksize, ksize), (1, 1), (ksize // 2, ksize // 2), (1, 1),
-                         ACT_SIGMOID)
-        out = ops.attention_apply(x, ca, sa, drop_p, seed)
+        if ops.FUSE_POOL_FC:
+            ca, pooled, hidden, sp = ops.channel_attention_spatial_pool(x, w1, w2)
+        else:
+            ca, pooled, hidden = ops.channel_attention(x, w1, w2)
+            sp = ops.spatial_pool(x, ca)
+        sa, out = _sa_apply(x, ca, sp, wsa, zero_bias, ksize, drop_p, seed)
         ctx.cfg = (ksize, float(drop_p), int(seed))
         ctx.sinks = tuple(_sink(t) for t in (fc0_r, fc0_i, fc2_r, fc2_i, c1_r, c1_i))
         ctx.save_for_backward(x, ca, sa, sp, pooled, hidden, w1, w2, wsa)
@@ -293,15 +301,19 @@
         w2, _ = packed_weight(fc2_r, fc2_i, None, None, False)
         wsa, zero_bias = packed_weight(c1_r, c1_i, None, None, False)
         if stat is not None and use_batch_stats and weight is not None and ops.FUSE_APPLY_POOL:
-            a, stats, coef, ca, pooled, hidden = ops.cbn_channel_attention(x, weight, bias, running_mean, running_covar, eps,
-                                                                           momentum, act, stat, w1, w2)
+            res = ops.cbn_channel_attention(x, weight, bias, running_mean, running_covar, eps, momentum, act, stat, w1, w2,
+                                            with_sp=ops.FUSE_POOL_FC)
+            a, stats, coef, ca, pooled, hidden = res[:6]
+            sp = res[6] if ops.FUSE_POOL_FC else ops.spatial_pool(a, ca)
         else:
             a, stats, coef = ops.cbn(x, weight, bias, running_mean, running_covar, eps, momentum, use_batch_stats, act, 0.0, 0,
                                      stat=stat)
-            ca, pooled, hidden = ops.channel_attention(a, w1, w2)
-        sp = ops.spatial_pool(a, ca)
-        sa = ops.cconv2d(sp, None, wsa, zero_bias, (ksize, ksize), (1, 1), (ksize // 2, ksize // 2), (1, 1), ACT_SIGMOID)
-        out = ops.attention_apply(a, ca, sa, drop_p, seed)
+            if ops.FUSE_POOL_FC:
+                ca, pooled, hidden, sp = ops.channel_attention_spatial_pool(a, w1, w2)
+            else:
+                ca, pooled, hidden = ops.channel_attention(a, w1, w2)
+                sp = ops.spatial_pool(a, ca)
+        sa, out = _sa_apply(a, ca, sp, wsa, zero_bias, ksize, drop_p, seed)
         ctx.cfg = (bool(use_batch_stats), act, weight is not None, ksize, float(drop_p), int(seed))
         ctx.sinks = tuple(_sink(t) for t in (weight, bias, fc0_r, fc0_i, fc2_r, fc2_i, c1_r, c1_i))
         ctx.save_for_backward(x, weight, stats, coef, a, ca, sa, sp, pooled, hidden, w1, w2, wsa)
diff --git a/dcs-net_amd/dcsnet/ops.py b/dcs-net_amd/dcsnet/ops.py
--- a/dcs-net_amd/dcsnet/ops.py
+++ b/dcs-net_amd/dcsnet/ops.py
@@ -262,6 +262,9 @@
 import os as _os
 FUSE_APPLY_POOL = _os.environ.get('DCS_FUSE_APPLY_POOL', '1') != '0'
 STATS_EPILOGUE = _os.environ.get('DCS_STATS_EPILOGUE', '1') != '0'
+FUSE_POOL_FC = _os.environ.get('DCS_FUSE_POOL_FC', '1') != '0'
+FUSE_SA_APPLY = _os.environ.get('DCS_FUSE_SA_APPLY', '1') != '0'
+FUSE_SKIP_MERGES = _os.environ.get('DCS_FUSE_SKIP_MERGES', '1') != '0'
 
 
 def _conv_bytes(act, n_in, n_out, n_w):
@@ -454,7 +457,7 @@
     return y, stats, coef
 
 
-def cbn_channel_attention(x, weight, bias, running_mean, running_covar, eps, momentum, act, stat, w1, w2):
+def cbn_channel_attention(x, weight, bias, running_mean, running_covar, eps, momentum, act, stat, w1, w2, with_sp=False):
     _chk(x, 'x', 5, act=True)
     for n, t in (('weight', weight), ('bias', bias), ('running_mean', running_mean), ('running_covar', running_covar),
                  ('w1', w1), ('w2', w2)):
@@ -477,6 +480,11 @@
                                               ptr(stats), ptr(coef), ptr(part), int(rows), int(part.shape[2]), ptr(pivot),
                                               ptr(ws), ws.numel(), B, HW, C, eps, -1.0 if momentum is None else momentum, act,
                                               cur_stream()), 'dcs_cbn_fwd_slabs_pool')
+    if with_sp:
+        sp = new(B, H, W, 2, 2)
+        check(_sym('dcs_spatial_pool_fc_fwd', a)(ptr(a), ptr(ws), ws.numel(), 0, ptr(w1), ptr(w2), ptr(ca), ptr(pooled), ptr(hidden),
+                                                 ptr(sp), B, HW, C, Ch, cur_stream()), 'dcs_spatial_pool_fc_fwd')
+        return a, stats, coef, ca, pooled, hidden, sp
     check(lib.dcs_channel_attention_fc_fwd(ptr(ws), ptr(w1), ptr(w2), ptr(ca), ptr(pooled), ptr(hidden), B, HW, C, Ch,
                                            cur_stream()), 'dcs_channel_attention_fc_fwd')
     return a, stats, coef, ca, pooled, hidden
@@ -525,6 +533,40 @@
     check(_sym('dcs_channel_attention_fwd', x)(ptr(x), ptr(w1), ptr(w2), ptr(ca), ptr(pooled), ptr(hidden), ptr(ws),
                                         ws.numel(), B, H * W, C, Ch, cur_stream()), 'dcs_channel_attention_fwd')
     return ca, pooled, hidden
+
+
+def channel_attention_spatial_pool(x, w1, w2):
+    _chk(x, 'x', 5, act=True)
+    _chk(w1, 'w1')
+    _chk(w2, 'w2')
+    B, H, W, C, _ = x.shape
+    Ch = w1.shape[-2]
+    new = lambda *sh: torch.empty(sh, dtype=torch.float32, device=x.device)
+    ca, pooled, hidden, sp = new(B, C, 2), new(B, C, 2), new(B, Ch, 2), new(B, H, W, 2, 2)
+    nbytes = _lib.load().dcs_ca_workspace_bytes(B, H * W, C)
+    if nbytes < 0:
+        raise _lib.DcsHipError(f'channel_attention_spatial_pool: unsupported channel count C={C}')
+    ws = _workspace(nbytes, x.device)
+    check(_sym('dcs_spatial_pool_fc_fwd', x)(ptr(x), ptr(ws), ws.numel(), 1, ptr(w1), ptr(w2), ptr(ca), ptr(pooled), ptr(hidden),
+                                             ptr(sp), B, H * W, C, Ch, cur_stream()), 'dcs_spatial_pool_fc_fwd')
+    return ca, pooled, hidden, sp
+
+
+def attention_sa_apply(x, ca, sp, wsa, bias, drop_p=0.0, seed=0):
+    _chk(x, 'x', 5, act=True)
+    _chk(ca, 'ca', 3)
+    _chk(sp, 'sp', 5)
+    _chk(wsa, 'wsa', 4)
+    _chk(bias, 'bias', 2)
+    B, H, W, C, _ = x.shape
+    if tuple(wsa.shape[:3]) != (49, 2, 1) or tuple(sp.shape) != (B, H, W, 2, 2) or tuple(ca.shape) != (B, C, 2):
+        raise _lib.DcsHipError(f'attention_sa_apply: wsa {tuple(wsa.shape)}, sp {tuple(sp.shape)}, ca {tuple(ca.shape)} for x {tuple(x.shape)}')
+    sa = torch.empty((B, H, W, 1, 2), dtype=torch.float32, device=x.device)
+    y = torch.empty_like(x)
+    check(_sym('dcs_attention_sa_apply_fwd', x, y)(ptr(x), ptr(ca), ptr(sp), ptr(wsa), ptr(bias), ptr(sa), ptr(y), B, H, W, C,
+                                                   float(drop_p), int(seed), ptr(SEED_STATE), cur_stream()),
+          'dcs_attention_sa_apply_fwd')
+    return sa, y
 
 
 def spatial_pool(x, ca=None):
@@ -625,7 +667,9 @@
     if nbytes < 0:
         raise _lib.DcsHipError('attention_blocks_fwd: unsupported block geometry')
     ws = _workspace(nbytes, dev)
-    check(_sym('dcs_attention_fwd_batched', *xs)(n, items, ptr(ws), ws.numel(), B, cur_stream()), 'dcs_attention_fwd_batched')
+    merges = (1 if FUSE_POOL_FC else 0) | (2 if FUSE_SA_APPLY else 0) if FUSE_SKIP_MERGES else 0
+    check(_sym('dcs_attention_fwd_batched_merged', *xs)(n, items, ptr(ws), ws.numel(), B, merges, cur_stream()),
+          'dcs_attention_fwd_batched_merged')
     return outs
 
 
diff --git a/include/dcsnet_hip.h b/include/dcsnet_hip.h
--- a/include/dcsnet_hip.h
+++ b/include/dcsnet_hip.h
@@ -133,6 +133,13 @@
                             int B, long HW, int C, float drop_p, unsigned long long seed,
                             const unsigned long long* seed_dev, dcs_stream_t stream);
 
+int dcs_spatial_pool_fc_fwd(const float* x, void* part, long part_bytes, int pool_first, const float* w1, const float* w2,
+                            float* ca_out, float* pooled_out, float* hidden_out, float* sp,
+                            int B, long HW, int C, int Ch, dcs_stream_t stream);
+int dcs_attention_sa_apply_fwd(const float* x, const float* ca, const float* sp, const float* wsa, const float* sa_bias,
+                               float* sa, float* y, int B, int H, int W, int C, float drop_p, unsigned long long seed,
+                               const unsigned long long* seed_dev, dcs_stream_t stream);
+
 typedef struct {
     const float* x; const float* w1; const float* w2; const float* wsa; const float* sa_bias;
     float* ca; float* pooled; float* hidden; float* sp; float* sa; float* y;
@@ -144,6 +151,8 @@
 long dcs_attention_fwd_batched_workspace_bytes(int n, const dcs_attention_item* items, int B);
 int dcs_attention_fwd_batched(int n, const dcs_attention_item* items, void* workspace, long workspace_bytes, int B,
                               dcs_stream_t stream);
+int dcs_attention_fwd_batched_merged(int n, const dcs_attention_item* items, void* workspace, long workspace_bytes, int B,
+                                     int merges, dcs_stream_t stream);
 long dcs_attention_bwd_batched_workspace_bytes(int n, const dcs_attention_item* items, int B);
 int dcs_attention_bwd_batched(int n, const dcs_attention_item* items, void* workspace, long workspace_bytes, int B,
                               dcs_stream_t stream);
@@ -413,6 +422,14 @@
                               const unsigned long long* seed_dev, dcs_stream_t stream);
 int dcs_attention_fwd_batched_h(int n, const dcs_attention_item* items, void* workspace, long workspace_bytes, int B,
                                 dcs_stream_t stream);
+int dcs_attention_fwd_batched_merged_h(int n, const dcs_attention_item* items, void* workspace, long workspace_bytes, int B,
+                                       int merges, dcs_stream_t stream);
+int dcs_spatial_pool_fc_fwd_h(const dcs_bf16_t* x, void* part, long part_bytes, int pool_first, const float* w1, const float* w2,
+                              float* ca_out, float* pooled_out, float* hidden_out, float* sp,
+                              int B, long HW, int C, int Ch, dcs_stream_t stream);
+int dcs_attention_sa_apply_fwd_h(const dcs_bf16_t* x, const float* ca, const float* sp, const float* wsa, const float* sa_bias,
+                                 float* sa, dcs_bf16_t* y, int B, int H, int W, int C, float drop_p, unsigned long long seed,
+                                 const unsigned long long* seed_dev, dcs_stream_t stream);
 int dcs_attention_bwd_sa_h(const dcs_bf16_t* x, const dcs_bf16_t* g_out, const float* ca, const float* sa, float* g_pre,
                            int B, long HW, int C, float drop_p, unsigned long long seed, const unsigned long long* seed_dev,
                            dcs_stream_t stream);
```

Result: no change. 2.589 million, median of 6 (+0.7%).
